# XiaoHan-Git/RO-MAP

Hardware: AMD Instinct MI355X
Metric: ray-samples/sec (train: hash-encode->MLP->composite fwd+bwd+optimizer) per object-NeRF (higher is better)
Workload: dtype fp16 params/activations, fp32 accumulate + fp32 master; 1 GPU; OfflineNeRF-style training, 1 synthetic 'room'-like object per GPU, base.json defaults (hash L=16 F=2 T=2^16, MLP 64x1), R=4096 rays x S=32 samples/step, 40 views 640x480 resident in HBM; objects=1, samples_per_ray=32, backend=1, parallelism=object-per-GPU (no training collective; RCCL gather-to-root of the final render), launcher=single process, ranks_in_collective=1, visible_devices=1

## Files before the change

include/mon_core_diag.h:

```cpp
#ifndef MON_CORE_DIAG_H
#define MON_CORE_DIAG_H
#include "mon_core.h"
#ifdef __cplusplus
extern "C" {
#endif

int mon_object_debug_read(mon_object* obj, int which, void* dst, size_t bytes);
int mon_dataset_debug_read(mon_dataset* ds, uint32_t frame, uint32_t* rgba, float* depth, float* pose16);
int mon_microbench(int device, int mode, int pattern, uint32_t n_entries, uint32_t n_ops, float* ms);
int mon_debug_fast_index(const mon_config* cfg, int level, uint32_t x, uint32_t y, uint32_t z, uint32_t* index, uint32_t* size);
int mon_debug_frag_layout(int encoded_width_padded, int n_neurons, int n_hidden_layers, int n_levels, int* source, int* slots, int* n_image, int* n_mlp);
int mon_debug_acc_layout(int encoded_width_padded, int n_neurons, int n_hidden_layers, int n_levels, int* param, int* n_cols);
int mon_selftest_mfma(int device, const uint16_t* A, const uint16_t* B, float* D);
int mon_debug_yaml_number(const char* text, const char* key, double* value);
int mon_debug_occupancy_state(mon_object* obj, uint32_t out[2]);
int mon_debug_occupancy_grid(mon_object* obj, uint32_t* raw, uint32_t* dilated, float* raw_threshold, uint32_t* n_parts);
int mon_debug_set_train_occupancy(mon_object* obj, const uint32_t* bits);

int mon_debug_render_jobs(mon_object* obj, int side, uint32_t* jobs);

int mon_debug_set_render_grid(mon_object* obj, int side, const uint32_t* bits);

int mon_debug_scene_samples(mon_object* const* objs, size_t n_objs, int side, mon_frame_bbox rect, const float* Twc16, size_t k, float* t, float* alpha,
                            float* rgb, uint32_t* count);
int mon_debug_scene_composite(int device, uint32_t n_rays, uint32_t n_lists, const float* t, const float* alpha, const float* rgb, const uint32_t* count,
                              const float* dn, float* out_rgb, float* out_depth, float* out_opacity, int32_t* out_instance);

int mon_debug_pose_samples(mon_object* obj, int side, const mon_frame_bbox* obs, size_t n_obs, const float* Tow16, const mon_pose_refine_params* p,
                           uint32_t iteration, float* x, float* raw, float* dldx);

int mon_debug_scene_pose_samples(mon_object* const* objs, size_t n_objs, int side, const mon_frame_bbox* obs, size_t n_obs, const float* Twc16,
                                 const mon_pose_refine_params* p, uint32_t iteration, const float* level_weights, size_t k, float* x_o, float* x_c, float* t,
                                 float* raw, float* dldx, uint32_t* count);
int mon_debug_scene_composite_grad(int device, uint32_t n_rays, uint32_t n_lists, const float* t, const float* alpha, const float* rgb, const uint32_t* count,
                                   const float* cstar, const float* mstar, const float* dstar, const float* dn, float w_rgb, float w_mask, float w_depth,
                                   float huber, float* out_l, float* out_W, float* out_D, float* out_dalpha, float* out_dc);
int mon_debug_checkpoint_timing(int enable, double* kernel_ms);

#ifdef __cplusplus
}
#endif
#endif
```

ro-map_amd/__init__.py:

```python
from .binding import (MonConfig, MonBBox, MonError, Dataset, ObjectNeRF, default_config, config_from_json, device_count, lib, lib_path,
                      exported_symbols, BUF, selftest_mfma, microbench, fast_index, OfflineManager, OnlineManager, png_read, png_write, marching_cubes,
                              generate_toc, frag_layout, acc_layout, device_mem_info, set_logical_devices, set_offline_schedule, set_option, get_option, diag_lib, diag_lib_path,
                              diag_symbols, yaml_number, MonRenderSkipStats, render_scene, scene_samples, scene_composite, PoseRefineParams, pose_refine_default,
                      PoseC2FParams, pose_c2f_default, pose_c2f_weights, scene_pose_loss, scene_refine_camera, scene_pose_samples,
                      scene_composite_grad, CheckpointInfo, checkpoint_info, checkpoint_timing, MON_LOAD_BOXES,
                      rccl_lib, rccl_lib_path, rccl_symbols, gather_plan, Gather)
```

ro-map_amd/binding.py:

```python
import ctypes as C
import os

import numpy as np

_HERE = os.path.dirname(os.path.abspath(__file__))


class MonError(RuntimeError):
    def __init__(self, code, msg):
        super().__init__("mon_core error %d: %s" % (code, msg)); self.code = code


class MonConfig(C.Structure):
    _fields_ = [("n_levels", C.c_int32), ("n_features", C.c_int32), ("log2_hashmap_size", C.c_int32), ("base_resolution", C.c_int32),
                ("per_level_scale", C.c_float), ("n_neurons", C.c_int32), ("n_hidden_layers", C.c_int32), ("rays_per_batch", C.c_int32),
                ("n_samples", C.c_int32), ("loss_scale", C.c_float), ("learning_rate", C.c_float), ("beta1", C.c_float), ("beta2", C.c_float),
                ("epsilon", C.c_float), ("l2_reg", C.c_float), ("ema_decay", C.c_float), ("decay_start", C.c_int32), ("decay_interval", C.c_int32),
                ("decay_base", C.c_float), ("param_seed", C.c_uint32), ("rng_flags", C.c_uint32), ("sample_seed", C.c_uint64),
                ("use_depth", C.c_int32), ("occupancy_skip", C.c_int32)]


class MonBBox(C.Structure):
    _fields_ = [("FrameId", C.c_uint32), ("x", C.c_uint32), ("y", C.c_uint32), ("h", C.c_uint32), ("w", C.c_uint32)]

# ... 19 lines not shown


class CheckpointInfo(C.Structure):
    _fields_ = [("version", C.c_uint32), ("cfg", MonConfig), ("class_id", C.c_int32), ("Tow", C.c_float * 16), ("aabb_min", C.c_float * 3),
                ("aabb_max", C.c_float * 3), ("n_params", C.c_uint32), ("n_mlp_params", C.c_uint32), ("n_grid_params", C.c_uint32),
                ("train_step", C.c_uint32), ("iter", C.c_uint32), ("n_boxes", C.c_uint32), ("backend", C.c_int32), ("has_occupancy", C.c_uint32),
                ("lazy_ema", C.c_uint32), ("file_bytes", C.c_uint64)]


MON_LOAD_BOXES = 1


def checkpoint_info(path, verify=True):
    i = CheckpointInfo(); _check(lib().mon_checkpoint_read_info(os.fsencode(path), int(bool(verify)), C.byref(i))); return i


def checkpoint_timing(enable=True):
    ms = C.c_double(0); _check(diag_lib().mon_debug_checkpoint_timing(int(bool(enable)), C.byref(ms))); return ms.value


class MonProfile(C.Structure):
    _fields_ = [("ms", C.c_double * 8), ("launches", C.c_uint64 * 8)]


K_BATCH, K_FWDBWD, K_OPTIM, K_RENDER = 0, 1, 2, 3

_SIGS = {
    "mon_last_error": (C.c_char_p, []),
    "mon_version": (C.c_int, []),
    "mon_device_count": (C.c_int, [C.POINTER(C.c_int)]),
    "mon_set_logical_devices": (C.c_int, [C.c_int]),
    "mon_offline_set_schedule": (C.c_int, [C.c_int, C.c_int]),
    "mon_set_option": (C.c_int, [C.c_char_p, C.c_long]),
    "mon_get_option": (C.c_int, [C.c_char_p, C.POINTER(C.c_long)]),
    "mon_config_default": (C.c_int, [C.POINTER(MonConfig)]),
    "mon_config_from_json": (C.c_int, [C.c_char_p, C.POINTER(MonConfig)]),
    "mon_dataset_create": (C.c_int, [C.c_int, C.c_int, C.c_int, C.c_float, C.c_float, C.c_float, C.c_float, C.c_uint32, C.c_int, C.POINTER(C.c_void_p)]),
    "mon_dataset_add_frame": (C.c_int, [C.c_void_p, C.c_uint32, C.c_void_p, C.c_int, C.c_int, C.c_void_p, C.c_void_p, C.c_void_p]),
    "mon_dataset_n_frames": (C.c_int, [C.c_void_p, C.POINTER(C.c_uint32)]),
    "mon_dataset_destroy": (C.c_int, [C.c_void_p]),
    "mon_object_create": (C.c_int, [C.c_void_p, C.POINTER(MonConfig), C.c_int, C.c_void_p, C.c_void_p, C.c_void_p, C.POINTER(C.c_void_p)]),
    "mon_object_add_boxes": (C.c_int, [C.c_void_p, C.c_void_p, C.c_size_t]),
    "mon_object_train": (C.c_int, [C.c_void_p, C.c_int, C.POINTER(C.c_float)]),
    "mon_object_render": (C.c_int, [C.c_void_p, MonBBox, C.c_void_p, C.c_int, C.c_void_p, C.c_void_p, C.c_void_p, C.c_int]),
    "mon_object_render_snapshot": (C.c_int, [C.c_void_p, MonBBox, C.c_void_p, C.c_int, C.c_void_p, C.c_void_p, C.c_void_p, C.POINTER(C.c_uint32)]),
    "mon_object_density_grid": (C.c_int, [C.c_void_p, C.c_int, C.c_int, C.c_int, C.c_void_p]),
    "mon_object_info_get": (C.c_int, [C.c_void_p, C.POINTER(MonInfo)]),
    "mon_object_get_params": (C.c_int, [C.c_void_p, C.c_int, C.c_void_p, C.c_size_t]),
    "mon_object_set_params": (C.c_int, [C.c_void_p, C.c_void_p, C.c_size_t]),
    "mon_object_train_stages": (C.c_int, [C.c_void_p, C.c_int]),
    "mon_object_set_backend": (C.c_int, [C.c_void_p, C.c_int]),
    "mon_object_set_debug_dump": (C.c_int, [C.c_void_p, C.c_int]),
    "mon_object_set_profiling": (C.c_int, [C.c_void_p, C.c_int]),
    "mon_object_get_profile": (C.c_int, [C.c_void_p, C.POINTER(MonProfile), C.c_int]),
    "mon_object_destroy": (C.c_int, [C.c_void_p]),
    "mon_offline_create": (C.c_int, [C.c_char_p, C.c_char_p, C.c_int, C.POINTER(C.c_void_p)]),
    "mon_offline_init": (C.c_int, [C.c_void_p]),
    "mon_offline_read_dataset": (C.c_int, [C.c_void_p]),
    "mon_offline_create_nerf": (C.c_int, [C.c_void_p, C.c_char_p]),
    "mon_offline_wait_threads_end": (C.c_int, [C.c_void_p]),
    "mon_offline_n_objects": (C.c_int, [C.c_void_p, C.POINTER(C.c_int)]),
    "mon_offline_object_loss": (C.c_int, [C.c_void_p, C.c_int, C.POINTER(C.c_float), C.POINTER(C.c_int)]),
    "mon_offline_render_test": (C.c_int, [C.c_void_p, C.c_int, C.c_char_p, C.c_int]),
    "mon_offline_save_mesh": (C.c_int, [C.c_void_p, C.c_int, C.c_char_p]),
    "mon_offline_destroy": (C.c_int, [C.c_void_p]),
    "mon_object_generate_mesh": (C.c_int, [C.c_void_p, C.c_int, C.c_float, C.POINTER(C.c_uint32), C.POINTER(C.c_uint32)]),
    "mon_object_mesh_counts": (C.c_int, [C.c_void_p, C.POINTER(C.c_uint32), C.POINTER(C.c_uint32), C.POINTER(C.c_uint32)]),
    "mon_object_get_mesh": (C.c_int, [C.c_void_p, C.c_void_p, C.c_void_p, C.c_void_p, C.c_void_p, C.c_int]),
    "mon_device_mem_info": (C.c_int, [C.c_int, C.c_void_p, C.c_void_p]),
    "mon_object_mesh_generation": (C.c_int, [C.c_void_p, C.c_void_p]),
    "mon_object_get_config": (C.c_int, [C.c_void_p, C.c_void_p]),
    "mon_object_copy_mesh": (C.c_int, [C.c_void_p, C.c_uint32, C.c_uint32, C.c_void_p, C.c_void_p, C.c_void_p, C.c_void_p, C.c_void_p, C.c_void_p, C.c_void_p,
            C.c_int]),
    "mon_object_get_mesh_raw": (C.c_int, [C.c_void_p, C.c_void_p, C.c_void_p]),
    "mon_object_save_mesh": (C.c_int, [C.c_void_p, C.c_char_p]),
    "mon_marching_cubes": (C.c_int, [C.c_int, C.c_void_p, C.c_int, C.c_int, C.c_int, C.c_float, C.c_void_p, C.c_void_p, C.c_void_p, C.c_void_p, C.c_void_p,
            C.c_uint32, C.c_uint32,
                                     C.POINTER(C.c_uint32), C.POINTER(C.c_uint32), C.POINTER(C.c_uint32)]),
    "mon_offline_get_intrinsics": (C.c_int, [C.c_void_p] + [C.POINTER(C.c_float)] * 4 + [C.POINTER(C.c_int)] * 2),
    "mon_offline_get_poses": (C.c_int, [C.c_void_p, C.c_void_p, C.c_size_t, C.POINTER(C.c_size_t)]),
    "mon_offline_object_meta": (C.c_int, [C.c_void_p, C.c_int, C.POINTER(C.c_int), C.c_void_p, C.c_void_p, C.c_void_p, C.c_void_p, C.c_size_t,
            C.POINTER(C.c_size_t)]),
    "mon_offline_set_output_dir": (C.c_int, [C.c_void_p, C.c_char_p]),
    "mon_offline_object": (C.c_int, [C.c_void_p, C.c_int, C.POINTER(C.c_void_p)]),
    "mon_online_object": (C.c_int, [C.c_void_p, C.c_size_t, C.POINTER(C.c_void_p)]),
    "mon_online_render_nerfs_test": (C.c_int, [C.c_void_p, C.c_char_p, C.c_size_t, C.POINTER(C.c_char_p), C.c_void_p, C.c_void_p, C.c_size_t, C.c_float]),
    "mon_generate_toc": (C.c_int, [C.c_float, C.c_float, C.c_float, C.c_void_p]),
    "mon_online_create": (C.c_int, [C.c_char_p, C.c_int, C.c_int, C.POINTER(C.c_void_p)]),
    "mon_online_init": (C.c_int, [C.c_void_p]),
    "mon_online_dataset_init": (C.c_int, [C.c_void_p, C.c_float, C.c_float, C.c_float, C.c_float, C.c_int, C.c_int, C.c_size_t]),
    "mon_online_new_frame": (C.c_int, [C.c_void_p, C.c_uint32, C.c_char_p, C.c_void_p, C.c_int, C.c_void_p, C.c_void_p, C.c_void_p]),
    "mon_online_create_nerf": (C.c_int, [C.c_void_p, C.c_int, C.c_void_p, C.c_void_p, C.c_void_p, C.POINTER(C.c_size_t)]),
    "mon_online_update_nerf_bbox": (C.c_int, [C.c_void_p, C.c_size_t, C.c_void_p, C.c_size_t, C.c_int]),
    "mon_online_get_frame_idx": (C.c_int, [C.c_void_p, C.c_char_p, C.POINTER(C.c_int)]),
    "mon_online_update_dataset": (C.c_int, [C.c_void_p, C.c_uint32, C.c_uint32, C.c_void_p]),
    "mon_online_get_pose": (C.c_int, [C.c_void_p, C.c_uint32, C.c_void_p]),
    "mon_online_wait_threads_end": (C.c_int, [C.c_void_p]),
    "mon_online_object_info": (C.c_int, [C.c_void_p, C.c_size_t, C.POINTER(C.c_float), C.POINTER(C.c_int), C.POINTER(C.c_int), C.POINTER(C.c_uint32)]),
    "mon_online_render": (C.c_int, [C.c_void_p, C.c_size_t, MonBBox, C.c_void_p, C.c_void_p, C.c_void_p, C.c_void_p]),
    "mon_online_destroy": (C.c_int, [C.c_void_p]),
    "mon_png_read": (C.c_int, [C.c_char_p, C.POINTER(C.c_int), C.POINTER(C.c_int), C.POINTER(C.c_int), C.POINTER(C.c_int), C.c_void_p, C.c_size_t]),
    "mon_png_write": (C.c_int, [C.c_char_p, C.c_int, C.c_int, C.c_int, C.c_int, C.c_void_p]),
    "mon_write_render_pngs": (C.c_int, [C.c_char_p, C.c_char_p, C.c_char_p, C.c_uint32, C.c_uint32, C.c_void_p, C.c_void_p, C.c_void_p]),
    "mon_physical_device": (C.c_int, [C.c_int, C.POINTER(C.c_int)]),
    "mon_offline_object_stamp": (C.c_int, [C.c_void_p, C.c_int, C.c_size_t, C.c_char_p, C.c_size_t]),
    "mon_device_synchronize": (C.c_int, [C.c_int]),
    "mon_object_set_render_skip": (C.c_int, [C.c_void_p, C.c_int, C.c_float]),
    "mon_object_render_skip_stats": (C.c_int, [C.c_void_p, C.c_int, C.POINTER(MonRenderSkipStats)]),
    "mon_object_render_occupancy": (C.c_int, [C.c_void_p, C.c_int, C.c_int, C.c_void_p]),
    "mon_scene_render": (C.c_int, [C.c_void_p, C.c_size_t, C.c_int, MonBBox, C.c_void_p, C.c_void_p, C.c_void_p, C.c_void_p, C.c_void_p]),
    "mon_online_render_scene": (C.c_int, [C.c_void_p, MonBBox, C.c_void_p, C.c_void_p, C.c_void_p, C.c_void_p, C.c_void_p]),
    "mon_pose_refine_default": (C.c_int, [C.POINTER(PoseRefineParams)]),
    "mon_object_pose_loss": (C.c_int, [C.c_void_p, C.c_int, C.c_void_p, C.c_size_t, C.c_void_p, C.POINTER(PoseRefineParams), C.c_uint32,
            C.POINTER(C.c_float), C.c_void_p]),
    "mon_object_refine_pose": (C.c_int, [C.c_void_p, C.c_int, C.c_void_p, C.c_size_t, C.POINTER(PoseRefineParams), C.c_void_p, C.c_void_p]),
    "mon_online_refine_pose": (C.c_int, [C.c_void_p, C.c_size_t, C.c_void_p, C.c_size_t, C.POINTER(PoseRefineParams), C.c_void_p, C.c_void_p]),
    "mon_pose_c2f_default": (C.c_int, [C.POINTER(PoseC2FParams)]),
    "mon_pose_c2f_weights": (C.c_int, [C.POINTER(PoseC2FParams), C.c_int, C.c_int, C.c_int, C.c_void_p]),
    "mon_object_pose_loss_levels": (C.c_int, [C.c_void_p, C.c_int, C.c_void_p, C.c_size_t, C.c_void_p, C.POINTER(PoseRefineParams), C.c_uint32,
            C.c_void_p, C.POINTER(C.c_float), C.c_void_p]),
    "mon_object_refine_pose_c2f": (C.c_int, [C.c_void_p, C.c_int, C.c_void_p, C.c_size_t, C.POINTER(PoseRefineParams), C.POINTER(PoseC2FParams),
            C.c_void_p, C.c_void_p]),
    "mon_online_refine_pose_c2f": (C.c_int, [C.c_void_p, C.c_size_t, C.c_void_p, C.c_size_t, C.POINTER(PoseRefineParams), C.POINTER(PoseC2FParams),
            C.c_void_p, C.c_void_p]),
    "mon_scene_pose_loss": (C.c_int, [C.c_void_p, C.c_size_t, C.c_int, C.c_void_p, C.c_size_t, C.c_void_p, C.POINTER(PoseRefineParams), C.c_uint32,
            C.c_void_p, C.POINTER(C.c_float), C.c_void_p]),
    "mon_scene_refine_camera": (C.c_int, [C.c_void_p, C.c_size_t, C.c_int, C.c_void_p, C.c_size_t, C.POINTER(PoseRefineParams), C.POINTER(PoseC2FParams),
            C.c_void_p, C.c_void_p]),
    "mon_online_refine_camera": (C.c_int, [C.c_void_p, C.c_void_p, C.c_size_t, C.POINTER(PoseRefineParams), C.POINTER(PoseC2FParams), C.c_void_p,
            C.c_void_p]),
    "mon_checkpoint_read_info": (C.c_int, [C.c_char_p, C.c_int, C.c_void_p]),
    "mon_object_save": (C.c_int, [C.c_void_p, C.c_char_p]),
    "mon_object_load": (C.c_int, [C.c_void_p, C.c_char_p, C.c_uint32, C.POINTER(C.c_void_p)]),
    "mon_online_save_map": (C.c_int, [C.c_void_p, C.c_char_p]),
    "mon_online_load_map": (C.c_int, [C.c_void_p, C.c_char_p, C.c_uint32, C.POINTER(C.c_size_t)]),
}


_DIAG_SIGS = {
    "mon_object_debug_read": (C.c_int, [C.c_void_p, C.c_int, C.c_void_p, C.c_size_t]),
    "mon_dataset_debug_read": (C.c_int, [C.c_void_p, C.c_uint32, C.c_void_p, C.c_void_p, C.c_void_p]),
    "mon_microbench": (C.c_int, [C.c_int, C.c_int, C.c_int, C.c_uint32, C.c_uint32, C.POINTER(C.c_float)]),
    "mon_debug_frag_layout": (C.c_int, [C.c_int, C.c_int, C.c_int, C.c_int, C.c_void_p, C.c_void_p, C.POINTER(C.c_int), C.POINTER(C.c_int)]),
    "mon_debug_acc_layout": (C.c_int, [C.c_int, C.c_int, C.c_int, C.c_int, C.c_void_p, C.POINTER(C.c_int)]),
    "mon_debug_fast_index": (C.c_int, [C.POINTER(MonConfig), C.c_int, C.c_uint32, C.c_uint32, C.c_uint32, C.POINTER(C.c_uint32), C.POINTER(C.c_uint32)]),
    "mon_selftest_mfma": (C.c_int, [C.c_int, C.c_void_p, C.c_void_p, C.c_void_p]),
    "mon_debug_yaml_number": (C.c_int, [C.c_char_p, C.c_char_p, C.POINTER(C.c_double)]),
    "mon_debug_render_jobs": (C.c_int, [C.c_void_p, C.c_int, C.POINTER(C.c_uint32)]),
    "mon_debug_occupancy_state": (C.c_int, [C.c_void_p, C.POINTER(C.c_uint32)]),
    "mon_debug_occupancy_grid": (C.c_int, [C.c_void_p, C.c_void_p, C.c_void_p, C.POINTER(C.c_float), C.POINTER(C.c_uint32)]),
    "mon_debug_set_train_occupancy": (C.c_int, [C.c_void_p, C.c_void_p]),
    "mon_debug_set_render_grid": (C.c_int, [C.c_void_p, C.c_int, C.c_void_p]),
    "mon_debug_checkpoint_timing": (C.c_int, [C.c_int, C.POINTER(C.c_double)]),
    "mon_debug_scene_samples": (C.c_int, [C.c_void_p, C.c_size_t, C.c_int, MonBBox, C.c_void_p, C.c_size_t, C.c_void_p, C.c_void_p, C.c_void_p, C.c_void_p]),
    "mon_debug_scene_composite": (C.c_int, [C.c_int, C.c_uint32, C.c_uint32, C.c_void_p, C.c_void_p, C.c_void_p, C.c_void_p, C.c_void_p, C.c_void_p,
            C.c_void_p, C.c_void_p, C.c_void_p]),
    "mon_debug_pose_samples": (C.c_int, [C.c_void_p, C.c_int, C.c_void_p, C.c_size_t, C.c_void_p, C.POINTER(PoseRefineParams), C.c_uint32, C.c_void_p,
            C.c_void_p, C.c_void_p]),
    "mon_debug_scene_pose_samples": (C.c_int, [C.c_void_p, C.c_size_t, C.c_int, C.c_void_p, C.c_size_t, C.c_void_p, C.POINTER(PoseRefineParams), C.c_uint32,
            C.c_void_p, C.c_size_t, C.c_void_p, C.c_void_p, C.c_void_p, C.c_void_p, C.c_void_p, C.c_void_p]),
    "mon_debug_scene_composite_grad": (C.c_int, [C.c_int, C.c_uint32, C.c_uint32, C.c_void_p, C.c_void_p, C.c_void_p, C.c_void_p, C.c_void_p, C.c_void_p,
            C.c_void_p, C.c_void_p, C.c_float, C.c_float, C.c_float, C.c_float, C.c_void_p, C.c_void_p, C.c_void_p, C.c_void_p, C.c_void_p]),
}


def exported_symbols():
    return sorted(_SIGS)


_RCCL_SIGS = {
    "mon_gather_create": (C.c_int, [C.c_int, C.POINTER(C.c_void_p)]),
    "mon_gather_destroy": (C.c_int, [C.c_void_p]),
    "mon_gather_plan": (C.c_int, [C.c_void_p, C.c_void_p, C.c_int, C.c_int, C.c_void_p, C.c_void_p]),
    "mon_gather_renders": (C.c_int, [C.c_void_p, C.c_void_p, C.c_void_p, C.c_void_p, C.c_int, C.c_int, C.c_void_p, C.c_void_p, C.c_void_p]),
    "mon_gather_stats": (C.c_int, [C.c_void_p, C.POINTER(C.c_uint64), C.POINTER(C.c_uint64), C.POINTER(C.c_int), C.POINTER(C.c_double)]),
    "mon_gather_transport_stats": (C.c_int, [C.c_void_p, C.POINTER(C.c_int), C.POINTER(C.c_uint64), C.POINTER(C.c_int), C.POINTER(C.c_uint64), C.POINTER(C.c_int)]),
    "mon_gather_set_transport": (C.c_int, [C.c_void_p, C.c_int]),
    "mon_gather_last_error": (C.c_char_p, []),
    "mon_offline_render_test_gathered": (C.c_int, [C.c_void_p, C.c_void_p, C.c_char_p, C.c_int]),
}
_rccl_lib = None


def rccl_symbols():
    return sorted(_RCCL_SIGS)


def rccl_lib_path():
    return os.path.join(os.path.dirname(os.path.abspath(__file__)), "libmon_core_rccl.so")


def rccl_lib():
    global _rccl_lib
    if _rccl_lib is None:
        lib()
        L = C.CDLL(rccl_lib_path(), mode=C.RTLD_GLOBAL)
        for name, (res, args) in _RCCL_SIGS.items():
            f = getattr(L, name); f.restype = res; f.argtypes = args
        _rccl_lib = L
    return _rccl_lib


def gather_plan(object_device, n_pix, n_devices):
    d = np.ascontiguousarray(object_device, np.int32); p = np.ascontiguousarray(n_pix, np.uint32)
    per = np.zeros(n_devices, np.uint64); off = np.zeros(len(d), np.uint64)
    rc = rccl_lib().mon_gather_plan(_p(d), _p(p), len(d), int(n_devices), _p(per), _p(off))
    if rc:
        raise MonError(rc, "mon_gather_plan failed")
    return per, off


def _gather_error():
    return (rccl_lib().mon_gather_last_error() or b"").decode("utf-8", "replace")


class Gather:

    def __init__(self, root_device=0):
        self.h = C.c_void_p()
        rc = rccl_lib().mon_gather_create(int(root_device), C.byref(self.h))
        if rc:
            raise MonError(rc, "mon_gather_create: " + _gather_error())

    AUTO, RCCL, PEER_COPY = 0, 1, 2

    def set_transport(self, transport):
        rc = rccl_lib().mon_gather_set_transport(self.h, int(transport))
        if rc:
            raise MonError(rc, "mon_gather_set_transport: " + _gather_error())

    def renders(self, objects, boxes, poses16, pose_is_Toc=False):
        n = len(objects); b = np.ascontiguousarray(boxes, np.uint32).reshape(n, 5); T = np.ascontiguousarray(poses16, np.float32).reshape(n, 16)
        oh = (C.c_void_p * n)(*[o.h for o in objects])
        rgb = [np.empty((int(q[3]), int(q[4]), 3), np.float32) for q in b]; dep = [np.empty((int(q[3]), int(q[4])), np.float32) for q in b]
        msk = [np.empty_like(d) for d in dep]
        pr = (C.c_void_p * n)(*[a.ctypes.data for a in rgb]); pd = (C.c_void_p * n)(*[a.ctypes.data for a in dep])
        pm = (C.c_void_p * n)(*[a.ctypes.data for a in msk])
        rc = rccl_lib().mon_gather_renders(self.h, oh, _p(b), _p(T), int(pose_is_Toc), n, pr, pd, pm)
        if rc:
            raise MonError(rc, "mon_gather_renders: " + _gather_error())
        return list(zip(rgb, dep, msk))

    def stats(self):
        a = C.c_uint64(0); b = C.c_uint64(0); s = C.c_int(0); ms = C.c_double(0)
        rccl_lib().mon_gather_stats(self.h, C.byref(a), C.byref(b), C.byref(s), C.byref(ms))
        nr = C.c_int(0); br = C.c_uint64(0); mr = C.c_int(0); bc = C.c_uint64(0); mc = C.c_int(0)
        rccl_lib().mon_gather_transport_stats(self.h, C.byref(nr), C.byref(br), C.byref(mr), C.byref(bc), C.byref(mc))
        return dict(bytes_over_links=a.value, bytes_on_root=b.value, sending_devices=s.value, transfer_ms=ms.value, n_ranks=nr.value, bytes_rccl=br.value,
                messages_rccl=mr.value, bytes_peer_copy=bc.value, messages_peer_copy=mc.value)

    def offline_render_test(self, manager, out_dir, max_views=0):
        rc = rccl_lib().mon_offline_render_test_gathered(self.h, manager.h, out_dir.encode(), int(max_views))
        if rc:
            raise MonError(rc, "mon_offline_render_test_gathered: " + _gather_error())

    def close(self):
        if self.h:
            rccl_lib().mon_gather_destroy(self.h); self.h = C.c_void_p()


def diag_symbols():
    return sorted(_DIAG_SIGS)


def lib_path():
    return os.environ.get("MON_CORE_LIB") or os.path.join(_HERE, "libmon_core.so")


_lib = None


def lib():
    global _lib
    if _lib is None:
        p = lib_path()
        if not os.path.exists(p):
            raise MonError(-1, "libmon_core.so not built (run python -c 'import __graft_entry__ as g; g.build()')")
        L = C.CDLL(p)
        for name, (res, args) in _SIGS.items():
            fn = getattr(L, name); fn.restype = res; fn.argtypes = args
        _lib = L
        for kv in filter(None, os.environ.get("MON_OPTIONS", "").split(",")):
            k, v = kv.split("=")
            if k.strip() == "offline_schedule":
                o, i = v.lower().split("x"); rc = L.mon_offline_set_schedule(int(o), int(i))
            else:
                rc = L.mon_set_option(k.strip().encode(), int(v))
            if rc != 0:
                raise MonError(rc, L.mon_last_error().decode("utf-8", "replace"))
    return _lib


_diag = None


def diag_lib_path():
    return os.path.join(os.path.dirname(lib_path()), "libmon_core_diag.so")


def diag_lib():
    global _diag
    if _diag is None:
        lib()
        p = diag_lib_path()
        if not os.path.exists(p):
            raise MonError(-1, "libmon_core_diag.so not built")
        L = C.CDLL(p)
        for name, (res, args) in _DIAG_SIGS.items():
            fn = getattr(L, name); fn.restype = res; fn.argtypes = args
        _diag = L
    return _diag


def set_option(name, value):
    _check(lib().mon_set_option(name.encode(), int(value)))


def get_option(name):
    v = C.c_long(0); _check(lib().mon_get_option(name.encode(), C.byref(v))); return v.value


def yaml_number(text, key):
    v = C.c_double(0); _check(diag_lib().mon_debug_yaml_number(text.encode(), key.encode(), C.byref(v))); return v.value


def _check(rc):
    if rc != 0:
        raise MonError(rc, lib().mon_last_error().decode("utf-8", "replace"))


def _p(a):
    return None if a is None else a.ctypes.data_as(C.c_void_p)


def device_count():
    n = C.c_int(0)
    rc = lib().mon_device_count(C.byref(n))
    return n.value if rc == 0 else 0


def set_offline_schedule(outer=10, inner=500):
    _check(lib().mon_offline_set_schedule(int(outer), int(inner)))


def set_logical_devices(n):
    _check(lib().mon_set_logical_devices(int(n)))


def device_mem_info(device=0):
    f = C.c_size_t(0); t = C.c_size_t(0); _check(lib().mon_device_mem_info(int(device), C.byref(f), C.byref(t))); return f.value, t.value


def default_config(**kw):
    c = MonConfig(); _check(lib().mon_config_default(C.byref(c)))
    kw = dict(kw)
    rng = int(kw.pop("xorwow", 0)) | (int(bool(kw.pop("tcnn_init_order", 0))) << 4) | ((int(kw.pop("xorwow_lanes", 0)) // 1024) << 16)
    for k, v in kw.items():
        setattr(c, k, v)
    c.rng_flags |= rng
    return c


def config_from_json(path):
    c = MonConfig(); _check(lib().mon_config_from_json(path.encode(), C.byref(c))); return c


def selftest_mfma(A_h, B_h, device=0):
    A = np.ascontiguousarray(A_h, np.uint16); B = np.ascontiguousarray(B_h, np.uint16); D = np.empty((32, 32), np.float32)
    _check(diag_lib().mon_selftest_mfma(device, _p(A), _p(B), _p(D))); return D


def fast_index(cfg, level, x, y, z):
    i = C.c_uint32(0); n = C.c_uint32(0); _check(diag_lib().mon_debug_fast_index(C.byref(cfg), level, x, y, z, C.byref(i), C.byref(n))); return i.value, n.value


def microbench(mode, pattern, n_entries, n_ops, device=0):
    ms = C.c_float(0); _check(diag_lib().mon_microbench(device, mode, pattern, n_entries, n_ops, C.byref(ms))); return ms.value


class Dataset:

    def __init__(self, device, H, W, fx, fy, cx, cy, max_frames, use_depth=False):
        self.h = C.c_void_p(); self.H, self.W = H, W
        _check(lib().mon_dataset_create(device, H, W, fx, fy, cx, cy, max_frames, int(use_depth), C.byref(self.h)))

    def add_frame(self, frame_id, rgb_u8, instance_u8, Twc16, depth=None, is_bgr=False):
        rgb = np.ascontiguousarray(rgb_u8, np.uint8); inst = np.ascontiguousarray(instance_u8, np.uint8)
        pose = np.ascontiguousarray(Twc16, np.float32); d = None if depth is None else np.ascontiguousarray(depth, np.float32)
        assert rgb.shape[:2] == (self.H, self.W) and inst.shape == (self.H, self.W) and pose.size == 16
        _check(lib().mon_dataset_add_frame(self.h, frame_id, _p(rgb), rgb.shape[2], int(is_bgr), _p(inst), _p(d), _p(pose)))

    @property
    def n_frames(self):
        n = C.c_uint32(0); _check(lib().mon_dataset_n_frames(self.h, C.byref(n))); return n.value

    def debug_read(self, frame_id, with_depth=False):
        rgba = np.empty((self.H, self.W), np.uint32); pose = np.empty(16, np.float32); dep = np.empty((self.H, self.W), np.float32) if with_depth else None
        _check(diag_lib().mon_dataset_debug_read(self.h, frame_id, _p(rgba), _p(dep), _p(pose)))
        return rgba, dep, pose

    def close(self):
        if self.h:
            lib().mon_dataset_destroy(self.h); self.h = None


BUF = dict(master=0, half=1, ema=2, m1=3, m2=4, steps=5, gmlp=6, ggrid_h=9, pts=10, tdist=11, E=12, Hid=13, O=14, dO=15, dHid=16, dE=17,
           rgb_ray=18, depth_ray=19, mask_ray=20, loss_ray=21, ray_o=22, ray_d=23, ray_t0=24, ray_t1=25, target=26, target_depth=27, bgcol=28,
           ray_flag=29, ray_dn=31, mask=32, state=33, frag_train=34, frag_ref=35, x_all=36, e_soa=37, half_tiles=38, ggrid_f32=39, live_cnt=40)


class ObjectNeRF:

    def __init__(self, dataset, cfg, class_id, Tow16, aabb_min, aabb_max):
        self.h = C.c_void_p(); self.cfg = cfg; self.ds = dataset
        a, b, c = (np.ascontiguousarray(v, np.float32) for v in (Tow16, aabb_min, aabb_max))
        _check(lib().mon_object_create(dataset.h, C.byref(cfg), int(class_id), _p(a), _p(b), _p(c), C.byref(self.h)))
        self.R, self.S = cfg.rays_per_batch, cfg.n_samples

    def close(self):
        if self.h:
            lib().mon_object_destroy(self.h); self.h = None

    def add_boxes(self, boxes):
        b = np.ascontiguousarray(boxes, np.uint32).reshape(-1, 5)
        _check(lib().mon_object_add_boxes(self.h, _p(b), b.shape[0]))

    def save(self, path):
        _check(lib().mon_object_save(self.h, os.fsencode(path)))

    @classmethod
    def load(cls, dataset, path, with_boxes=True):
        h = C.c_void_p()
        _check(lib().mon_object_load(dataset.h, os.fsencode(path), MON_LOAD_BOXES if with_boxes else 0, C.byref(h)))
        o = cls.__new__(cls); o.h = h; o.ds = dataset
        o.cfg = MonConfig(); _check(lib().mon_object_get_config(h, C.byref(o.cfg))); o.R, o.S = o.cfg.rays_per_batch, o.cfg.n_samples
        return o

    def train(self, iters):
        loss = C.c_float(0); _check(lib().mon_object_train(self.h, iters, C.byref(loss))); return loss.value

    def train_stages(self, bits):
        _check(lib().mon_object_train_stages(self.h, bits))

    def set_backend(self, backend):
        _check(lib().mon_object_set_backend(self.h, backend))

    def info(self):
        i = MonInfo(); _check(lib().mon_object_info_get(self.h, C.byref(i))); return i

    def render(self, box, pose16, pose_is_Toc=False):
        FrameId, x, y, h, w = (int(v) for v in box)
        rgb = np.empty((h, w, 3), np.float32); depth = np.empty((h, w), np.float32); mask = np.empty((h, w), np.float32)
        pose = np.ascontiguousarray(pose16, np.float32)
        _check(lib().mon_object_render(self.h, MonBBox(FrameId, x, y, h, w), _p(pose), int(pose_is_Toc), _p(rgb), _p(depth), _p(mask), 0))
        return rgb, depth, mask

    def render_snapshot(self, box, pose16, pose_is_Toc=False):
        FrameId, x, y, h, w = (int(v) for v in box)
        rgb = np.empty((h, w, 3), np.float32); depth = np.empty((h, w), np.float32); mask = np.empty((h, w), np.float32); st = C.c_uint32(0)
        pose = np.ascontiguousarray(pose16, np.float32)
        _check(lib().mon_object_render_snapshot(self.h, MonBBox(FrameId, x, y, h, w), _p(pose), int(pose_is_Toc), _p(rgb), _p(depth), _p(mask), C.byref(st)))
        return rgb, depth, mask, st.value

    def render_into(self, box, pose16, rgb_ptr, depth_ptr, mask_ptr, on_device, pose_is_Toc=False):
        FrameId, x, y, h, w = (int(v) for v in box)
        pose = np.ascontiguousarray(pose16, np.float32)
        _check(lib().mon_object_render(self.h, MonBBox(FrameId, x, y, h, w), _p(pose), int(pose_is_Toc), C.c_void_p(int(rgb_ptr)), C.c_void_p(int(depth_ptr)),
                C.c_void_p(int(mask_ptr)), int(bool(on_device))))

    def generate_mesh(self, res=64, thresh=2.0):
        nv = C.c_uint32(0); ni = C.c_uint32(0)
        _check(lib().mon_object_generate_mesh(self.h, int(res), float(thresh), C.byref(nv), C.byref(ni))); return nv.value, ni.value

    def get_mesh(self, try_lock=False, raw=False):
        nv = C.c_uint32(0); nr = C.c_uint32(0); ni = C.c_uint32(0)
        _check(lib().mon_object_mesh_counts(self.h, C.byref(nv), C.byref(nr), C.byref(ni)))
        for _ in range(8):
            cv, ci = nv.value, ni.value
            out = dict(verts=np.empty((cv, 3), np.float32), normals=np.empty((cv, 3), np.float32), colors=np.empty((cv, 3), np.uint8), indices=np.empty(ci,
                    np.uint32))
            rc = lib().mon_object_copy_mesh(self.h, cv, ci, _p(out["verts"]), _p(out["normals"]), _p(out["colors"]), _p(out["indices"]),
                                            C.byref(nv), C.byref(nr), C.byref(ni), int(try_lock))
            if rc == 1 and (nv.value > cv or ni.value > ci):
                continue
            _check(rc); break
        else:
            raise MonError(1, "get_mesh: mesh kept growing")
        out = {k: (v[:nv.value] if k != "indices" else v[:ni.value]) for k, v in out.items()}; out["n_verts_real"] = nr.value
        if raw:
            out["normals_raw"] = np.empty((nv.value, 3), np.float32); out["colors_f32"] = np.empty((nv.value, 3), np.float32)
            _check(lib().mon_object_get_mesh_raw(self.h, _p(out["normals_raw"]), _p(out["colors_f32"])))
        return out

    def mesh_generation(self):
        g = C.c_uint64(0); _check(lib().mon_object_mesh_generation(self.h, C.byref(g))); return g.value

    def save_mesh(self, path):
        _check(lib().mon_object_save_mesh(self.h, path.encode()))

    def set_render_skip(self, enable, min_alpha=1e-3):
        _check(lib().mon_object_set_render_skip(self.h, int(bool(enable)), float(min_alpha)))

    def render_skip_stats(self, side=0):
        st = MonRenderSkipStats(); _check(lib().mon_object_render_skip_stats(self.h, int(side), C.byref(st)))
        return {f: int(getattr(st, f)) for f, _ in MonRenderSkipStats._fields_}

    def render_occupancy(self, side=0, dilated=True):
        w = np.empty(8192, np.uint32); _check(lib().mon_object_render_occupancy(self.h, int(side), int(bool(dilated)), _p(w)))
        return np.unpackbits(w.view(np.uint8), bitorder="little").astype(bool).reshape(64, 64, 64)

    def debug_set_render_grid(self, side, grid):
        if grid is None:
            _check(diag_lib().mon_debug_set_render_grid(self.h, int(side), None)); return
        w = np.packbits(np.ascontiguousarray(grid, bool).reshape(-1), bitorder="little").view(np.uint32)
        _check(diag_lib().mon_debug_set_render_grid(self.h, int(side), _p(w)))

    def density_grid(self, rx, ry, rz):
        out = np.empty(rx * ry * rz, np.float32); _check(lib().mon_object_density_grid(self.h, rx, ry, rz, _p(out))); return out

    def get_params(self, which=0):
        n = self.info().n_params
        out = np.empty(n, np.float32 if which == 0 else np.uint16)
        _check(lib().mon_object_get_params(self.h, which, _p(out), out.nbytes)); return out

    def set_params(self, master):
        m = np.ascontiguousarray(master, np.float32); _check(lib().mon_object_set_params(self.h, _p(m), m.size))

    def buffer(self, name):
        i = self.info(); R, B, n = self.R, self.R * self.S, i.n_params
        W, NH, Ep = self.cfg.n_neurons, self.cfg.n_hidden_layers, i.encoded_width
        shapes = dict(master=(np.float32, n), half=(np.uint16, n), ema=(np.uint16, n), m1=(np.float32, n), m2=(np.float32, n), steps=(np.uint32, n),
                      gmlp=(np.float32, i.n_mlp_params), ggrid_h=(np.uint16, i.n_grid_params), ggrid_f32=(np.float32, i.n_grid_params), pts=(np.float32, B * 3), tdist=(np.float32, B),
                      E=(np.uint16, B * Ep), Hid=(np.uint16, B * W * NH), O=(np.uint16, B * 4), dO=(np.uint16, B * 4), dHid=(np.uint16, B * W * NH),
                      dE=(np.uint16, B * Ep), rgb_ray=(np.float32, R * 3), depth_ray=(np.float32, R), mask_ray=(np.float32, R), loss_ray=(np.float32, R),
                      ray_o=(np.float32, R * 3), ray_d=(np.float32, R * 3), ray_t0=(np.float32, R), ray_t1=(np.float32, R), target=(np.float32, R * 3),
                      target_depth=(np.float32, R), bgcol=(np.float32, R * 3), ray_flag=(np.uint8, R), ray_dn=(np.float32, R), mask=(np.uint64, R // 64),
                      state=(np.uint32, 28 + 2 * 128 * 16), frag_train=(np.uint16, 64 * 512), frag_ref=(np.uint16, 64 * 512),
                      live_cnt=(np.uint32, 2 * 64 * 16), x_all=(np.float32, B * 4), e_soa=(np.uint16, B * 2 * self.cfg.n_levels), half_tiles=(np.uint16, i.n_grid_params))
        dt, cnt = shapes[name]; out = np.empty(cnt, dt)
        _check(diag_lib().mon_object_debug_read(self.h, BUF[name], _p(out), out.nbytes)); return out

    def occupancy_state(self):
        out = (C.c_uint32 * 2)(); _check(diag_lib().mon_debug_occupancy_state(self.h, out)); return int(out[0]), int(out[1])

    def occupancy_grid(self):
        raw = np.empty(8192, np.uint32); dil = np.empty(8192, np.uint32); thr = C.c_float(0); n_parts = C.c_uint32(0)
        _check(diag_lib().mon_debug_occupancy_grid(self.h, _p(raw), _p(dil), C.byref(thr), C.byref(n_parts)))
        return raw, dil, float(thr.value), int(n_parts.value)

    def set_train_occupancy(self, bits):
        if bits is None:
            _check(diag_lib().mon_debug_set_train_occupancy(self.h, None)); return
        w = np.ascontiguousarray(bits, np.uint32); assert w.size == 8192
        _check(diag_lib().mon_debug_set_train_occupancy(self.h, _p(w)))

    def render_jobs(self, side=0):
        n = C.c_uint32(0); _check(diag_lib().mon_debug_render_jobs(self.h, int(side), C.byref(n))); return n.value

    def pose_loss(self, obs, Tow16, params=None, side=0, iteration=0):
        b, prm = _pose_boxes(obs), _pose_params(params); pose = np.ascontiguousarray(Tow16, np.float32).reshape(16)
        loss = C.c_float(0); g = np.empty(6, np.float32)
        _check(lib().mon_object_pose_loss(self.h, int(side), _p(b), b.shape[0], _p(pose), C.byref(prm), int(iteration), C.byref(loss), _p(g)))
        return loss.value, g

    def refine_pose(self, obs, Tow16, params=None, side=0):
        b, prm = _pose_boxes(obs), _pose_params(params); pose = np.array(Tow16, np.float32).reshape(16)
        trace = np.empty(prm.iters + 1, np.float32)
        _check(lib().mon_object_refine_pose(self.h, int(side), _p(b), b.shape[0], C.byref(prm), _p(pose), _p(trace)))
        return pose, trace

    def pose_loss_levels(self, obs, Tow16, level_weights, params=None, side=0, iteration=0):
        b, prm = _pose_boxes(obs), _pose_params(params); pose = np.ascontiguousarray(Tow16, np.float32).reshape(16)
        w = np.ascontiguousarray(level_weights, np.float32).reshape(-1)
        if w.size != self.cfg.n_levels:
            raise ValueError("level_weights: %d values for %d levels" % (w.size, self.cfg.n_levels))
        loss = C.c_float(0); g = np.empty(6, np.float32)
        _check(lib().mon_object_pose_loss_levels(self.h, int(side), _p(b), b.shape[0], _p(pose), C.byref(prm), int(iteration), _p(w), C.byref(loss), _p(g)))
        return loss.value, g

    def refine_pose_c2f(self, obs, Tow16, params=None, c2f=None, side=0):
        b, prm, c = _pose_boxes(obs), _pose_params(params), _c2f_params(c2f); pose = np.array(Tow16, np.float32).reshape(16)
        trace = np.empty(prm.iters + 1, np.float32)
        _check(lib().mon_object_refine_pose_c2f(self.h, int(side), _p(b), b.shape[0], C.byref(prm), C.byref(c), _p(pose), _p(trace)))
        return pose, trace

    def pose_samples(self, obs, Tow16, params=None, side=0, iteration=0):
        b, prm = _pose_boxes(obs), _pose_params(params); pose = np.ascontiguousarray(Tow16, np.float32).reshape(16)
        n = int(prm.rays_per_iter) or int(sum(int(v[3]) * int(v[4]) for v in b))
        x = np.empty((n, 64, 3), np.float32); raw = np.empty((n, 64, 4), np.float32); g = np.empty((n, 64, 3), np.float32)
        _check(diag_lib().mon_debug_pose_samples(self.h, int(side), _p(b), b.shape[0], _p(pose), C.byref(prm), int(iteration), _p(x), _p(raw), _p(g)))
        return x, raw, g

    def set_debug_dump(self, on):
        _check(lib().mon_object_set_debug_dump(self.h, int(on)))

    def set_profiling(self, on):
        _check(lib().mon_object_set_profiling(self.h, int(on)))

    def profile(self, reset=True):
        p = MonProfile(); _check(lib().mon_object_get_profile(self.h, C.byref(p), int(reset)))
        return {"ms": list(p.ms), "launches": list(p.launches)}


def png_read(path):
    w, h, c, d = C.c_int(0), C.c_int(0), C.c_int(0), C.c_int(0)
    _check(lib().mon_png_read(path.encode(), C.byref(w), C.byref(h), C.byref(c), C.byref(d), None, 0))
    buf = np.empty(w.value * h.value * c.value * d.value // 8, np.uint8)
    _check(lib().mon_png_read(path.encode(), C.byref(w), C.byref(h), C.byref(c), C.byref(d), _p(buf), buf.nbytes))
    if d.value == 16:
        return buf.view(">u2").astype(np.uint16).reshape(h.value, w.value, c.value)
    return buf.reshape(h.value, w.value, c.value)


def png_write(path, arr):
    a = np.asarray(arr)
    if a.ndim == 2:
        a = a[..., None]
    data = np.ascontiguousarray(a.astype(">u2") if a.dtype == np.uint16 else a.astype(np.uint8))
    _check(lib().mon_png_write(path.encode(), a.shape[1], a.shape[0], a.shape[2], 16 if arr.dtype == np.uint16 else 8, data.ctypes.data_as(C.c_void_p)))


class OfflineManager:

    def __init__(self, dataset_path, config_path, use_dense_depth=False):
        self.h = C.c_void_p()
        _check(lib().mon_offline_create(dataset_path.encode(), config_path.encode(), int(use_dense_depth), C.byref(self.h)))

    def init(self):
        _check(lib().mon_offline_init(self.h))

    def read_dataset(self):
        _check(lib().mon_offline_read_dataset(self.h))

    def create_nerf(self, object_file):
        _check(lib().mon_offline_create_nerf(self.h, object_file.encode()))

    def wait_threads_end(self):
        _check(lib().mon_offline_wait_threads_end(self.h))

    def n_objects(self):
        n = C.c_int(0); _check(lib().mon_offline_n_objects(self.h, C.byref(n))); return n.value

    def object_loss(self, idx):
        l = C.c_float(0); d = C.c_int(0); _check(lib().mon_offline_object_loss(self.h, idx, C.byref(l), C.byref(d))); return l.value, d.value

    def set_output_dir(self, path):
        _check(lib().mon_offline_set_output_dir(self.h, path.encode()))

    def intrinsics(self):
        f = [C.c_float(0) for _ in range(4)]; hw = [C.c_int(0), C.c_int(0)]
        _check(lib().mon_offline_get_intrinsics(self.h, *[C.byref(v) for v in f + hw])); return tuple(v.value for v in f + hw)

    def poses(self):
        n = C.c_size_t(0); _check(lib().mon_offline_get_poses(self.h, None, 0, C.byref(n)))
        T = np.empty((n.value, 16), np.float32); _check(lib().mon_offline_get_poses(self.h, _p(T), n.value, C.byref(n))); return T

    def object_meta(self, idx):
        n = C.c_size_t(0); cls = C.c_int(0); Tow = np.empty(16, np.float32); a0 = np.empty(3, np.float32); a1 = np.empty(3, np.float32)
        _check(lib().mon_offline_object_meta(self.h, idx, C.byref(cls), _p(Tow), _p(a0), _p(a1), None, 0, C.byref(n)))
        boxes = np.empty((n.value, 5), np.uint32)
        _check(lib().mon_offline_object_meta(self.h, idx, None, None, None, None, _p(boxes), n.value, C.byref(n)))
        return dict(cls=cls.value, Tow=Tow, aabb_min=a0, aabb_max=a1, boxes=boxes)

    def object(self, idx):
        h = C.c_void_p(); _check(lib().mon_offline_object(self.h, idx, C.byref(h))); return _borrowed_object(h)

    def render_test(self, idx, out_dir, max_views=0):
        _check(lib().mon_offline_render_test(self.h, idx, out_dir.encode(), max_views))

    def close(self):
        if self.h:
            lib().mon_offline_destroy(self.h); self.h = None


class OnlineManager:

    def __init__(self, config_path, use_sparse_depth=False, train_step_iterations=500):
        self.h = C.c_void_p()
        _check(lib().mon_online_create(config_path.encode(), int(use_sparse_depth), int(train_step_iterations), C.byref(self.h)))

    def init(self):
        _check(lib().mon_online_init(self.h))

    def dataset_init(self, fx, fy, cx, cy, H, W, imgs):
        _check(lib().mon_online_dataset_init(self.h, fx, fy, cx, cy, H, W, imgs))

    def new_frame(self, img_id, stamp, bgr_u8, instance_u8, Twc16, depth=None):
        bgr = np.ascontiguousarray(bgr_u8, np.uint8); inst = np.ascontiguousarray(instance_u8, np.uint8); pose = np.ascontiguousarray(Twc16, np.float32)
        d = None if depth is None else np.ascontiguousarray(depth, np.float32)
        _check(lib().mon_online_new_frame(self.h, img_id, stamp.encode(), _p(bgr), bgr.shape[2], _p(inst), _p(d), _p(pose)))

    def create_nerf(self, cls, Tow16, aabb_min, aabb_max):
        a, b, c = (np.ascontiguousarray(v, np.float32) for v in (Tow16, aabb_min, aabb_max)); idx = C.c_size_t(0)
        _check(lib().mon_online_create_nerf(self.h, int(cls), _p(a), _p(b), _p(c), C.byref(idx))); return idx.value

    def update_nerf_bbox(self, idx, boxes, train_step):
        b = np.ascontiguousarray(boxes, np.uint32).reshape(-1, 5)
        _check(lib().mon_online_update_nerf_bbox(self.h, idx, _p(b), b.shape[0], int(train_step)))

    def update_dataset(self, cur_id, Twc16s):
        T = np.ascontiguousarray(Twc16s, np.float32).reshape(-1, 16); _check(lib().mon_online_update_dataset(self.h, int(cur_id), T.shape[0], _p(T)))

    def get_pose(self, frame_id):
        T = np.empty(16, np.float32); _check(lib().mon_online_get_pose(self.h, int(frame_id), _p(T))); return T

    def get_frame_idx(self, stamp):
        i = C.c_int(0); _check(lib().mon_online_get_frame_idx(self.h, stamp.encode(), C.byref(i))); return i.value

# ... 220 lines not shown
```

ro-map_amd/csrc/diag.cpp:

```cpp
#include <algorithm>
#include <cstring>
#include <string>
#include <vector>
#include "model.h"
#include "frag_layout.h"
#include "../../include/mon_core_diag.h"

namespace mon {
void set_error(const char* fmt, ...);
int ensure_ema_current(Model& m);
int microbench(int device, int mode, int pattern, uint32_t n_entries, uint32_t n_ops, float* ms);
int selftest_mfma(int device, const uint16_t* A, const uint16_t* B, float* D);
bool read_yaml_number(const std::string& text, const char* key, double& v);

#define HIPCHECK(expr)                                                                                         \
    do { hipError_t _e = (expr); if (_e != hipSuccess) {                                                       \
        set_error("%s failed: %s (%s:%d)", #expr, hipGetErrorString(_e), __FILE__, __LINE__); return MON_ERR_HIP; } } while (0)

int model_debug_read(Model& m, int which, void* dst, size_t bytes) {
    model_leave_lane(m);
    if (which == MON_BUF_EMA) { int rc = ensure_ema_current(m); if (rc) return rc; }
    const size_t R = m.oc.R, B = R * m.oc.S, n = m.n_params; const void* src = nullptr; size_t sz = 0;
    if (m.P.rec && (which == MON_BUF_MASTER || which == MON_BUF_M1 || which == MON_BUF_M2 || which == MON_BUF_STEPS)) {
        if (!dst || bytes < n * 4) { set_error("debug_read: buffer too small"); return MON_ERR_ARG; }
        HIPCHECK(use_device(m.device)); void* tmp = nullptr; HIPCHECK(hipMalloc(&tmp, n * 4));
        launch_state_unpack(m.train_stream, m.P.rec, which == MON_BUF_MASTER ? 0 : which == MON_BUF_M1 ? 1 : which == MON_BUF_M2 ? 2 : 3, tmp, (uint32_t)n);
        hipError_t e = hipStreamSynchronize(m.train_stream); if (e == hipSuccess) e = hipMemcpy(dst, tmp, n * 4, hipMemcpyDeviceToHost);
        (void)hipFree(tmp); HIPCHECK(e); return MON_OK;
    }
    switch (which) {
        case MON_BUF_MASTER: src = m.P.master; sz = n * 4; break;       case MON_BUF_HALF: src = m.P.half; sz = n * 2; break;
        case MON_BUF_EMA: src = m.P.ema; sz = n * 2; break;             case MON_BUF_M1: src = m.P.m1; sz = n * 4; break;
        case MON_BUF_M2: src = m.P.m2; sz = n * 4; break;
        case MON_BUF_STEPS: src = m.P.steps ? (const void*)m.P.steps : (const void*)m.P.steps16; sz = n * 4; break;
        case MON_BUF_GMLP: src = m.P.gmlp; sz = (size_t)m.nd.n_mlp * 4; break;
        case MON_BUF_GGRID_H: src = m.P.ggrid; sz = (size_t)m.n_grid * 2; break;
        case MON_BUF_GGRID_F32: src = m.P.ggrid; sz = (size_t)m.n_grid * 4; break;
        case MON_BUF_PTS: src = m.B.pts; sz = B * 12; break;            case MON_BUF_TDIST: src = m.B.tdist; sz = B * 4; break;
        case MON_BUF_E: src = m.B.E; sz = B * m.nd.Epad * 2; break;     case MON_BUF_HID: src = m.B.Hid; sz = B * m.nd.W * m.nd.NH * 2; break;
        case MON_BUF_O: src = m.B.O; sz = B * 8; break;                 case MON_BUF_DO: src = m.B.dO; sz = B * 8; break;
        case MON_BUF_DHID: src = m.B.dHid; sz = B * m.nd.W * m.nd.NH * 2; break;
        case MON_BUF_DE: src = m.B.dE; sz = B * m.nd.Epad * 2; break;
        case MON_BUF_RGB_RAY: src = m.B.rgb_ray; sz = R * 12; break;    case MON_BUF_DEPTH_RAY: src = m.B.depth_ray; sz = R * 4; break;
        case MON_BUF_MASK_RAY: src = m.B.mask_ray; sz = R * 4; break;   case MON_BUF_LOSS_RAY: src = m.B.loss_ray; sz = R * 4; break;
        case MON_BUF_RAY_O: src = m.B.ray_o; sz = R * 12; break;        case MON_BUF_RAY_D: src = m.B.ray_d; sz = R * 12; break;
        case MON_BUF_RAY_T0: src = m.B.ray_t0; sz = R * 4; break;       case MON_BUF_RAY_T1: src = m.B.ray_t1; sz = R * 4; break;
        case MON_BUF_TARGET: src = m.B.target; sz = R * 12; break;      case MON_BUF_TARGET_DEPTH: src = m.B.target_depth; sz = R * 4; break;
        case MON_BUF_BGCOL: src = m.B.bgcol; sz = R * 12; break;        case MON_BUF_RAY_FLAG: src = m.B.ray_flag; sz = R; break;
        case MON_BUF_RAY_DN: src = m.B.ray_dn; sz = R * 4; break;       case MON_BUF_MASK: src = m.B.mask; sz = (R / 64) * 8; break;
        case MON_BUF_STATE: src = m.d_state; sz = sizeof(DevState); break;
        case MON_BUF_FRAG_TRAIN: src = m.d_frag_train; sz = 64 * 512 * 2; break;
        case MON_BUF_X_ALL: if (!m.d_x_all) { set_error("debug_read: level-tile encode not in use"); return MON_ERR_STATE; } src = m.d_x_all; sz = B * 16;
        break;
        case MON_BUF_E_SOA: if (!m.d_e_soa) { set_error("debug_read: level-tile encode not in use"); return MON_ERR_STATE; } src = m.d_e_soa;
        sz = B * (size_t)m.nd.L * 4; break;
        case MON_BUF_HALF_TILES: if (!m.d_half_tiles) { set_error("debug_read: level-tile encode not in use"); return MON_ERR_STATE; } src = m.d_half_tiles;
        sz = (size_t)m.n_grid * 2; break;
        case MON_BUF_LIVE_CNT: if (!m.d_live_cnt) { set_error("debug_read: no live-sample lists (occupancy_skip off, or not on the level tiles)"); return MON_ERR_STATE; }
            src = m.d_live_cnt; sz = 2u * kLiveMaxParts * kLiveCntStride * 4u; break;
        case MON_BUF_FRAG_REF:
            if (!m.d_frag_render) { set_error("debug_read: fused backend not available"); return MON_ERR_STATE; }
            HIPCHECK(use_device(m.device)); HIPCHECK(hipMemsetAsync(m.d_frag_render, 0, 64 * 512 * 2, m.train_stream));
            launch_build_frag_image(m.train_stream, m.P.half, m.nd, m.d_frag_render); src = m.d_frag_render; sz = 64 * 512 * 2; break;
        default: set_error("debug_read: unknown buffer id %d", which); return MON_ERR_ARG;
    }
    if (!dst || bytes < sz) { set_error("debug_read: buffer too small (%zu < %zu)", bytes, sz); return MON_ERR_ARG; }
    HIPCHECK(use_device(m.device)); HIPCHECK(hipStreamSynchronize(m.train_stream));
    if (which == MON_BUF_STEPS && !m.P.steps) {
        std::vector<uint16_t> h16(n); HIPCHECK(hipMemcpy(h16.data(), src, n * 2, hipMemcpyDeviceToHost));
        uint32_t* out = reinterpret_cast<uint32_t*>(dst); for (size_t i = 0; i < n; ++i) out[i] = h16[i];
        return MON_OK;
    }
    if (which == MON_BUF_GGRID_H || which == MON_BUF_GGRID_F32) {
        std::vector<uint16_t> tab(m.n_grid); HIPCHECK(hipMemcpy(tab.data(), m.P.ggrid, (size_t)m.n_grid * 2, hipMemcpyDeviceToHost));
        std::vector<float> acc(m.n_grid);
        for (uint32_t i = 0; i < m.n_grid; ++i) { _Float16 h; std::memcpy(&h, &tab[i], 2); acc[i] = (float)h; }
        const bool parts = (m.backend == 1 && m.lds_mask) || (m.backend == 0 && m.hybrid_scatter && which == MON_BUF_GGRID_F32);
        if (parts) {
            const uint32_t n_ent = m.part_halves / 2, n_half = n_ent / 2;
            std::vector<uint16_t> pa(m.part_halves), pb(m.part_halves);
            auto val = [&](const std::vector<uint16_t>& part, uint32_t e, uint32_t f) { _Float16 h;
                std::memcpy(&h, &part[((size_t)f * 2 + (e & 1u)) * n_half + (e >> 1)], 2); return (float)h; };
            for (uint32_t q = 0; q < m.scatter.max_P; q += 2) {
                HIPCHECK(hipMemcpy(pa.data(), m.d_gpart + (size_t)q * m.part_halves, (size_t)m.part_halves * 2, hipMemcpyDeviceToHost));
                if (q + 1 < m.scatter.max_P) HIPCHECK(hipMemcpy(pb.data(), m.d_gpart + (size_t)(q + 1) * m.part_halves, (size_t)m.part_halves * 2,
                        hipMemcpyDeviceToHost));
                for (int l = 0; l < m.nd.L; ++l) {
                    const bool lds_level = m.backend == 1 ? ((m.lds_mask >> l) & 1u) != 0u : true;
                    if (q >= m.scatter.P[l] || !lds_level) continue;
                    const bool two = q + 1 < m.scatter.P[l];
                    for (uint32_t e = m.lt.offset[l]; e < m.lt.offset[l + 1]; ++e) for (uint32_t f = 0; f < 2; ++f)
                        acc[2 * e + f] += two ? val(pa, e, f) + val(pb, e, f) : val(pa, e, f);
                }
            }
        }
        if (which == MON_BUF_GGRID_F32) {
            if (!dst || bytes < (size_t)m.n_grid * 4) { set_error("debug_read: buffer too small"); return MON_ERR_ARG; }
            std::memcpy(dst, acc.data(), (size_t)m.n_grid * 4); return MON_OK;
        }
        uint16_t* out = reinterpret_cast<uint16_t*>(dst);
        for (uint32_t i = 0; i < m.n_grid; ++i) { const _Float16 h = (_Float16)acc[i]; std::memcpy(&out[i], &h, 2); }
        return MON_OK;
    }
    HIPCHECK(hipMemcpy(dst, src, sz, hipMemcpyDeviceToHost));
    return MON_OK;
}


}

using namespace mon;
#define REQUIRE(p, what) do { if (!(p)) { set_error("%s: null %s", __func__, what); return MON_ERR_ARG; } } while (0)

extern "C" {
int mon_object_debug_read(mon_object* o, int which, void* dst, size_t bytes) { REQUIRE(o, "object"); return model_debug_read(*o->m, which, dst, bytes); }
int mon_dataset_debug_read(mon_dataset* ds, uint32_t frame, uint32_t* rgba, float* depth, float* pose16) {
    REQUIRE(ds, "dataset"); Dataset& d = *ds->d;
    if (frame >= d.max_frames) { set_error("dataset_debug_read: frame %u >= capacity %u", frame, d.max_frames); return MON_ERR_ARG; }
    const size_t px = (size_t)d.K.H * d.K.W;
    HIPCHECK(use_device(d.device)); HIPCHECK(hipDeviceSynchronize());
    if (rgba) HIPCHECK(hipMemcpy(rgba, d.d_rgba + px * frame, px * 4, hipMemcpyDeviceToHost));
    if (depth && d.d_depth) HIPCHECK(hipMemcpy(depth, d.d_depth + px * frame, px * 4, hipMemcpyDeviceToHost));
    if (pose16) HIPCHECK(hipMemcpy(pose16, d.d_poses + 16 * (size_t)frame, 64, hipMemcpyDeviceToHost));
    return MON_OK;
}
int mon_microbench(int device, int mode, int pattern, uint32_t n_entries, uint32_t n_ops, float* ms) { REQUIRE(ms, "ms");
    return microbench(device, mode, pattern, n_entries, n_ops, ms); }
int mon_debug_fast_index(const mon_config* cfg, int level, uint32_t x, uint32_t y, uint32_t z, uint32_t* index, uint32_t* size) {
    REQUIRE(cfg, "cfg"); REQUIRE(index, "index"); REQUIRE(size, "size");
    LevelTable lt{}; NetDims nd{}; uint32_t n_grid = 0; int rc = level_table_build(*cfg, lt, nd, n_grid); if (rc) return rc;
    if (level < 0 || level >= nd.L) { set_error("level out of range"); return MON_ERR_ARG; }
    LevelFast lf{}; level_fast_build(lt, nd, lf);
    *index = fast_grid_index(lf, level, x, y, z); *size = lf.size[level]; return MON_OK;
}
int mon_debug_frag_layout(int epad, int W, int NH, int L, int* source, int* slots, int* n_image, int* n_mlp) {
    if (!(epad == 16 || epad == 32) || !((((W == 32 || W == 64) && (NH == 1 || NH == 2)) || (W == 128 && NH == 1))) || L < 1 || 2 * L > epad) { set_error("frag_layout: unsupported shape");
        return MON_ERR_ARG; }
    const FragDims d{ epad, W, NH, L };
    if (n_image) *n_image = d.N_FRAGS() * 512;
    if (n_mlp) *n_mlp = d.N_MLP();
    if (source) for (int i = 0; i < d.N_FRAGS() * 512; ++i) source[i] = frag_source(d, i);
    if (slots) for (int p = 0; p < d.N_MLP(); ++p) { int o[2] = { -1, -1 }; const int n = frag_slots(d, p, o); slots[2 * p] = n > 0 ? o[0] : -1;
        slots[2 * p + 1] = n > 1 ? o[1] : -1; }
    return MON_OK;
}
int mon_debug_acc_layout(int epad, int W, int NH, int L, int* param, int* n_cols) {
    if (!(epad == 16 || epad == 32) || !((((W == 32 || W == 64) && (NH == 1 || NH == 2)) || (W == 128 && NH == 1))) || L < 1 || 2 * L > epad) { set_error("acc_layout: unsupported shape");
        return MON_ERR_ARG; }
    const FragDims d{ epad, W, NH, L };
    if (n_cols) *n_cols = acc_cols(d);
    if (param) for (int i = 0; i < acc_cols(d); ++i) param[i] = acc_param(d, i);
    return MON_OK;
}
int mon_selftest_mfma(int device, const uint16_t* A, const uint16_t* B, float* D) { REQUIRE(A, "A"); REQUIRE(B, "B"); REQUIRE(D, "D");
    return selftest_mfma(device, A, B, D); }
int mon_debug_checkpoint_timing(int enable, double* kernel_ms) { return mon::checkpoint_timing(enable, kernel_ms); }
int mon_debug_occupancy_state(mon_object* o, uint32_t out[2]) {
    if (!o || !o->m || !out) { mon::set_error("debug_occupancy_state: null argument"); return MON_ERR_ARG; }
    out[0] = o->m->occ_refreshed_iter; out[1] = o->m->occ_next_refresh; return MON_OK;
}
int mon_debug_occupancy_grid(mon_object* o, uint32_t* raw, uint32_t* dilated, float* raw_threshold, uint32_t* n_parts) {
    if (!o || !o->m) { mon::set_error("debug_occupancy_grid: null object"); return MON_ERR_ARG; }
    mon::Model& m = *o->m;
    if (!m.d_occ) { mon::set_error("debug_occupancy_grid: the object has no occupancy grid"); return MON_ERR_STATE; }
    mon::model_leave_lane(m);
    HIPCHECK(mon::use_device(m.device)); HIPCHECK(hipStreamSynchronize(m.train_stream));
    constexpr size_t bytes = (size_t)mon::kOccWords * 4;
    if (raw) HIPCHECK(hipMemcpy(raw, m.occ_refreshed_iter ? m.d_occ_tmp : m.d_occ, bytes, hipMemcpyDeviceToHost));
    if (dilated) HIPCHECK(hipMemcpy(dilated, m.d_occ, bytes, hipMemcpyDeviceToHost));
    if (raw_threshold) *raw_threshold = m.occ_raw_threshold;
    if (n_parts) { const uint32_t B = m.oc.R * m.oc.S, spw = mon::encode_tiles_spw(B); *n_parts = m.d_live_idx ? (B + spw - 1u) / spw : 0u; }
    return MON_OK;
}
int mon_debug_set_train_occupancy(mon_object* o, const uint32_t* bits) {
    if (!o || !o->m) { mon::set_error("debug_set_train_occupancy: null object"); return MON_ERR_ARG; }
    mon::Model& m = *o->m;
    if (!m.d_occ) { mon::set_error("debug_set_train_occupancy: the object has no occupancy grid"); return MON_ERR_STATE; }
    mon::model_leave_lane(m);
    HIPCHECK(mon::use_device(m.device)); HIPCHECK(hipStreamSynchronize(m.train_stream));
    constexpr size_t bytes = (size_t)mon::kOccWords * 4;
    if (bits) {
        HIPCHECK(hipMemcpy(m.d_occ, bits, bytes, hipMemcpyHostToDevice)); HIPCHECK(hipMemcpy(m.d_occ_tmp, bits, bytes, hipMemcpyHostToDevice));
        m.occ_pinned = true; if (!m.occ_refreshed_iter) m.occ_refreshed_iter = m.h_state.iter > 1u ? m.h_state.iter : 1u;
    } else if (m.occ_pinned) {
        m.occ_pinned = false;
        if (m.h_state.iter < (uint32_t)mon::kOccWarmup) { HIPCHECK(hipMemset(m.d_occ, 0xff, bytes)); m.occ_refreshed_iter = 0; }
        m.occ_next_refresh = 0;
    }
    m.points_ready = false;
    return MON_OK;
}
int mon_debug_render_jobs(mon_object* o, int side, uint32_t* jobs) {
    if (!o || !o->m || !jobs) { mon::set_error("debug_render_jobs: null argument"); return MON_ERR_ARG; }
    if (!o->m->tile_ok) { mon::set_error("debug_render_jobs: this object does not render on level tiles"); return MON_ERR_STATE; }
    mon::TileWs* ws = nullptr; const int rc = mon::tile_ws_get(*o->m, side, 0, &ws); if (rc) return rc;
    std::lock_guard<std::mutex> l(ws->mu);
    if (!ws->counters) { mon::set_error("debug_render_jobs: no tile workspace on the object's device"); return MON_ERR_STATE; }
    if (mon::use_device(o->m->device) != hipSuccess || hipDeviceSynchronize() != hipSuccess) { mon::set_error("debug_render_jobs: device error");
        return MON_ERR_HIP; }
    if (hipMemcpy(jobs, ws->counters + 16u * ((ws->flip + 1u) & 1u), 4, hipMemcpyDeviceToHost) != hipSuccess) {
        mon::set_error("debug_render_jobs: copy failed"); return MON_ERR_HIP; }
    return MON_OK;
}
int mon_debug_set_render_grid(mon_object* o, int side, const uint32_t* bits) { REQUIRE(o, "object");
    return mon::model_debug_set_render_grid(*o->m, side, bits); }
int mon_debug_scene_samples(mon_object* const* objs, size_t n_objs, int side, mon_frame_bbox rect, const float* Twc16, size_t k, float* t, float* alpha,
                            float* rgb, uint32_t* count) {
    REQUIRE(objs, "objs"); REQUIRE(Twc16, "Twc16");
    if (n_objs == 0 || k >= n_objs || rect.w == 0 || rect.h == 0) { set_error("debug_scene_samples: empty list or rect, or k out of range"); return MON_ERR_ARG; }
    std::vector<mon::Model*> ms(n_objs);
    for (size_t j = 0; j < n_objs; ++j) { REQUIRE(objs[j], "object"); ms[j] = objs[j]->m; }
    const size_t px = (size_t)rect.w * rect.h; std::vector<float> img(3 * px), dep(px);
    const mon::SceneDump dump{ (uint32_t)k, t, alpha, rgb, count };
    return mon::scene_render(ms.data(), n_objs, side, rect, Twc16, img.data(), dep.data(), nullptr, nullptr, nullptr, &dump);
}
int mon_debug_scene_composite(int device, uint32_t n_rays, uint32_t n_lists, const float* t, const float* alpha, const float* rgb, const uint32_t* count,
                              const float* dn, float* out_rgb, float* out_depth, float* out_opacity, int32_t* out_instance) {
    REQUIRE(t, "t"); REQUIRE(alpha, "alpha"); REQUIRE(rgb, "rgb"); REQUIRE(count, "count"); REQUIRE(dn, "dn"); REQUIRE(out_rgb, "out_rgb");
    REQUIRE(out_depth, "out_depth"); REQUIRE(out_opacity, "out_opacity"); REQUIRE(out_instance, "out_instance");
    if (n_rays == 0 || n_lists == 0 || n_lists > mon::kSceneMaxLists) { set_error("debug_scene_composite: %u rays, %u lists", n_rays, n_lists);
        return MON_ERR_ARG; }
    const size_t nl = (size_t)n_lists * n_rays, ns = nl * mon::kSceneListLen;
    for (size_t i = 0; i < nl; ++i) if (count[i] > mon::kSceneListLen) { set_error("debug_scene_composite: count %u > 64", count[i]); return MON_ERR_ARG; }
    std::vector<float> attr(4 * ns);
    for (size_t i = 0; i < ns; ++i) { attr[4 * i] = alpha[i]; attr[4 * i + 1] = rgb[3 * i]; attr[4 * i + 2] = rgb[3 * i + 1]; attr[4 * i + 3] = rgb[3 * i + 2]; }
    HIPCHECK(mon::use_device(device));
    char* d = nullptr; const size_t b_t = ns * 4, b_a = ns * 16, b_c = nl * 4, b_dn = (size_t)n_rays * 4, b_out = (size_t)n_rays * 24;
    HIPCHECK(hipMalloc((void**)&d, b_t + b_a + b_c + b_dn + b_out));
    float* d_t = (float*)d; float* d_a = (float*)(d + b_t); uint32_t* d_c = (uint32_t*)(d + b_t + b_a); float* d_dn = (float*)(d + b_t + b_a + b_c);
    float* d_out = (float*)(d + b_t + b_a + b_c + b_dn);
    hipError_t e = hipMemcpy(d_t, t, b_t, hipMemcpyHostToDevice);
    if (e == hipSuccess) e = hipMemcpy(d_a, attr.data(), b_a, hipMemcpyHostToDevice);
    if (e == hipSuccess) e = hipMemcpy(d_c, count, b_c, hipMemcpyHostToDevice);
    if (e == hipSuccess) e = hipMemcpy(d_dn, dn, b_dn, hipMemcpyHostToDevice);
    if (e == hipSuccess) {
        mon::launch_scene_composite(nullptr, n_rays, n_lists, n_rays, d_t, d_a, d_c, d_dn, d_out, d_out + 3 * (size_t)n_rays, d_out + 4 * (size_t)n_rays,
                reinterpret_cast<int32_t*>(d_out + 5 * (size_t)n_rays));
        e = hipGetLastError();
    }
    if (e == hipSuccess) e = hipDeviceSynchronize();
    std::vector<float> out(6 * (size_t)n_rays);
    if (e == hipSuccess) e = hipMemcpy(out.data(), d_out, b_out, hipMemcpyDeviceToHost);
    (void)hipFree(d);
    HIPCHECK(e);
    std::memcpy(out_rgb, out.data(), 12 * (size_t)n_rays); std::memcpy(out_depth, out.data() + 3 * (size_t)n_rays, 4 * (size_t)n_rays);
    std::memcpy(out_opacity, out.data() + 4 * (size_t)n_rays, 4 * (size_t)n_rays); std::memcpy(out_instance, out.data() + 5 * (size_t)n_rays, 4 * (size_t)n_rays);
    return MON_OK;
}
int mon_debug_pose_samples(mon_object* o, int side, const mon_frame_bbox* obs, size_t n_obs, const float* Tow16, const mon_pose_refine_params* p,
                           uint32_t iteration, float* x, float* raw, float* dldx) {
    REQUIRE(o, "object"); REQUIRE(obs, "obs"); REQUIRE(Tow16, "pose"); REQUIRE(p, "params");
    if (n_obs == 0) { set_error("debug_pose_samples: no boxes"); return MON_ERR_ARG; }
    const mon::PoseDump dump{ x, raw, dldx };
    return mon::pose_refine(*o->m, side, obs, n_obs, Tow16, *p, -1, iteration, nullptr, nullptr, nullptr, nullptr, &dump);
}
int mon_debug_scene_pose_samples(mon_object* const* objs, size_t n_objs, int side, const mon_frame_bbox* obs, size_t n_obs, const float* Twc16,
                                 const mon_pose_refine_params* p, uint32_t iteration, const float* level_weights, size_t k, float* x_o, float* x_c, float* t,
                                 float* raw, float* dldx, uint32_t* count) {
    REQUIRE(objs, "objs"); REQUIRE(obs, "obs"); REQUIRE(Twc16, "Twc16"); REQUIRE(p, "params");
    if (n_objs == 0 || n_objs > mon::kSceneMaxLists || k >= n_objs) { set_error("debug_scene_pose_samples: empty list or k out of range"); return MON_ERR_ARG; }
    std::vector<mon::Model*> ms(n_objs);
    for (size_t j = 0; j < n_objs; ++j) { REQUIRE(objs[j], "object"); ms[j] = objs[j]->m; }
    const mon::ScenePoseDump dump{ (uint32_t)k, x_o, x_c, t, raw, dldx, count };
    return mon::scene_pose(ms.data(), n_objs, side, obs, n_obs, Twc16, *p, -1, iteration, nullptr, nullptr, nullptr, nullptr, &dump, level_weights);
}
int mon_debug_scene_composite_grad(int device, uint32_t n_rays, uint32_t n_lists, const float* t, const float* alpha, const float* rgb, const uint32_t* count,
                                   const float* cstar, const float* mstar, const float* dstar, const float* dn, float w_rgb, float w_mask, float w_depth,
                                   float huber, float* out_l, float* out_W, float* out_D, float* out_dalpha, float* out_dc) {
    REQUIRE(t, "t"); REQUIRE(alpha, "alpha"); REQUIRE(rgb, "rgb"); REQUIRE(count, "count"); REQUIRE(cstar, "cstar"); REQUIRE(mstar, "mstar");
    REQUIRE(dstar, "dstar"); REQUIRE(dn, "dn"); REQUIRE(out_l, "out_l"); REQUIRE(out_W, "out_W"); REQUIRE(out_D, "out_D"); REQUIRE(out_dalpha, "out_dalpha");
    REQUIRE(out_dc, "out_dc");
    if (n_rays == 0 || n_lists == 0 || n_lists > mon::kSceneMaxLists) { set_error("debug_scene_composite_grad: %u rays, %u lists", n_rays, n_lists);
        return MON_ERR_ARG; }
    const size_t nl = (size_t)n_lists * n_rays, ns = nl * mon::kSceneListLen;
    for (size_t i = 0; i < nl; ++i) if (count[i] > mon::kSceneListLen) { set_error("debug_scene_composite_grad: count %u > 64", count[i]); return MON_ERR_ARG; }
    std::vector<float> attr(4 * ns), ray(12 * (size_t)n_rays, 0.f);
    for (size_t i = 0; i < ns; ++i) { attr[4 * i] = alpha[i]; attr[4 * i + 1] = rgb[3 * i]; attr[4 * i + 2] = rgb[3 * i + 1]; attr[4 * i + 3] = rgb[3 * i + 2]; }
    for (size_t r = 0; r < n_rays; ++r) {
        float M = 0.f; for (uint32_t k = 0; k < n_lists; ++k) M = std::max(M, mstar[(size_t)k * n_rays + r]);
        float* q = ray.data() + 12 * r; q[0] = cstar[3 * r]; q[1] = cstar[3 * r + 1]; q[2] = cstar[3 * r + 2]; q[3] = dstar[r]; q[4] = dn[r]; q[5] = M;
    }
    if (!mon::launch_scene_composite_grad || !mon::scene_comp_grad_grid) { set_error("debug_scene_composite_grad: built without kernels_scene_pose.hip");
        return MON_ERR_STATE; }
    HIPCHECK(mon::use_device(device));
    const uint32_t n_lp = mon::scene_comp_grad_grid(n_rays);
    const size_t b_t = ns * 4, b_a = ns * 16, b_c = nl * 4, b_m = nl * 4, b_ray = (size_t)n_rays * 48, b_gw = ns * 8, b_grow = (size_t)n_rays * 16,
                 b_lp = (size_t)n_lp * 4, b_W = nl * 4, b_D = (size_t)n_rays * 4;
    const size_t sizes[] = { b_a, b_ray, b_grow, b_gw, b_t, b_c, b_m, b_lp, b_W, b_D };
    size_t off[11] = { 0 }; for (int i = 0; i < 10; ++i) off[i + 1] = off[i] + ((sizes[i] + 15) & ~(size_t)15);
    char* d = nullptr; HIPCHECK(hipMalloc((void**)&d, off[10]));
    float* d_a = (float*)(d + off[0]); float* d_ray = (float*)(d + off[1]); float* d_grow = (float*)(d + off[2]); float* d_gw = (float*)(d + off[3]);
    float* d_t = (float*)(d + off[4]); uint32_t* d_c = (uint32_t*)(d + off[5]); float* d_m = (float*)(d + off[6]); float* d_lp = (float*)(d + off[7]);
    float* d_W = (float*)(d + off[8]); float* d_D = (float*)(d + off[9]);
    hipError_t e = hipMemcpy(d_t, t, b_t, hipMemcpyHostToDevice);
    if (e == hipSuccess) e = hipMemcpy(d_a, attr.data(), b_a, hipMemcpyHostToDevice);
    if (e == hipSuccess) e = hipMemcpy(d_c, count, b_c, hipMemcpyHostToDevice);
    if (e == hipSuccess) e = hipMemcpy(d_m, mstar, b_m, hipMemcpyHostToDevice);
    if (e == hipSuccess) e = hipMemcpy(d_ray, ray.data(), b_ray, hipMemcpyHostToDevice);
    if (e == hipSuccess) e = hipMemset(d_gw, 0, b_gw);
    if (e == hipSuccess) {
        mon::SceneCompGradArgs a{}; a.n_rays = n_rays; a.n_lists = n_lists; a.cap = n_rays; a.t = d_t; a.attr = reinterpret_cast<const float4*>(d_a); a.cnt = d_c;
        a.mstar = d_m; a.ray = reinterpret_cast<const float4*>(d_ray); a.w_rgb = w_rgb; a.w_mask = w_mask; a.w_depth = w_depth; a.huber = huber;
        a.gw = reinterpret_cast<float2*>(d_gw); a.grow = reinterpret_cast<float4*>(d_grow); a.loss_part = d_lp; a.out_W = d_W; a.out_D = d_D;
        mon::launch_scene_composite_grad(nullptr, a);
        e = hipGetLastError();
    }
    if (e == hipSuccess) e = hipDeviceSynchronize();
    std::vector<float> gw(2 * ns), grow(4 * (size_t)n_rays);
    if (e == hipSuccess) e = hipMemcpy(gw.data(), d_gw, b_gw, hipMemcpyDeviceToHost);
// ... 20 lines not shown
```

ro-map_amd/csrc/diag_kernels.hip:

```cpp
#include "device_common.h"
#include "model.h"

namespace mon {
void set_error(const char* fmt, ...);

__global__ void __launch_bounds__(64) k_selftest_mfma(const uint16_t* __restrict__ A, const uint16_t* __restrict__ B, float* __restrict__ D) {
    const int l = threadIdx.x, i = l & 31, hk = l >> 5;
    half8_t a, b;
#pragma unroll
    for (int j = 0; j < 8; ++j) {
        a[j] = reinterpret_cast<const half_t*>(A)[i * 16 + 8 * hk + j];
        b[j] = reinterpret_cast<const half_t*>(B)[(8 * hk + j) * 32 + i];
    }
    float16_t c = { 0 };
    c = __builtin_amdgcn_mfma_f32_32x32x16_f16(a, b, c, 0, 0, 0);
#pragma unroll
    for (int r = 0; r < 16; ++r) D[((r & 3) + 8 * (r >> 2) + 4 * hk) * 32 + i] = c[r];
}

int selftest_mfma(int device, const uint16_t* A, const uint16_t* B, float* D) {
    int ndev = 0;
    if (hipGetDeviceCount(&ndev) != hipSuccess || ndev < 1 || use_device(device) != hipSuccess) { set_error("selftest: no HIP device");
        return MON_ERR_NO_DEVICE; }
    uint16_t *dA = nullptr, *dB = nullptr; float* dD = nullptr;
    if (hipMalloc((void**)&dA, 32 * 16 * 2) != hipSuccess || hipMalloc((void**)&dB, 16 * 32 * 2) != hipSuccess
            || hipMalloc((void**)&dD, 32 * 32 * 4) != hipSuccess) { set_error("selftest: hipMalloc failed"); return MON_ERR_HIP; }
    hipMemcpy(dA, A, 32 * 16 * 2, hipMemcpyHostToDevice); hipMemcpy(dB, B, 16 * 32 * 2, hipMemcpyHostToDevice);
    hipLaunchKernelGGL(k_selftest_mfma, dim3(1), dim3(64), 0, 0, dA, dB, dD);
    const hipError_t e = hipMemcpy(D, dD, 32 * 32 * 4, hipMemcpyDeviceToHost);
    hipFree(dA); hipFree(dB); hipFree(dD);
    if (e != hipSuccess) { set_error("selftest: %s", hipGetErrorString(e)); return MON_ERR_HIP; }
    return MON_OK;
}


}
```

ro-map_amd/csrc/kernels_optim.hip:

```cpp
#include <cstdlib>
#include "device_common.h"
#include "model.h"
#include "frag_layout.h"
#include "batch_device.h"
#include "encode_device.h"
#include "store_policy.h"

namespace mon {

template <bool STREAM, class T> __device__ __forceinline__ void state_store(T v, T* p) { policy_store<STREAM ? MON_SP_STATE : MON_SP_PLAIN>(v, p); }

__device__ __forceinline__ float adam_update(float g, float w, float& m1, float& m2, uint32_t& steps, float lr0, const OptimConst& oc, uint32_t step_cap) {
    const float gsq = g * g;
    m1 = oc.beta1 * m1 + (1.f - oc.beta1) * g;
    m2 = oc.beta2 * m2 + (1.f - oc.beta2) * gsq;
    const uint32_t cs = min(steps + 1u, step_cap); steps = cs;
    const float lr = lr0 * sqrtf(1.f - exp2f((float)cs * oc.log2_beta2)) / (1.f - exp2f((float)cs * oc.log2_beta1));
    const float eff = lr / (sqrtf(m2) + oc.epsilon);
    return w - eff * m1;
}

__device__ __forceinline__ void ema_catch_up(half8_t& e, const half8_t& w, uint32_t t, uint32_t k, float log2_d) {
    const float dk = exp2f((float)k * log2_d), a = dk * (1.f - exp2f((float)t * log2_d)), b = 1.f - dk, inv = 1.f / (1.f - exp2f((float)(t + k) * log2_d));
#pragma unroll
    for (int j = 0; j < 8; ++j) e[j] = (half_t)(((float)e[j] * a + (float)w[j] * b) * inv);
}

template <bool DENSE, bool LAZY, bool ONE = false ,
          bool LIVE = false>
__global__ void __launch_bounds__(256) k_optimizer(ParamPtrs p, OptimConst oc, const DevState* __restrict__ st, DevState* __restrict__ st_next, OptimNext nx,
        uint32_t lazy_below) {
    const uint32_t n_extra = nx.cand_blocks + nx.pos_blocks, n_opt = gridDim.x - n_extra, vblock = blockIdx.x < n_opt ? blockIdx.x + n_extra
            : blockIdx.x - n_opt;
    typedef uint32_t u32x4 __attribute__((ext_vector_type(4)));
    constexpr int kSpHalf = DENSE ? MON_SP_HALF : MON_SP_PLAIN, kSpTiles = DENSE ? MON_SP_TILES : MON_SP_PLAIN, kSpEma = DENSE ? MON_SP_EMA : MON_SP_PLAIN;
    constexpr int kSpFrag = DENSE ? MON_SP_FRAG : MON_SP_PLAIN;
    float* const prec = LAZY ? p.rec : nullptr;
    const uint32_t step_cap = (p.steps16 || prec) ? 65535u : 0xffffffffu;
    auto st_master = [&](uint32_t c) -> float* { return prec ? prec + 32u * (size_t)c : p.master + 8u * (size_t)c; };
    auto st_m1 = [&](uint32_t c) -> float* { return prec ? prec + 32u * (size_t)c + 8u : p.m1 + 8u * (size_t)c; };
    auto st_m2 = [&](uint32_t c) -> float* { return prec ? prec + 32u * (size_t)c + 16u : p.m2 + 8u * (size_t)c; };
    auto st_steps16 = [&](uint32_t c) -> uint16_t* { return prec ? reinterpret_cast<uint16_t*>(prec + 32u * (size_t)c + 24u) : p.steps16 + 8u * (size_t)c; };
    auto ema_step_of = [&](uint32_t c) -> uint32_t* { return prec ? reinterpret_cast<uint32_t*>(prec + 32u * (size_t)c + 28u) : p.ema_step + c; };
    auto load_steps = [&](uint32_t i0, u32x4& s0, u32x4& s1) __attribute__((always_inline)) {
        if (p.steps16 || prec) { const u32x4 v = *reinterpret_cast<const u32x4*>(st_steps16(i0 >> 3));
            s0 = u32x4{ v[0] & 0xffffu, v[0] >> 16, v[1] & 0xffffu, v[1] >> 16 }; s1 = u32x4{ v[2] & 0xffffu, v[2] >> 16, v[3] & 0xffffu, v[3] >> 16 }; }
        else { s0 = *reinterpret_cast<const u32x4*>(p.steps + i0); s1 = *reinterpret_cast<const u32x4*>(p.steps + i0 + 4); }
    };
    struct Pre { float4_t w0, w1, a0, a1, b0, b1; u32x4 s0, s1; half8_t e; float4_t gm0, gm1; };
    auto issue = [&](uint32_t c, Pre& L) __attribute__((always_inline)) {
        const uint32_t i0 = c << 3;
        L.w0 = *reinterpret_cast<const float4_t*>(st_master(c)); L.w1 = *reinterpret_cast<const float4_t*>(st_master(c) + 4);
        L.a0 = *reinterpret_cast<const float4_t*>(st_m1(c)); L.a1 = *reinterpret_cast<const float4_t*>(st_m1(c) + 4);
        L.b0 = *reinterpret_cast<const float4_t*>(st_m2(c)); L.b1 = *reinterpret_cast<const float4_t*>(st_m2(c) + 4);
        load_steps(i0, L.s0, L.s1);
        L.e = *reinterpret_cast<const half8_t*>(p.ema + i0);
        if (i0 < oc.n_mlp) { L.gm0 = *reinterpret_cast<const float4_t*>(p.gmlp + i0); L.gm1 = *reinterpret_cast<const float4_t*>(p.gmlp + i0 + 4); }
    };
    Pre early; bool early_issued = false;
    if constexpr (ONE) {
        const uint32_t extra0 = nx.cand_blocks + nx.pos_blocks;
        if (vblock >= extra0) { const uint32_t ce = (vblock - extra0) * blockDim.x + threadIdx.x; if (ce < (oc.n_params >> 3)) { issue(ce, early);
                early_issued = true; } }
    }
    const uint32_t n_valid = st->n_valid, step = st->step;
    const bool eager = DENSE && (ONE || !(lazy_below != 0u && st->n_scatter_now <= lazy_below));
    const uint32_t extra = nx.cand_blocks + nx.pos_blocks;
    const bool cand_block = vblock < extra;
    if (vblock < nx.cand_blocks) gen_candidate(nx.b, nx.ds, nx.oc, st->n_boxes, st->iter + 1u, vblock * blockDim.x + threadIdx.x);
    else if (cand_block) {
        __shared__ PointsLds plds;
        const uint32_t nwords = nx.oc.R >> 6, nv = points_prefix(plds, nx.b.mask, nwords);
        if (vblock == 0 && threadIdx.x == 0) st_next->n_valid_pre = nv;
#if defined(MON_OPT_ABLATE) && (MON_OPT_ABLATE & 4)
        if (false)
#else
        if (nv != 0u)
#endif
            for (uint32_t s = vblock * blockDim.x + threadIdx.x; s < nx.oc.R * 32u; s += nx.pos_blocks * blockDim.x) {
                if constexpr (LIVE) points_sample<true>(plds, nx.b, nx.oc, st->iter + 1u, nv, nwords, s, reinterpret_cast<float4_t*>(nx.x_all), nx.live);
                else points_sample<false>(plds, nx.b, nx.oc, st->iter + 1u, nv, nwords, s, reinterpret_cast<float4_t*>(nx.x_all));
            }
    }
    const uint32_t bid = vblock - extra, nblk = gridDim.x - extra;
    const float lr0 = st->lr;
    const uint32_t cur = step + 1u;
    const float d = oc.ema_decay;
    const float deb_old = st->ema_deb_old, deb_new = st->ema_deb_new;
    if (vblock == 0 && threadIdx.x == 0) {
        DevState& nxs = *st_next;
        nxs.iter = st->iter + 1u; nxs.n_valid = n_valid; nxs.loss_sum = st->loss_sum;
        { const uint32_t tot = st->n_scatter_now; nxs.n_scatter_last = tot; nxs.n_scatter_total = st->n_scatter_total + tot; }
        uint32_t nstep = step;
        if (n_valid != 0u) {
            nstep = cur; nxs.skipped = st->skipped;
            nxs.lr = ((int)cur >= oc.decay_start && oc.decay_interval > 0 && ((int)cur - oc.decay_start) % oc.decay_interval == 0) ? lr0 * oc.decay_base : lr0;
        } else { nxs.skipped = st->skipped + 1u; nxs.lr = lr0; }
        nxs.step = nstep;
        nxs.ema_deb_old = 1.f - (float)pow((double)d, (double)nstep); nxs.ema_deb_new = 1.f / (1.f - (float)pow((double)d, (double)(nstep + 1u)));
    }
    const bool pow2_scale = (__float_as_uint(oc.loss_scale) & 0x007fffffu) == 0u && oc.loss_scale > 0.f;
    const float inv_scale = 1.0f / oc.loss_scale;
    auto unscale = [&](float g) { return pow2_scale ? g * inv_scale : g / oc.loss_scale; };
    if (n_valid != 0u && !cand_block) {
        const uint32_t n_chunks = oc.n_params >> 3, c_stride = nblk * blockDim.x, c_first = bid * blockDim.x + threadIdx.x;
        half8_t nx_g, nx_w, nx_e;
        auto prefetch = [&](uint32_t cn) {
            if (!DENSE && cn < n_chunks && (cn << 3) >= oc.n_mlp) {
                const uint32_t in0 = cn << 3;
                nx_g = *reinterpret_cast<const half8_t*>(p.ggrid + (in0 - oc.n_mlp));
                if (!LAZY) { nx_w = *reinterpret_cast<const half8_t*>(p.half + in0); nx_e = *reinterpret_cast<const half8_t*>(p.ema + in0); }
            }
        };
        auto update_chunk = [&](uint32_t c, bool pre, const half8_t& cur_g, const half8_t& cur_w, const half8_t& cur_e,
                const Pre* L = nullptr) __attribute__((always_inline)) {
            const uint32_t i0 = c << 3;
            const bool is_matrix = i0 < oc.n_mlp;
            float g[8]; bool any = false;
            uint32_t lvl_off = 0u, lvl_end = p.sl.entry_offset[1];
            float4_t w0, w1, a0, a1, b0, b1; uint4 s0, s1;
            if (L) { w0 = L->w0; w1 = L->w1; a0 = L->a0; a1 = L->a1; b0 = L->b0; b1 = L->b1; s0 = uint4{ L->s0[0], L->s0[1], L->s0[2], L->s0[3] };
                s1 = uint4{ L->s1[0], L->s1[1], L->s1[2], L->s1[3] }; }
            else if (eager) {
                w0 = *reinterpret_cast<const float4_t*>(st_master(c)); w1 = *reinterpret_cast<const float4_t*>(st_master(c) + 4);
                a0 = *reinterpret_cast<const float4_t*>(st_m1(c)); a1 = *reinterpret_cast<const float4_t*>(st_m1(c) + 4);
                b0 = *reinterpret_cast<const float4_t*>(st_m2(c)); b1 = *reinterpret_cast<const float4_t*>(st_m2(c) + 4);
                { u32x4 t0, t1; load_steps(i0, t0, t1); s0 = uint4{ t0[0], t0[1], t0[2], t0[3] }; s1 = uint4{ t1[0], t1[1], t1[2], t1[3] }; }
            }
            const bool lazy_chunk = LAZY && !is_matrix;
            half8_t ema_in;
            if (L) ema_in = L->e;
            else if (!lazy_chunk) ema_in = pre ? cur_e : *reinterpret_cast<const half8_t*>(p.ema + i0);
            if (is_matrix) {
#pragma unroll
                for (int j = 0; j < 8; ++j) {
                    const uint32_t i = i0 + j;
                    const float gs = L ? (j < 4 ? L->gm0[j & 3] : L->gm1[j & 3]) : p.gmlp[i]; p.gmlp[i] = 0.f;
                    g[j] = unscale(gs);
                }
                any = true;
            } else {
#pragma unroll
                for (int j = 0; j < 8; ++j) g[j] = 0.f;
                if (!DENSE) {
                    half8_t* gp = reinterpret_cast<half8_t*>(p.ggrid + (i0 - oc.n_mlp));
                    const half8_t gh = pre ? cur_g : *reinterpret_cast<const half8_t*>(p.ggrid + (i0 - oc.n_mlp));
                    bool anyg = false;
#pragma unroll
                    for (int j = 0; j < 8; ++j) { g[j] = (float)gh[j]; anyg |= (float)gh[j] != 0.f; }
                    if (anyg) { half8_t z;
#pragma unroll
                        for (int j = 0; j < 8; ++j) z[j] = (half_t)0.f;
                        *gp = z; }
                }
                uint32_t n_part = 0;
                if (p.gpart) {
                    const uint32_t e0 = (i0 - oc.n_mlp) >> 1; int lvl = 0;
#pragma unroll
                    for (int l = 1; l < kMaxLevels; ++l) { const bool in = e0 >= p.sl.entry_offset[l]; lvl += in ? 1 : 0;
                        lvl_off = in ? p.sl.entry_offset[l] : lvl_off; lvl_end = in ? p.sl.entry_offset[l + 1] : lvl_end; }
                    n_part = p.sl.P[lvl];
                }
                const uint16_t* pp = p.gpart + ((i0 - oc.n_mlp) >> 2);
                const size_t plane = p.part_stride >> 2;
                auto quad = [&](uint32_t q, float (&v)[8]) {
#pragma unroll
                    for (int f = 0; f < 2; ++f)
#pragma unroll
                        for (int b = 0; b < 2; ++b) {
                            const half2_t h = *reinterpret_cast<const half2_t*>(pp + ((size_t)(q * 2u + (uint32_t)f) * 2u + (uint32_t)b) * plane);
                            v[2 * b + f] = (float)h.x; v[2 * (2 + b) + f] = (float)h.y;
                        }
                };
                uint32_t q = 0;
#if defined(MON_OPT_ABLATE) && (MON_OPT_ABLATE & 2)
                for (int j = 0; j < 8; ++j) g[j] = 1e-3f;
                n_part = 0;
#endif
                for (; q + 2 <= n_part; q += 2) {
                    float va[8], vb[8]; quad(q, va); quad(q + 1u, vb);
#pragma unroll
                    for (int j = 0; j < 8; ++j) g[j] += va[j] + vb[j];
                }
                for (; q < n_part; ++q) {
                    float va[8]; quad(q, va);
#pragma unroll
                    for (int j = 0; j < 8; ++j) g[j] += va[j];
                }
#pragma unroll
                for (int j = 0; j < 8; ++j) { any |= g[j] != 0.f; g[j] = unscale(g[j]); }
            }
            if (lazy_chunk && !any) return;
            half8_t wh;
            if (eager) {
                const float wm[8] = { w0[0], w0[1], w0[2], w0[3], w1[0], w1[1], w1[2], w1[3] };
#pragma unroll
                for (int j = 0; j < 8; ++j) wh[j] = (half_t)wm[j];
            } else wh = (pre && !LAZY) ? cur_w : *reinterpret_cast<const half8_t*>(p.half + i0);
            if (lazy_chunk) {
                ema_in = *reinterpret_cast<const half8_t*>(p.ema + i0);
                const uint32_t last = *ema_step_of(c), k = (cur - 1u) - last;
                if (k) ema_catch_up(ema_in, wh, last, k, oc.log2_decay);
                *ema_step_of(c) = cur;
            }
            if (any) {
                if (!eager) {
                    w0 = *reinterpret_cast<const float4_t*>(st_master(c)); w1 = *reinterpret_cast<const float4_t*>(st_master(c) + 4);
                    a0 = *reinterpret_cast<const float4_t*>(st_m1(c)); a1 = *reinterpret_cast<const float4_t*>(st_m1(c) + 4);
                    b0 = *reinterpret_cast<const float4_t*>(st_m2(c)); b1 = *reinterpret_cast<const float4_t*>(st_m2(c) + 4);
                    { u32x4 t0, t1; load_steps(i0, t0, t1); s0 = uint4{ t0[0], t0[1], t0[2], t0[3] }; s1 = uint4{ t1[0], t1[1], t1[2], t1[3] }; }
                }
                float w[8] = { w0[0], w0[1], w0[2], w0[3], w1[0], w1[1], w1[2], w1[3] };
                float m1[8] = { a0[0], a0[1], a0[2], a0[3], a1[0], a1[1], a1[2], a1[3] };
                float m2[8] = { b0[0], b0[1], b0[2], b0[3], b1[0], b1[1], b1[2], b1[3] };
                uint32_t sc[8] = { s0.x, s0.y, s0.z, s0.w, s1.x, s1.y, s1.z, s1.w };
#pragma unroll
                for (int j = 0; j < 8; ++j) {
                    float gj = g[j];
                    if (is_matrix) gj += oc.l2_reg * w[j];
                    else if (gj == 0.f) continue;
#if defined(MON_OPT_ABLATE) && (MON_OPT_ABLATE & 1)
                    m1[j] += gj; m2[j] += gj; sc[j] += 1u; w[j] -= 1e-6f * gj;
#else
                    w[j] = adam_update(gj, w[j], m1[j], m2[j], sc[j], lr0, oc, step_cap);
#endif
                    wh[j] = (half_t)w[j];
                }
                state_store<!LAZY>(float4_t{ w[0], w[1], w[2], w[3] }, reinterpret_cast<float4_t*>(st_master(c)));
                state_store<!LAZY>(float4_t{ w[4], w[5], w[6], w[7] }, reinterpret_cast<float4_t*>(st_master(c) + 4));
                state_store<!LAZY>(float4_t{ m1[0], m1[1], m1[2], m1[3] }, reinterpret_cast<float4_t*>(st_m1(c)));
                state_store<!LAZY>(float4_t{ m1[4], m1[5], m1[6], m1[7] }, reinterpret_cast<float4_t*>(st_m1(c) + 4));
                state_store<!LAZY>(float4_t{ m2[0], m2[1], m2[2], m2[3] }, reinterpret_cast<float4_t*>(st_m2(c)));
                state_store<!LAZY>(float4_t{ m2[4], m2[5], m2[6], m2[7] }, reinterpret_cast<float4_t*>(st_m2(c) + 4));
                typedef uint32_t u4v __attribute__((ext_vector_type(4)));
                if (p.steps16 || prec) state_store<!LAZY>(u4v{ sc[0] | (sc[1] << 16), sc[2] | (sc[3] << 16), sc[4] | (sc[5] << 16), sc[6] | (sc[7] << 16) },
                        reinterpret_cast<u4v*>(st_steps16(c)));
                else { state_store<!LAZY>(u4v{ sc[0], sc[1], sc[2], sc[3] }, reinterpret_cast<u4v*>(p.steps + i0));
                    state_store<!LAZY>(u4v{ sc[4], sc[5], sc[6], sc[7] }, reinterpret_cast<u4v*>(p.steps + i0 + 4)); }
                policy_store<kSpHalf>(wh, reinterpret_cast<half8_t*>(p.half + i0));
#if defined(MON_OPT_ABLATE) && (MON_OPT_ABLATE & 8)
                if (false) {
#else
                if (p.half_tiles && !is_matrix) {
#endif
                    const uint32_t e0 = (i0 - oc.n_mlp) >> 1, size = lvl_end - lvl_off, e_rel = e0 - lvl_off;
                    if (size <= kEncWholeMax) policy_store<kSpTiles>(wh, reinterpret_cast<half8_t*>(p.half_tiles + 2u * (size_t)e0));
                    else {
                        const size_t s0 = lvl_off + (e_rel >> 1);
                        policy_store<kSpTiles>(half4_t{ wh[0], wh[1], wh[4], wh[5] }, reinterpret_cast<half4_t*>(p.half_tiles + 2u * s0));
                        policy_store<kSpTiles>(half4_t{ wh[2], wh[3], wh[6], wh[7] }, reinterpret_cast<half4_t*>(p.half_tiles + 2u * (s0 + (size >> 1))));
                    }
                }
                if (is_matrix && nx.frag_image) {
#pragma unroll
                    for (int j = 0; j < 8; ++j) { int sl[2]; const int ns = frag_slots(nx.fd, (int)(i0 + j), sl);
                        for (int q = 0; q < ns; ++q) policy_store<kSpFrag>((half_t)wh[j], reinterpret_cast<half_t*>(nx.frag_image) + sl[q]); }
                }
            }
            half8_t* ep = reinterpret_cast<half8_t*>(p.ema + i0);
            half8_t e = ema_in;
#pragma unroll
            for (int j = 0; j < 8; ++j) e[j] = (half_t)((((float)e[j] * d) * deb_old + (float)wh[j] * (1.f - d)) * deb_new);
            policy_store<kSpEma>(e, ep);
        };
        if constexpr (LAZY) {
            constexpr uint32_t kQueueCap = 2048;
            __shared__ uint32_t queue[4][kQueueCap];
            const uint32_t wave = threadIdx.x >> 6, lane = threadIdx.x & 63u; uint32_t qn = 0;
            const half8_t none{};
            if (p.touched) {
                const uint32_t w_end = (n_chunks + 3u) >> 2; uint32_t* flags = reinterpret_cast<uint32_t*>(p.touched);
                constexpr uint32_t kFlagPre = 8;
                const uint32_t wf0 = (p.first_flag_chunk >> 2) + c_first - lane; uint32_t fpre[kFlagPre];
#pragma unroll
                for (uint32_t k = 0; k < kFlagPre; ++k) { const uint32_t w = wf0 + k * c_stride + lane; fpre[k] = (w < w_end) ? flags[w] : 0u; }
                for (uint32_t c = c_first; c < p.first_flag_chunk; c += c_stride) update_chunk(c, false, none, none, none);
                uint32_t trip = 0;
                for (uint32_t w0 = wf0; w0 < w_end; w0 += c_stride, ++trip) {
                    const uint32_t w = w0 + lane; uint32_t f = 0u;
                    if (trip < kFlagPre) {
#pragma unroll
                        for (uint32_t k = 0; k < kFlagPre; ++k) f = (trip == k) ? fpre[k] : f;
                    } else if (w < w_end) f = flags[w];
                    if (f) flags[w] = 0u;
                    uint32_t before = 0u, total = 0u;
#pragma unroll
                    for (uint32_t j = 0; j < 4u; ++j) {
                        const unsigned long long tm = __ballot(((f >> (8u * j)) & 0xffu) != 0u);
                        before += (uint32_t)__popcll(tm & ((1ull << lane) - 1ull)); total += (uint32_t)__popcll(tm);
                    }
                    if (total == 0u) continue;
                    uint32_t pos = qn + before; qn += total;
#pragma unroll
                    for (uint32_t j = 0; j < 4u; ++j) {
                        if (((f >> (8u * j)) & 0xffu) == 0u) continue;
                        const uint32_t c = 4u * w + j;
                        if (pos < kQueueCap) queue[wave][pos] = c; else update_chunk(c, false, none, none, none);
                        ++pos;
                    }
                }
            } else {
            prefetch(c_first);
            for (uint32_t c0 = c_first - lane; c0 < n_chunks; c0 += c_stride) {
                const uint32_t c = c0 + lane; const bool valid = c < n_chunks;
                const half8_t cur_g = nx_g; prefetch(c + c_stride);
                bool direct = false, touched = false;
                if (valid) {
                    const uint32_t i0 = c << 3;
                    if (i0 < oc.n_mlp) direct = true;
                    else {
                        const uint32_t e0 = (i0 - oc.n_mlp) >> 1; int lvl = 0;
#pragma unroll
                        for (int l = 1; l < kMaxLevels; ++l) lvl += (e0 >= p.sl.entry_offset[l]) ? 1 : 0;
                        if (p.gpart && p.sl.P[lvl]) direct = true;
                        else { const uint4 gb = __builtin_bit_cast(uint4, cur_g); touched = ((gb.x | gb.y | gb.z | gb.w) & 0x7fff7fffu) != 0u; }
                    }
                }
                const unsigned long long tm = __ballot(touched);
                const uint32_t pos = qn + (uint32_t)__popcll(tm & ((1ull << lane) - 1ull));
                if (touched) { if (pos < kQueueCap) queue[wave][pos] = c; else direct = true; }
                qn += (uint32_t)__popcll(tm);
                if (direct) update_chunk(c, false, none, none, none);
            }
            }
            if (qn > kQueueCap) qn = kQueueCap;
            const auto update_queued = [&](uint32_t c) __attribute__((always_inline)) {
                const uint32_t i0 = c << 3;
                half8_t* gp = reinterpret_cast<half8_t*>(p.ggrid + (i0 - oc.n_mlp));
                const half8_t gh = *gp; half8_t e = *reinterpret_cast<const half8_t*>(p.ema + i0);
                const uint32_t last = *ema_step_of(c);
                const float4_t w0 = *reinterpret_cast<const float4_t*>(st_master(c)), w1 = *reinterpret_cast<const float4_t*>(st_master(c) + 4);
                const float4_t a0 = *reinterpret_cast<const float4_t*>(st_m1(c)), a1 = *reinterpret_cast<const float4_t*>(st_m1(c) + 4);
                const float4_t b0 = *reinterpret_cast<const float4_t*>(st_m2(c)), b1 = *reinterpret_cast<const float4_t*>(st_m2(c) + 4);
                u32x4 t0, t1; load_steps(i0, t0, t1);
                float g[8]; bool any = false;
#pragma unroll
                for (int j = 0; j < 8; ++j) { g[j] = (float)gh[j]; any |= g[j] != 0.f; }
                if (!any) return;
                { half8_t z;
#pragma unroll
                  for (int j = 0; j < 8; ++j) z[j] = (half_t)0.f;
                  *gp = z; }
#pragma unroll
                for (int j = 0; j < 8; ++j) g[j] = unscale(g[j]);
                float w[8] = { w0[0], w0[1], w0[2], w0[3], w1[0], w1[1], w1[2], w1[3] };
                half8_t wh;
#pragma unroll
                for (int j = 0; j < 8; ++j) wh[j] = (half_t)w[j];
                const uint32_t k = (cur - 1u) - last;
                if (k) ema_catch_up(e, wh, last, k, oc.log2_decay);
                *ema_step_of(c) = cur;
                float m1[8] = { a0[0], a0[1], a0[2], a0[3], a1[0], a1[1], a1[2], a1[3] };
                float m2[8] = { b0[0], b0[1], b0[2], b0[3], b1[0], b1[1], b1[2], b1[3] };
                uint32_t sc[8] = { t0[0], t0[1], t0[2], t0[3], t1[0], t1[1], t1[2], t1[3] };
#pragma unroll
                for (int j = 0; j < 8; ++j) {
                    if (g[j] == 0.f) continue;
                    w[j] = adam_update(g[j], w[j], m1[j], m2[j], sc[j], lr0, oc, step_cap);
                    wh[j] = (half_t)w[j];
                }
                state_store<false>(float4_t{ w[0], w[1], w[2], w[3] }, reinterpret_cast<float4_t*>(st_master(c)));
                state_store<false>(float4_t{ w[4], w[5], w[6], w[7] }, reinterpret_cast<float4_t*>(st_master(c) + 4));
                state_store<false>(float4_t{ m1[0], m1[1], m1[2], m1[3] }, reinterpret_cast<float4_t*>(st_m1(c)));
                state_store<false>(float4_t{ m1[4], m1[5], m1[6], m1[7] }, reinterpret_cast<float4_t*>(st_m1(c) + 4));
                state_store<false>(float4_t{ m2[0], m2[1], m2[2], m2[3] }, reinterpret_cast<float4_t*>(st_m2(c)));
                state_store<false>(float4_t{ m2[4], m2[5], m2[6], m2[7] }, reinterpret_cast<float4_t*>(st_m2(c) + 4));
                typedef uint32_t u4v __attribute__((ext_vector_type(4)));
                if (p.steps16 || prec) state_store<false>(u4v{ sc[0] | (sc[1] << 16), sc[2] | (sc[3] << 16), sc[4] | (sc[5] << 16), sc[6] | (sc[7] << 16) },
                        reinterpret_cast<u4v*>(st_steps16(c)));
                else { state_store<false>(u4v{ sc[0], sc[1], sc[2], sc[3] }, reinterpret_cast<u4v*>(p.steps + i0));
                    state_store<false>(u4v{ sc[4], sc[5], sc[6], sc[7] }, reinterpret_cast<u4v*>(p.steps + i0 + 4)); }
                *reinterpret_cast<half8_t*>(p.half + i0) = wh;
#pragma unroll
                for (int j = 0; j < 8; ++j) e[j] = (half_t)((((float)e[j] * d) * deb_old + (float)wh[j] * (1.f - d)) * deb_new);
                *reinterpret_cast<half8_t*>(p.ema + i0) = e;
            };
            for (uint32_t q0 = 0; q0 < qn; q0 += 64u) if (q0 + lane < qn) update_queued(queue[wave][q0 + lane]);
        } else if (eager) {
            const half8_t none{};
            const uint32_t c0 = c_first, c1 = c_first + c_stride;
            if constexpr (ONE) {
                if (c0 < n_chunks) { if (!early_issued) issue(c0, early); update_chunk(c0, false, none, none, none, &early); }
            } else if (c0 < n_chunks) {
                Pre A, B2; const bool two = c1 < n_chunks;
                issue(c0, A); if (two) issue(c1, B2);
                update_chunk(c0, false, none, none, none, &A);
                if (two) update_chunk(c1, false, none, none, none, &B2);
                for (uint32_t c = c1 + c_stride; c < n_chunks; c += c_stride) update_chunk(c, false, none, none, none);
            }
        } else {
            prefetch(c_first);
            for (uint32_t c = c_first; c < n_chunks; c += c_stride) {
                const bool pre = !DENSE && (c << 3) >= oc.n_mlp;
                const half8_t cur_g = nx_g, cur_w = nx_w, cur_e = nx_e;
                prefetch(c + c_stride);
                update_chunk(c, pre, cur_g, cur_w, cur_e);
            }
        }
    }
}

__global__ void __launch_bounds__(256) k_reduce_partials(const float* __restrict__ partials, uint32_t n_partials, uint32_t stride, uint32_t n_cols, FragDims fd,
                                                         float* __restrict__ gmlp, DevState* __restrict__ st) {
    if (st->n_valid == 0u) return;
    __shared__ float4_t red[256];
    const uint32_t c4 = threadIdx.x & 3u, sub = threadIdx.x >> 2;
    const uint32_t p0 = blockIdx.x * 16u + c4 * 4u;
    float4_t acc = { 0.f, 0.f, 0.f, 0.f };
    if (p0 < n_cols + 4u) {
        for (uint32_t k = sub; k < n_partials; k += 64u) acc += *reinterpret_cast<const float4_t*>(partials + (size_t)k * stride + p0);
    }
    red[threadIdx.x] = acc;
    __syncthreads();
    for (int off = 128; off >= 4; off >>= 1) { if ((int)threadIdx.x < off) red[threadIdx.x] += red[threadIdx.x + off]; __syncthreads(); }
    if (threadIdx.x < 4u) {
        const float4_t v = red[threadIdx.x];
#pragma unroll
        for (int j = 0; j < 4; ++j) { const uint32_t pi = p0 + j; if (pi < n_cols) { const int prm = acc_param(fd, (int)pi); if (prm >= 0) gmlp[prm] = v[j];
                } else if (pi == n_cols) st->loss_sum = v[j]; }
    }
}

void launch_reduce_partials(hipStream_t s, const float* partials, uint32_t n_partials, const NetDims& nd, float* gmlp, DevState* st) {
    const uint32_t n_cols = fused_partial_cols(nd);
    hipLaunchKernelGGL(k_reduce_partials, dim3((n_cols + 1 + 15) / 16), dim3(256), 0, s, partials, n_partials, n_cols + 64u, n_cols, FragDims{ nd.Epad, nd.W,
            nd.NH, nd.L }, gmlp, st);
}

__global__ void __launch_bounds__(256) k_ema_finalize(ParamPtrs p, OptimConst oc, const DevState* __restrict__ st) {
    const uint32_t done = st->step, n_chunks = oc.n_params >> 3;
    for (uint32_t c = (oc.n_mlp >> 3) + blockIdx.x * blockDim.x + threadIdx.x; c < n_chunks; c += gridDim.x * blockDim.x) {
        uint32_t* lp = p.rec ? reinterpret_cast<uint32_t*>(p.rec + 32u * (size_t)c + 28u) : p.ema_step + c;
        const uint32_t last = *lp;
        if (last >= done) continue;
        half8_t e = *reinterpret_cast<const half8_t*>(p.ema + (c << 3)); const half8_t w = *reinterpret_cast<const half8_t*>(p.half + (c << 3));
        ema_catch_up(e, w, last, done - last, oc.log2_decay);
        *reinterpret_cast<half8_t*>(p.ema + (c << 3)) = e; *lp = done;
    }
}
void launch_ema_finalize(hipStream_t s, const ParamPtrs& p, const OptimConst& oc, const DevState* st) {
    hipLaunchKernelGGL(k_ema_finalize, dim3(2048), dim3(256), 0, s, p, oc, st);
}

__global__ void __launch_bounds__(256) k_master_to_half(const float* __restrict__ master, uint16_t* __restrict__ half, uint32_t n) {
    for (uint32_t i = blockIdx.x * blockDim.x + threadIdx.x; i < n; i += gridDim.x * blockDim.x) { const half_t h = (half_t)master[i];
        half[i] = __builtin_bit_cast(uint16_t, h); }
}
__global__ void __launch_bounds__(256) k_copy_params(const uint4* __restrict__ src, uint4* __restrict__ dst, uint32_t n16,
        const uint16_t* __restrict__ src_tail, uint16_t* __restrict__ dst_tail, uint32_t n_tail) {
    for (uint32_t i = blockIdx.x * blockDim.x + threadIdx.x; i < n16; i += gridDim.x * blockDim.x) dst[i] = src[i];
    if (blockIdx.x == 0 && threadIdx.x < n_tail) dst_tail[threadIdx.x] = src_tail[threadIdx.x];
}
void launch_copy_params(hipStream_t s, const uint16_t* src, uint16_t* dst, uint32_t n) {
    const uint32_t n16 = n / 8u, tail = n - n16 * 8u;
    const uint32_t blocks = n16 >= 512u * 256u ? 512u : (n16 + 255u) / 256u + (n16 == 0u ? 1u : 0u);
    hipLaunchKernelGGL(k_copy_params, dim3(blocks), dim3(256), 0, s, reinterpret_cast<const uint4*>(src), reinterpret_cast<uint4*>(dst), n16,
            src + (size_t)n16 * 8u, dst + (size_t)n16 * 8u, tail);
}
__global__ void __launch_bounds__(256) k_state_unpack(const float* __restrict__ rec, int which, uint32_t* __restrict__ dst, uint32_t n) {
    for (uint32_t i = blockIdx.x * blockDim.x + threadIdx.x; i < n; i += gridDim.x * blockDim.x) {
        const float* r = rec + 32u * (size_t)(i >> 3);
        dst[i] = which < 3 ? __builtin_bit_cast(uint32_t, r[8 * which + (i & 7u)]) : (uint32_t)reinterpret_cast<const uint16_t*>(r + 24)[i & 7u];
    }
}
__global__ void __launch_bounds__(256) k_state_pack_master(const float* __restrict__ master, float* __restrict__ rec, uint32_t n) {
    for (uint32_t i = blockIdx.x * blockDim.x + threadIdx.x; i < n; i += gridDim.x * blockDim.x) rec[32u * (size_t)(i >> 3) + (i & 7u)] = master[i];
}
void launch_state_unpack(hipStream_t s, const float* rec, int which, void* dst, uint32_t n) {
    hipLaunchKernelGGL(k_state_unpack, dim3(2048), dim3(256), 0, s, rec, which, static_cast<uint32_t*>(dst), n);
}
void launch_state_pack_master(hipStream_t s, const float* master, float* rec, uint32_t n) {
    hipLaunchKernelGGL(k_state_pack_master, dim3(2048), dim3(256), 0, s, master, rec, n);
}
typedef uint32_t ck_u32x4 __attribute__((ext_vector_type(4)));
__global__ void __launch_bounds__(256) k_state_unpack_range(const float* __restrict__ rec, int which, ck_u32x4* __restrict__ dst, uint32_t first_chunk,
        uint32_t n_chunks) {
    const uint32_t n_pieces = 2u * n_chunks;
    for (uint32_t i = blockIdx.x * blockDim.x + threadIdx.x; i < n_pieces; i += gridDim.x * blockDim.x) {
        const float* r = rec + 32u * (size_t)(first_chunk + (i >> 1)) + 8u * (uint32_t)which + 4u * (i & 1u);
        dst[i] = *reinterpret_cast<const ck_u32x4*>(r);
    }
}
__global__ void __launch_bounds__(256) k_state_pack_range(float* __restrict__ rec, int which, const ck_u32x4* __restrict__ src, uint32_t first_chunk,
        uint32_t n_chunks) {
    const uint32_t n_pieces = 2u * n_chunks;
    for (uint32_t i = blockIdx.x * blockDim.x + threadIdx.x; i < n_pieces; i += gridDim.x * blockDim.x) {
        float* r = rec + 32u * (size_t)(first_chunk + (i >> 1)) + 8u * (uint32_t)which + 4u * (i & 1u);
        *reinterpret_cast<ck_u32x4*>(r) = src[i];
    }
}
__global__ void __launch_bounds__(256) k_steps_unpack_range(const ck_u32x4* __restrict__ base16, uint32_t stride16, ck_u32x4* __restrict__ dst,
        uint32_t first_chunk, uint32_t n_chunks) {
    for (uint32_t c = blockIdx.x * blockDim.x + threadIdx.x; c < n_chunks; c += gridDim.x * blockDim.x) {
        const ck_u32x4 v = base16[(size_t)(first_chunk + c) * stride16];
        dst[2u * c] = ck_u32x4{ v[0] & 0xffffu, v[0] >> 16, v[1] & 0xffffu, v[1] >> 16 };
        dst[2u * c + 1u] = ck_u32x4{ v[2] & 0xffffu, v[2] >> 16, v[3] & 0xffffu, v[3] >> 16 };
    }
}
__global__ void __launch_bounds__(256) k_steps_pack_range(ck_u32x4* __restrict__ base16, uint32_t stride16, const ck_u32x4* __restrict__ src,
        uint32_t first_chunk, uint32_t n_chunks) {
    for (uint32_t c = blockIdx.x * blockDim.x + threadIdx.x; c < n_chunks; c += gridDim.x * blockDim.x) {
        const ck_u32x4 a = src[2u * c], b = src[2u * c + 1u];
        const auto pk = [](uint32_t lo, uint32_t hi) -> uint32_t { return (lo < 65535u ? lo : 65535u) | ((hi < 65535u ? hi : 65535u) << 16); };
        base16[(size_t)(first_chunk + c) * stride16] = ck_u32x4{ pk(a[0], a[1]), pk(a[2], a[3]), pk(b[0], b[1]), pk(b[2], b[3]) };
    }
}
__global__ void __launch_bounds__(256) k_ema_step_unpack_range(const float* __restrict__ rec, uint32_t* __restrict__ dst, uint32_t first_chunk,
        uint32_t n_chunks) {
    const uint32_t n_quads = (n_chunks + 3u) >> 2;
    for (uint32_t q = blockIdx.x * blockDim.x + threadIdx.x; q < n_quads; q += gridDim.x * blockDim.x) {
        const uint32_t c = 4u * q; const uint32_t* w = reinterpret_cast<const uint32_t*>(rec) + 32u * (size_t)(first_chunk + c) + 28u;
        if (c + 4u <= n_chunks) reinterpret_cast<ck_u32x4*>(dst)[q] = ck_u32x4{ w[0], w[32], w[64], w[96] };
        else for (uint32_t j = 0; c + j < n_chunks; ++j) dst[c + j] = w[32u * j];
    }
}
__global__ void __launch_bounds__(256) k_ema_step_pack_range(float* __restrict__ rec, const uint32_t* __restrict__ src, uint32_t first_chunk,
        uint32_t n_chunks) {
    const uint32_t n_quads = (n_chunks + 3u) >> 2;
    for (uint32_t q = blockIdx.x * blockDim.x + threadIdx.x; q < n_quads; q += gridDim.x * blockDim.x) {
        const uint32_t c = 4u * q; uint32_t* w = reinterpret_cast<uint32_t*>(rec) + 32u * (size_t)(first_chunk + c) + 28u;
        if (c + 4u <= n_chunks) { const ck_u32x4 v = reinterpret_cast<const ck_u32x4*>(src)[q]; w[0] = v[0]; w[32] = v[1]; w[64] = v[2]; w[96] = v[3]; }
        else for (uint32_t j = 0; c + j < n_chunks; ++j) w[32u * j] = src[c + j];
    }
}
static uint32_t range_blocks(uint32_t lanes) { const uint32_t b = (lanes + 255u) / 256u; return b < 1u ? 1u : (b > 2048u ? 2048u : b); }
void launch_state_unpack_range(hipStream_t s, const float* rec, int which, void* dst, uint32_t first_chunk, uint32_t n_chunks) {
    if (n_chunks == 0u) return;
    if (which < 3) hipLaunchKernelGGL(k_state_unpack_range, dim3(range_blocks(2u * n_chunks)), dim3(256), 0, s, rec, which, static_cast<ck_u32x4*>(dst),
            first_chunk, n_chunks);
    else if (which == 3) hipLaunchKernelGGL(k_steps_unpack_range, dim3(range_blocks(n_chunks)), dim3(256), 0, s,
            reinterpret_cast<const ck_u32x4*>(rec + 24), 8u, static_cast<ck_u32x4*>(dst), first_chunk, n_chunks);
    else hipLaunchKernelGGL(k_ema_step_unpack_range, dim3(range_blocks((n_chunks + 3u) >> 2)), dim3(256), 0, s, rec, static_cast<uint32_t*>(dst), first_chunk,
            n_chunks);
}
void launch_state_pack_range(hipStream_t s, float* rec, int which, const void* src, uint32_t first_chunk, uint32_t n_chunks) {
    if (n_chunks == 0u) return;
    if (which < 3) hipLaunchKernelGGL(k_state_pack_range, dim3(range_blocks(2u * n_chunks)), dim3(256), 0, s, rec, which, static_cast<const ck_u32x4*>(src),
            first_chunk, n_chunks);
    else if (which == 3) hipLaunchKernelGGL(k_steps_pack_range, dim3(range_blocks(n_chunks)), dim3(256), 0, s, reinterpret_cast<ck_u32x4*>(rec + 24), 8u,
            static_cast<const ck_u32x4*>(src), first_chunk, n_chunks);
    else hipLaunchKernelGGL(k_ema_step_pack_range, dim3(range_blocks((n_chunks + 3u) >> 2)), dim3(256), 0, s, rec, static_cast<const uint32_t*>(src), first_chunk,
            n_chunks);
}
void launch_steps16_unpack_range(hipStream_t s, const uint16_t* steps16, void* dst, uint32_t first_chunk, uint32_t n_chunks) {
    if (n_chunks) hipLaunchKernelGGL(k_steps_unpack_range, dim3(range_blocks(n_chunks)), dim3(256), 0, s, reinterpret_cast<const ck_u32x4*>(steps16), 1u,
            static_cast<ck_u32x4*>(dst), first_chunk, n_chunks);
}
void launch_steps16_pack_range(hipStream_t s, uint16_t* steps16, const void* src, uint32_t first_chunk, uint32_t n_chunks) {
    if (n_chunks) hipLaunchKernelGGL(k_steps_pack_range, dim3(range_blocks(n_chunks)), dim3(256), 0, s, reinterpret_cast<ck_u32x4*>(steps16), 1u,
            static_cast<const ck_u32x4*>(src), first_chunk, n_chunks);
}
void launch_master_to_half(hipStream_t s, const float* master, uint16_t* half, uint32_t n) {
    hipLaunchKernelGGL(k_master_to_half, dim3(1024), dim3(256), 0, s, master, half, n);
}

void launch_optimizer(hipStream_t s, const ParamPtrs& p, const OptimConst& oc, const DevState* st, DevState* st_next, const OptimNext& nx,
        uint32_t lazy_below) {
    const uint32_t chunks = oc.n_params >> 3;
    uint32_t cap = chunks / (256u * 8u); if (cap < 1024u) cap = 1024u; if (cap > 2048u) cap = 2048u;
    uint32_t blocks = (chunks + 255) / 256; if (blocks > cap) blocks = cap; if (blocks < 1u) blocks = 1u;
    const dim3 grid(blocks + nx.cand_blocks + nx.pos_blocks); const bool live = nx.pos_blocks && nx.live.occ_bits;
#define MON_OPT_LAUNCH(D, L, O) do { if (live) hipLaunchKernelGGL((k_optimizer<D, L, O, true>), grid, dim3(256), 0, s, p, oc, st, st_next, nx, lazy_below); \
        else hipLaunchKernelGGL((k_optimizer<D, L, O, false>), grid, dim3(256), 0, s, p, oc, st, st_next, nx, lazy_below); } while (0)
    if (p.gpart && p.all_levels_dense) {
        if ((size_t)blocks * 256u >= chunks) MON_OPT_LAUNCH(true, false, true);
        else MON_OPT_LAUNCH(true, false, false);
    }
    else if (p.lazy) MON_OPT_LAUNCH(false, true, false);
    else MON_OPT_LAUNCH(false, false, false);
#undef MON_OPT_LAUNCH
}

}
```

ro-map_amd/csrc/model.cpp:

```cpp
#include <cmath>
#include <cstdarg>
#include <cstdio>
#include <cstdlib>
#include <algorithm>
#include <atomic>
#include <chrono>
#include <cstring>
#include <map>
#include <mutex>
#include <string>
#include <vector>
#include <dlfcn.h>
#include <unistd.h>
#include <zlib.h>
#include "model.h"
#include "xorwow.h"

namespace mon {

static thread_local std::string g_err;
void set_error(const char* fmt, ...) {
    char buf[1024]; va_list ap; va_start(ap, fmt); vsnprintf(buf, sizeof(buf), fmt, ap); va_end(ap); g_err = buf;
}
const char* last_error() { return g_err.c_str(); }
// ... 290 lines not shown
    InferShared* sh = static_cast<InferShared*>(d->upload); std::lock_guard<std::mutex> one(sh->mu);
    uint8_t* st_rgb = d->h_stage, *st_inst = st_rgb + px * 4; float* st_depth = reinterpret_cast<float*>(st_inst + ((px + 15) & ~(size_t)15));
    float* st_pose = st_depth + (d->use_depth ? px : 0);
    std::memcpy(st_rgb, rgb, px * (size_t)ch); std::memcpy(st_inst, inst, px); std::memcpy(st_pose, Twc, 64);
    launch_pack_frame(sh->stream, st_rgb, ch, ri, bi, st_inst, d->d_rgba + px * id, (uint32_t)px);
    if (d->use_depth) { std::memcpy(st_depth, depth, px * 4); launch_copy_from_host(sh->stream, st_depth, d->d_depth + px * id, (uint32_t)px); }
    launch_copy_from_host(sh->stream, st_pose, d->d_poses + 16 * (size_t)id, 16u);
    HIPCHECK(hipStreamSynchronize(sh->stream)); HIPCHECK(hipGetLastError());
    if (id + 1 > d->n_frames) d->n_frames = id + 1;
    d->present[id] = 1;
    return MON_OK;
}
int dataset_update_poses(Dataset* d, uint32_t first, uint32_t n, const float* Twc16s) {
    if (!d || !Twc16s || first + n > d->max_frames) {
        set_error("update_poses: frames %u..%u outside the dataset (%u frames)", first, first + n, d ? d->max_frames : 0u); return MON_ERR_ARG; }
    HIPCHECK(use_device(d->device));
    HIPCHECK(hipMemcpy(d->d_poses + 16 * (size_t)first, Twc16s, 64 * (size_t)n, hipMemcpyHostToDevice));
    return MON_OK;
}
int dataset_destroy(Dataset* d) {
    if (!d) return MON_OK;
    use_device(d->device);
    if (d->d_rgba) hipFree(d->d_rgba);
    if (d->d_depth) hipFree(d->d_depth);
    if (d->d_poses) hipFree(d->d_poses);
    if (d->h_stage) hipHostFree(d->h_stage);
    delete d; return MON_OK;
}

static std::mutex g_stream_mu; static std::map<int, std::vector<hipStream_t>> g_stream_pool;
static int stream_acquire(int device, hipStream_t* out) {
    { std::lock_guard<std::mutex> l(g_stream_mu); auto& v = g_stream_pool[device]; if (!v.empty()) { *out = v.back(); v.pop_back(); return MON_OK; } }
    HIPCHECK(hipStreamCreateWithFlags(out, hipStreamNonBlocking));
    return MON_OK;
}
static void stream_release(int device, hipStream_t s) { std::lock_guard<std::mutex> l(g_stream_mu); g_stream_pool[device].push_back(s); }
int stream_pool_reserve(int device, int n) {
    HIPCHECK(use_device(device));
    std::vector<hipStream_t> fresh;
    { std::lock_guard<std::mutex> l(g_stream_mu); n -= (int)g_stream_pool[device].size(); }
    int rc = MON_OK;
    for (int i = 0; i < n; ++i) {
        hipStream_t s; const hipError_t e = hipStreamCreateWithFlags(&s, hipStreamNonBlocking);
        if (e != hipSuccess) { set_error("hipStreamCreateWithFlags failed: %s", hipGetErrorString(e)); rc = MON_ERR_HIP; break; }
        fresh.push_back(s);
    }
    std::lock_guard<std::mutex> l(g_stream_mu); for (hipStream_t s : fresh) g_stream_pool[device].push_back(s);
    return rc;
}

struct InferState {
    InferShared* shared = nullptr;
    uint16_t* snap[2] = { nullptr, nullptr }; hipEvent_t ready[2] = { nullptr, nullptr }; uint32_t step_of[2] = { 0, 0 }; bool written[2] = { false, false };
    int latest = -1, readers[2] = { 0, 0 }; std::mutex mu;
    uint64_t epoch_of[2] = { 0, 0 };
    std::atomic<bool> wanted{ false }; std::chrono::steady_clock::time_point last_pub{};
    BatchPtrs rb{}; float *out_all = nullptr, *out_rgb = nullptr, *out_depth = nullptr, *out_mask = nullptr; size_t out_cap = 0; uint16_t* frag = nullptr;
    std::vector<void*> grown;
    RenderSkipSide rskip;
};

template <class T> static int dev_alloc(Model& m, T*& p, size_t n, bool zero = true) {
    void* q = nullptr; const size_t bytes = (n ? n : 1) * sizeof(T);
    HIPCHECK(hipMalloc(&q, bytes));
    if (zero) HIPCHECK(hipMemset(q, 0, bytes));
    m.allocs.push_back(q); p = (T*)q; return MON_OK;
}

static constexpr uint32_t kRenderChunkRays = 16384;

static int rskip_alloc(Model& m, RenderSkipSide& k) {
    if (k.d_grid) return MON_OK;
    int rc;
    if ((rc = dev_alloc(m, k.d_grid, kOccWords)) || (rc = dev_alloc(m, k.d_raw, kOccWords)) || (rc = dev_alloc(m, k.d_stats, 4))) return rc;
    HIPCHECK(hipHostMalloc((void**)&k.h_stats, 16, hipHostMallocDefault)); std::memset(k.h_stats, 0, 16);
    return MON_OK;
}
static const uint32_t* rskip_grid(Model& m, RenderSkipSide& k, hipStream_t s, float alpha, const uint16_t* prm, uint64_t epoch, uint16_t* frag) {
    if (!k.d_grid) return nullptr;
    if (!k.pinned && (!k.built || k.epoch != epoch || k.alpha != alpha)) {
        if (alpha <= 0.f) {
            (void)hipMemsetAsync(k.d_raw, 0xff, kOccWords * 4, s); (void)hipMemsetAsync(k.d_grid, 0xff, kOccWords * 4, s);
        } else {
            double diag2 = 0.0; for (int a = 0; a < 3; ++a) diag2 += (double)(m.oc.aabb.mx[a] - m.oc.aabb.mn[a]) * (m.oc.aabb.mx[a] - m.oc.aabb.mn[a]);
            const double dt = std::max(std::sqrt(diag2) / (2.0 * m.oc.S), 1e-9);
            launch_occupancy_update(s, m.lf, m.nd, prm, m.oc, frag, (float)std::log(-std::log1p(-(double)alpha) / dt), k.d_raw, k.d_grid);
        }
        k.built = true; k.epoch = epoch; k.alpha = alpha; ++k.builds;
    }
    return k.d_grid;
}
static RenderSkipArgs rskip_begin(Model& m, RenderSkipSide& k, hipStream_t s, bool on, float alpha, const uint16_t* prm, uint64_t epoch, uint16_t* frag) {
    k.active = false;
    if (!on || !k.d_grid) return RenderSkipArgs{};
    rskip_grid(m, k, s, alpha, prm, epoch, frag);
    (void)hipMemsetAsync(k.d_stats, 0, 16, s);
    k.active = true;
    RenderSkipArgs a; a.bits = k.d_grid; a.stats = k.d_stats; return a;
}
static void rskip_read(hipStream_t s, RenderSkipSide& k) { if (k.active) launch_copy_params(s, reinterpret_cast<const uint16_t*>(k.d_stats),
        reinterpret_cast<uint16_t*>(k.h_stats), 4u); }
static void rskip_end(RenderSkipSide& k) { if (k.active) { k.samples_live = k.h_stats[0]; k.samples_in_box = k.h_stats[1]; } }

static int upload_master(Model& m, const float* master) {
    const size_t n = m.n_params;
    if (!m.P.rec) {
        HIPCHECK(hipMemcpy(m.P.master, master, n * 4, hipMemcpyHostToDevice));
        launch_master_to_half(m.train_stream, m.P.master, m.P.half, (uint32_t)n);
        return MON_OK;
    }
    float* tmp = nullptr; HIPCHECK(hipMalloc((void**)&tmp, n * 4));
    hipError_t e = hipMemcpy(tmp, master, n * 4, hipMemcpyHostToDevice);
    if (e == hipSuccess) { launch_state_pack_master(m.train_stream, tmp, m.P.rec, (uint32_t)n);
        launch_master_to_half(m.train_stream, tmp, m.P.half, (uint32_t)n); e = hipStreamSynchronize(m.train_stream); }
    (void)hipFree(tmp); HIPCHECK(e); return MON_OK;
}
MeshState* mesh_state_create(int device);
static bool steps16_exact(const mon_config& cfg) {
    const double kSteps16Bound = std::ldexp(1.0, -29);
    return kSteps16 && std::pow((double)cfg.beta1, 65535.0) < kSteps16Bound && std::pow((double)cfg.beta2, 65535.0) < kSteps16Bound;
}
static int model_init(Model& m, Dataset* ds, const mon_config& cfg, int class_id, const float* Tow, const float* amin, const float* amax,
        bool init_params = true) {
    m.ds = ds; m.cfg = cfg; m.device = ds->device;
    int rc = level_table_build(cfg, m.lt, m.nd, m.n_grid);
    if (rc) return rc;
    m.n_params = m.nd.n_mlp + m.n_grid;
    level_fast_build(m.lt, m.nd, m.lf);
    {
        int shift = 0; while (shift < 23 && 128.0f * (float)(1u << shift) < cfg.loss_scale) ++shift;
        m.lf.fix_scale = 16777216.0f / (float)(1u << shift); m.lf.fix_clamp = 100.0f * (float)(1u << shift);
    }
    HIPCHECK(use_device(m.device));
    std::memcpy(m.oc.Tow.m, Tow, 64);
    for (int a = 0; a < 3; ++a) { m.oc.aabb.mn[a] = amin[a]; m.oc.aabb.mx[a] = amax[a]; }
    m.oc.instance_id = (uint32_t)(uint8_t)class_id;
    m.oc.R = (uint32_t)cfg.rays_per_batch; m.oc.S = (uint32_t)cfg.n_samples; m.oc.use_depth = cfg.use_depth && ds->use_depth;
    m.oc.sample_seed = cfg.sample_seed; m.oc.loss_scale = cfg.loss_scale;
    m.n_bins = kDefaultScatterBins;
    m.opt = OptimConst{ cfg.beta1, cfg.beta2, cfg.epsilon, cfg.l2_reg, cfg.ema_decay, cfg.loss_scale, cfg.decay_base, std::log2(cfg.beta1),
            std::log2(cfg.beta2), std::log2(cfg.ema_decay), cfg.decay_start, cfg.decay_interval, m.nd.n_mlp, m.n_params };
    { const int rcs = stream_acquire(m.device, &m.own_stream); if (rcs) return rcs; }
    m.train_stream = m.own_stream; m.lanes = lanes_get(m.device); m.lanes->objects.fetch_add(1);
    const size_t n = m.n_params;
    const bool steps16 = steps16_exact(cfg);
    m.lazy_ema = m.n_grid > (8u << 20);
    const bool records = m.lazy_ema && steps16 && kStateRecords && (n & 7u) == 0u;
    if (records) { if ((rc = dev_alloc(m, m.P.rec, 4 * n))) return rc; }
    else if ((rc = dev_alloc(m, m.P.master, n, false)) || (rc = dev_alloc(m, m.P.m1, n)) || (rc = dev_alloc(m, m.P.m2, n)) ||
             (rc = steps16 ? dev_alloc(m, m.P.steps16, n + 8) : dev_alloc(m, m.P.steps, n))) return rc;
    if ((rc = dev_alloc(m, m.P.half, n, false)) || (rc = dev_alloc(m, m.P.ema, n)) || (rc = records ? MON_OK : dev_alloc(m, m.d_ema_step, n / 8 + 1)) ||
        
        (rc = dev_alloc(m, m.P.gmlp, m.nd.n_mlp)) || (rc = dev_alloc(m, m.P.ggrid, m.n_grid))) return rc;
    if (init_params) {
        std::vector<float> master; init_params_host(cfg, m.nd, m.n_params, master);
        const int urc = upload_master(m, master.data()); if (urc) return urc;
    }
    const uint32_t R = m.oc.R, S = m.oc.S;
    m.ws_rays = R > kRenderChunkRays ? R : kRenderChunkRays;
    const bool fused_inference = fused_supported(m.nd, S, R) && options().backend != 0;
    const uint32_t Btrain = R * S, Brender = fused_inference ? Btrain : kRenderChunkRays * 2 * S;
    m.ws_samples = Btrain > Brender ? Btrain : Brender;
    BatchPtrs& B = m.B;
    if ((rc = dev_alloc(m, B.cand_o, 3 * (size_t)R)) || (rc = dev_alloc(m, B.cand_d, 3 * (size_t)R)) || (rc = dev_alloc(m, B.cand_dn, R)) ||
        (rc = dev_alloc(m, B.cand_t0, R)) || (rc = dev_alloc(m, B.cand_t1, R)) || (rc = dev_alloc(m, B.cand_depth, R)) ||
        (rc = dev_alloc(m, B.cand_rgba, R)) || (rc = dev_alloc(m, B.mask, (R + 63) / 64 + 64)) ||
        (rc = dev_alloc(m, B.ray_o, 3 * (size_t)m.ws_rays)) || (rc = dev_alloc(m, B.ray_d, 3 * (size_t)m.ws_rays))
                || (rc = dev_alloc(m, B.ray_dn, m.ws_rays)) ||
        (rc = dev_alloc(m, B.ray_t0, m.ws_rays)) || (rc = dev_alloc(m, B.ray_t1, m.ws_rays)) || (rc = dev_alloc(m, B.target, 3 * (size_t)R)) ||
        (rc = dev_alloc(m, B.target_depth, R)) || (rc = dev_alloc(m, B.bgcol, 3 * (size_t)R)) || (rc = dev_alloc(m, B.ray_flag, m.ws_rays)) ||
        (rc = dev_alloc(m, B.pts, 3 * (size_t)m.ws_samples)) || (rc = dev_alloc(m, B.tdist, m.ws_samples)) ||
        (rc = dev_alloc(m, B.E, (size_t)m.ws_samples * m.nd.Epad)) || (rc = dev_alloc(m, B.O, (size_t)m.ws_samples * kOut)) ||
        (rc = dev_alloc(m, B.Hid, (size_t)Btrain * m.nd.W * m.nd.NH)) || (rc = dev_alloc(m, B.dO, (size_t)Btrain * kOut)) ||
        (rc = dev_alloc(m, B.dHid, (size_t)Btrain * m.nd.W * m.nd.NH)) || (rc = dev_alloc(m, B.dE, (size_t)Btrain * m.nd.Epad)) ||
        (rc = dev_alloc(m, B.rgb_ray, 3 * (size_t)R)) || (rc = dev_alloc(m, B.depth_ray, R)) || (rc = dev_alloc(m, B.mask_ray, R))
                || (rc = dev_alloc(m, B.loss_ray, R)) ||
        (rc = dev_alloc(m, m.d_state, 2)) || (rc = dev_alloc(m, m.d_dw_partials, (size_t)(fused_partial_cols(m.nd) + 64) * kMaxFusedGrid)) ||
        (rc = dev_alloc(m, m.d_out_all, 5 * (size_t)kRenderChunkRays))) return rc;
    m.out_cap = kRenderChunkRays;
    if (rng_stream_mode(cfg.rng_flags)) {
        m.xw_lanes = rng_xorwow_lanes(cfg.rng_flags); m.xw_flavour = rng_stream_mode(cfg.rng_flags) == 2 ? kXorwowRocrand : kXorwowCurand;
        std::vector<XorwowState> st; xorwow_lane_states(0ull , m.xw_flavour, m.xw_lanes, st);
        XorwowState *d_a = nullptr, *d_b = nullptr, *d_c = nullptr;
        if ((rc = dev_alloc(m, d_a, m.xw_lanes, false)) || (rc = dev_alloc(m, d_b, m.xw_lanes, false)) || (rc = dev_alloc(m, d_c, m.xw_lanes, false)) ||
            (rc = dev_alloc(m, m.d_xw, 2 * (size_t)(5 + S) * R))) return rc;
        HIPCHECK(hipMemcpy(d_a, st.data(), sizeof(XorwowState) * m.xw_lanes, hipMemcpyHostToDevice));
        HIPCHECK(hipMemcpy(d_c, st.data(), sizeof(XorwowState) * m.xw_lanes, hipMemcpyHostToDevice));
        m.d_xw_states = d_a; m.d_xw_render_states = d_b; m.d_xw_render_init = d_c;
        m.oc.xw[0] = m.d_xw; m.oc.xw[1] = m.d_xw + (size_t)(5 + S) * R;
    }
    if (fused_supported(m.nd, S, m.oc.R)) {
        if ((rc = dev_alloc(m, m.d_frag_train, 64 * 512)) || (rc = dev_alloc(m, m.d_frag_render, 64 * 512))) return rc;
        m.lds_mask = scatter_plan(m.lt, m.nd, m.scatter);
        {
            int last = -1; for (int l = 0; l < m.nd.L; ++l) if ((m.lds_mask >> l) & 1u) last = l;
            m.part_halves = last < 0 ? 0u : ((2u * m.lt.offset[last + 1] + 15u) & ~15u);
        }
        if (m.lds_mask && ((rc = dev_alloc(m, m.d_de_soa, (size_t)m.nd.L * Btrain * 2)) || (rc = dev_alloc(m, m.d_x_soa, 4 * (size_t)Btrain)) ||
                           (rc = dev_alloc(m, m.d_gpart, (size_t)m.scatter.max_P * m.part_halves)))) return rc;
        const size_t big_bytes = m.lds_mask ? big_scatter_workspace_bytes(m.lt, m.nd, m.lds_mask, Btrain) : 0;
        const uint32_t big_switch = (uint32_t)options().big_switch;
        if (big_bytes && big_switch) { if ((rc = dev_alloc(m, m.d_big_ws, big_bytes))) return rc; m.big_switch = big_switch; }
        const bool tiles_pay = options().lds_encode >= 2 || Btrain >= 98304u;
        if (options().lds_encode && tiles_pay && m.lds_mask == ((1u << m.nd.L) - 1u) && encode_tiles_supported(m.lt, m.nd)) {
            if ((rc = dev_alloc(m, B.ray_rec, 12 * (size_t)R))) return rc;
            m.B_alt = B;
            if ((rc = dev_alloc(m, m.B_alt.cand_o, 3 * (size_t)R)) || (rc = dev_alloc(m, m.B_alt.cand_d, 3 * (size_t)R))
                    || (rc = dev_alloc(m, m.B_alt.cand_dn, R)) ||
                (rc = dev_alloc(m, m.B_alt.cand_t0, R)) || (rc = dev_alloc(m, m.B_alt.cand_t1, R)) || (rc = dev_alloc(m, m.B_alt.cand_depth, R)) ||
                (rc = dev_alloc(m, m.B_alt.cand_rgba, R)) || (rc = dev_alloc(m, m.B_alt.mask, (R + 63) / 64 + 64))) return rc;
            if ((rc = dev_alloc(m, m.d_x_all, 4 * (size_t)Btrain)) || (rc = dev_alloc(m, m.d_e_soa, (size_t)m.nd.L * Btrain * 2))
                    || (rc = dev_alloc(m, m.d_half_tiles, (size_t)m.n_grid + 64))) return rc;
            encode_tiles_setup_device();
        }
        const bool flags_on = kTouchedFlags;
        if (flags_on && m.lazy_ema && m.lds_mask && m.lds_mask != ((m.nd.L >= 32) ? 0xffffffffu : ((1u << m.nd.L) - 1u))
                && (rc = dev_alloc(m, m.d_touched, (m.n_params >> 3) + 16))) return rc;
    }
    if (!fused_supported(m.nd, S, m.oc.R) && (Btrain & 31u) == 0u) {
        if ((rc = dev_alloc(m, m.d_layers_T, layers_workspace_halves(m.nd, Btrain)))) return rc;
    }
    if (fused_supported(m.nd, S, m.oc.R)) { }
    else if (S == 32u && !m.lazy_ema) {
        ScatterLevels plan{}; const uint32_t mask = scatter_plan(m.lt, m.nd, plan);
        if (mask == ((1u << m.nd.L) - 1u) && (R % kDefaultScatterBins) == 0u) {
            m.scatter = plan; m.part_halves = (2u * m.lt.offset[m.nd.L] + 15u) & ~15u;
            if ((rc = dev_alloc(m, m.d_de_soa, (size_t)m.nd.L * Btrain * 2)) || (rc = dev_alloc(m, m.d_x_soa, 4 * (size_t)Btrain)) ||
                (rc = dev_alloc(m, m.d_gpart, (size_t)m.scatter.max_P * m.part_halves))) return rc;
            m.hybrid_scatter = true;
            const bool tiles_pay_b0 = options().lds_encode >= 2 || Btrain >= 98304u;
            if (m.d_layers_T && options().lds_encode && tiles_pay_b0 && encode_tiles_supported(m.lt, m.nd)) {
                if ((rc = dev_alloc(m, m.d_x_all, 4 * (size_t)Btrain)) || (rc = dev_alloc(m, m.d_e_soa, (size_t)m.nd.L * Btrain * 2))
                        || (rc = dev_alloc(m, m.d_half_tiles, (size_t)m.n_grid + 64))) return rc;
                encode_tiles_setup_device();
            }
        }
    }
    if (cfg.occupancy_skip && fused_supported(m.nd, S, m.oc.R)) {
        constexpr size_t words = (size_t)kOccRes * kOccRes * kOccRes / 32;
        if ((rc = dev_alloc(m, m.d_occ, words, false)) || (rc = dev_alloc(m, m.d_occ_tmp, words, false))
                || (rc = dev_alloc(m, m.d_frag_occ, 64 * 512))) return rc;
        HIPCHECK(hipMemset(m.d_occ, 0xff, words * 4));
        float diag2 = 0.f; for (int a = 0; a < 3; ++a) diag2 += (amax[a] - amin[a]) * (amax[a] - amin[a]);
        const float dt = std::sqrt(diag2) / (float)S;
        m.occ_raw_threshold = std::log(1e-3f / std::max(dt, 1e-6f));
        const uint32_t spw_l = encode_tiles_spw(Btrain), parts_l = (Btrain + spw_l - 1u) / spw_l, blocks_l = (Btrain + 255u) / 256u;
        if (m.d_e_soa && Btrain % 256u == 0u && parts_l <= kLiveMaxParts && ((blocks_l + parts_l - 1u) / parts_l) * 256u <= spw_l) {
            if ((rc = dev_alloc(m, m.d_live_idx, Btrain)) || (rc = dev_alloc(m, m.d_live_cnt, 2u * kLiveMaxParts * kLiveCntStride))) return rc;
        }
    }
    m.boxes_cap = 1024;
    if ((rc = dev_alloc(m, m.d_boxes, m.boxes_cap))) return rc;
    B.boxes = m.d_boxes; m.B_alt.boxes = m.d_boxes;
    m.h_state = DevState{}; m.h_state.lr = cfg.learning_rate;
    m.h_state.ema_deb_old = 0.0f; m.h_state.ema_deb_new = 1.0f / (1.0f - (float)std::pow((double)cfg.ema_decay, 1.0));
    m.d_state_next = m.d_state + 1;
    HIPCHECK(hipMemcpy(m.d_state, &m.h_state, sizeof(DevState), hipMemcpyHostToDevice));
    HIPCHECK(hipMemcpy(m.d_state_next, &m.h_state, sizeof(DevState), hipMemcpyHostToDevice));
    HIPCHECK(hipHostMalloc((void**)&m.h_state_pinned, sizeof(DevState), hipHostMallocDefault));
    m.backend = fused_supported(m.nd, S, m.oc.R) ? 1 : 0;
    if (options().backend >= 0) m.backend = options().backend ? (fused_supported(m.nd, S, m.oc.R) ? 1 : 0) : 0;
    m.mesh = mesh_state_create(m.device);
    m.tile_ok = fused_supported(m.nd, S, m.oc.R) && !m.lazy_ema && tile_render_supported(m.lt, m.nd);
    m.weights_epoch = next_weights_epoch();
    if (m.tile_ok) { tile_ws_object_born(m.device); m.tile_counted = true; }
    if (m.backend == 1 && !m.lazy_ema && !m.d_xw) {
        InferState* is = new InferState(); m.infer = is;
        if ((rc = infer_shared_get(m.device, (size_t)ds->K.W * (size_t)ds->K.H, &is->shared))) return rc;
        for (int k = 0; k < 2; ++k) { if ((rc = dev_alloc(m, is->snap[k], n, false))) return rc;
            HIPCHECK(hipEventCreateWithFlags(&is->ready[k], hipEventDisableTiming)); }
        is->rb = m.B;
        if ((rc = dev_alloc(m, is->rb.ray_o, 3 * (size_t)kRenderChunkRays)) || (rc = dev_alloc(m, is->rb.ray_d, 3 * (size_t)kRenderChunkRays))
                || (rc = dev_alloc(m, is->rb.ray_dn, kRenderChunkRays)) ||
            (rc = dev_alloc(m, is->rb.ray_t0, kRenderChunkRays)) || (rc = dev_alloc(m, is->rb.ray_t1, kRenderChunkRays))
                    || (rc = dev_alloc(m, is->rb.ray_flag, kRenderChunkRays)) ||
            (rc = dev_alloc(m, is->out_all, 5 * (size_t)kRenderChunkRays)) || (rc = dev_alloc(m, is->frag, 64 * 512))) return rc;
        is->out_cap = kRenderChunkRays;
    }
    HIPCHECK(hipStreamSynchronize(nullptr)); HIPCHECK(hipStreamSynchronize(m.train_stream));
    return MON_OK;
}

static int publish_snapshot(Model& m, bool force = true) {
    InferState* is = m.infer; if (!is) return MON_OK;
    const auto now = std::chrono::steady_clock::now();
    if (!force && is->latest >= 0 && !is->wanted.load() && now - is->last_pub < std::chrono::milliseconds(10)) return MON_OK;
    int w;
    {   std::lock_guard<std::mutex> l(is->mu); w = is->latest == 0 ? 1 : 0;
        if (is->readers[w] > 0) return MON_OK;
        is->written[w] = false; }
    const uint16_t* src = (m.h_state.step > 0) ? m.P.ema : m.P.half;
    launch_copy_params(m.train_stream, src, is->snap[w], m.n_params);
    HIPCHECK(hipEventRecord(is->ready[w], m.train_stream));
    { std::lock_guard<std::mutex> l(is->mu); is->step_of[w] = m.h_state.step; is->epoch_of[w] = next_weights_epoch(); is->written[w] = true; is->latest = w; }
    is->wanted.store(false); is->last_pub = now;
    return MON_OK;
}

int model_destroy(Model* mp);
static int config_check(const mon_config& cfg) {
    if (cfg.rays_per_batch < 64 || (cfg.rays_per_batch % 64) != 0 || cfg.n_samples < 1 || cfg.n_samples > 64) {
        set_error("rays_per_batch must be a multiple of 64, n_samples 1..64"); return MON_ERR_ARG; }
    if ((cfg.rng_flags & 3u) == 3u || (cfg.rng_flags & ~0xffff0013u) != 0u || (cfg.rng_flags >> 16) > 1024u) {
        set_error("rng_flags: bits 0-1 = 0 (counter RNG) | 1 (XORWOW, cuRAND flavour) | 2 (XORWOW, rocRAND flavour), bit 4 = tcnn init order, "
                  "bits 16-31 = XORWOW lanes / 1024 (at most 1024)");
        return MON_ERR_ARG;
// ... 1400 lines not shown
```

ro-map_amd/csrc/model.h:

```cpp
#pragma once
#include <hip/hip_runtime.h>
#include <stdint.h>
#include <atomic>
#include <mutex>
#include <string>
#include <vector>
#include "../../include/mon_core.h"
#include "device_common.h"
#include "frag_layout.h"

namespace mon {

struct DevState {
    uint32_t step;
    uint32_t iter;
    uint32_t n_valid;
    uint32_t n_boxes;
    float lr;
    float loss_sum;
    uint32_t n_valid_pre;
    uint32_t skipped;
    uint32_t n_scatter_now;
    float ema_deb_even_old, ema_deb_even_new;
    uint32_t reserved_bins[13];
    uint32_t n_scatter_last;
    uint32_t n_scatter_total;
    float ema_deb_old, ema_deb_new;
    uint32_t n_scatter[2 * kMaxScatterBins * kScatterCounterStride];
};

struct DatasetPtrs {
    const uint32_t* rgba;
    const float* depth;
    const float* poses;
    Intrinsics K;
};

struct ObjectConst {
    Mat4 Tow; Aabb aabb;
    uint32_t instance_id; uint32_t R; uint32_t S; int use_depth;
    uint64_t sample_seed;
    float loss_scale;
    const float* xw[2]; const float* xw_render;
};
__device__ __forceinline__ float batch_rand(const ObjectConst& oc, uint32_t stream, uint32_t step, uint32_t idx) {
    if (oc.xw[0]) return oc.xw[step & 1u][(stream == kStreamXY ? 0u : stream == kStreamColor ? 2u * oc.R : 5u * oc.R) + idx];
    return rand01(oc.sample_seed, stream, step, idx);
}
__device__ __forceinline__ float render_rand(const ObjectConst& oc, uint32_t idx) {
    return oc.xw_render ? oc.xw_render[idx] : rand01(oc.sample_seed, kStreamRender, 0u, idx); }

struct BatchPtrs {
    const mon_frame_bbox* boxes;
    float *cand_o, *cand_d, *cand_dn, *cand_t0, *cand_t1, *cand_depth; uint32_t* cand_rgba; unsigned long long* mask;
    float *ray_o, *ray_d, *ray_dn, *ray_t0, *ray_t1, *target, *target_depth, *bgcol; uint8_t* ray_flag;
    float *pts, *tdist;
    uint16_t *E, *Hid, *O, *dO, *dHid, *dE;
    float *rgb_ray, *depth_ray, *mask_ray, *loss_ray;
    float* ray_rec;
};

struct ScatterLevels { uint32_t entry_offset[kMaxLevels + 1]; uint8_t P[kMaxLevels]; uint8_t level[kMaxLevels]; uint32_t n_levels; uint32_t max_P; };

struct ParamPtrs {
    float* master; uint16_t* half; uint16_t* ema; float* m1; float* m2; uint32_t* steps;
    uint16_t* steps16;
    float* rec;
    float* gmlp;
    uint16_t* ggrid;
    const uint16_t* gpart; uint32_t part_stride;
    ScatterLevels sl;
    uint32_t* ema_step; int lazy;
    uint8_t* touched; uint32_t first_flag_chunk;
    int all_levels_dense;
    uint16_t* half_tiles;
};

constexpr uint32_t kEncWholeMax = 163840u / 4u;
__host__ __device__ inline uint32_t tile_slot(uint32_t off, uint32_t size, uint32_t e_rel) {
    return size <= kEncWholeMax ? off + e_rel : off + (e_rel & 1u) * (size >> 1) + (e_rel >> 1); }

struct OptimConst {
    float beta1, beta2, epsilon, l2_reg, ema_decay, loss_scale, decay_base, log2_beta1, log2_beta2, log2_decay;
    int decay_start, decay_interval;
    uint32_t n_mlp, n_params;
};

constexpr uint32_t kLiveMaxParts = 64, kLiveCntStride = 16;
struct LiveArgs { const uint32_t* occ_bits; uint32_t* idx; uint32_t* cnt; uint32_t spw, n_parts; };

struct OptimNext { uint32_t cand_blocks; uint16_t* frag_image; FragDims fd; BatchPtrs b; DatasetPtrs ds; ObjectConst oc;
                   uint32_t pos_blocks; float* x_all; LiveArgs live; };

enum {
    MON_BUF_MASTER = 0, MON_BUF_HALF = 1, MON_BUF_EMA = 2, MON_BUF_M1 = 3, MON_BUF_M2 = 4, MON_BUF_STEPS = 5,
    MON_BUF_GMLP = 6, MON_BUF_GGRID_H = 9, MON_BUF_PTS = 10, MON_BUF_TDIST = 11, MON_BUF_E = 12, MON_BUF_HID = 13,
    MON_BUF_O = 14, MON_BUF_DO = 15, MON_BUF_DHID = 16, MON_BUF_DE = 17, MON_BUF_RGB_RAY = 18, MON_BUF_DEPTH_RAY = 19,
    MON_BUF_MASK_RAY = 20, MON_BUF_LOSS_RAY = 21, MON_BUF_RAY_O = 22, MON_BUF_RAY_D = 23, MON_BUF_RAY_T0 = 24,
    MON_BUF_RAY_T1 = 25, MON_BUF_TARGET = 26, MON_BUF_TARGET_DEPTH = 27, MON_BUF_BGCOL = 28, MON_BUF_RAY_FLAG = 29,
    MON_BUF_RAY_DN = 31, MON_BUF_MASK = 32, MON_BUF_STATE = 33,
    MON_BUF_FRAG_TRAIN = 34,
    MON_BUF_FRAG_REF = 35,
    MON_BUF_X_ALL = 36,
    MON_BUF_E_SOA = 37,
    MON_BUF_HALF_TILES = 38,
    MON_BUF_LIVE_CNT = 40,
    MON_BUF_GGRID_F32 = 39
};

struct Options {
    std::atomic<long> backend{ -1 }, use_graph{ 0 }, big_switch{ 16384 }, lds_encode{ 1 }, train_lanes{ 2 }, roctx{ 0 }, step_variant{ 0 },
         keep_zero_samples{ 0 },
         tile_render{ 1 };
    std::atomic<long> offline_outer{ 10 }, offline_inner{ 500 };
#ifdef MON_OVERLAP_PROBE
    std::atomic<long> overlap{ 0 }, enc_lds_kb{ 0 };
#endif
};
#ifdef MON_VARIANT_STEPS32
constexpr bool kSteps16 = false;
#else
constexpr bool kSteps16 = true;
#endif
#ifdef MON_VARIANT_ARRAYS
constexpr bool kStateRecords = false;
#else
constexpr bool kStateRecords = true;
#endif
#ifdef MON_VARIANT_NO_FLAGS
constexpr bool kTouchedFlags = false;
#else
constexpr bool kTouchedFlags = true;
#endif
constexpr int kLaneChunk = 16;
constexpr long kOnlineSliceMin = 2;
Options& options();
int option_set(const char* name, long value);
int option_get(const char* name, long* value);

hipError_t use_device(int logical_device);
int set_logical_devices(int n);

void launch_gen_candidates(hipStream_t s, const BatchPtrs& b, const DatasetPtrs& ds, const ObjectConst& oc, const DevState* st);
void launch_build_rays(hipStream_t s, const BatchPtrs& b, const ObjectConst& oc, DevState* st);
void launch_gen_samples(hipStream_t s, const BatchPtrs& b, const ObjectConst& oc, const DevState* st, uint32_t S, uint32_t n_samples, uint32_t stream_id,
        uint32_t idx_base, int render, float* x4_or_null = nullptr);
void launch_render_rays(hipStream_t s, const BatchPtrs& b, const Intrinsics& K, const ObjectConst& oc, mon_frame_bbox box, const Mat4& pose, int pose_is_Toc,
        uint32_t pix0, uint32_t n);
void launch_grid_points(hipStream_t s, float* pts, int rx, int ry, int rz, uint32_t p0, uint32_t n);

void launch_encode(hipStream_t s, const LevelTable& lt, const NetDims& nd, const uint16_t* params, const float* pts, uint16_t* E, uint32_t n,
        const DevState* st_or_null);
void launch_mlp_forward(hipStream_t s, const NetDims& nd, const uint16_t* params, const uint16_t* E, uint16_t* Hid_or_null, uint16_t* O, uint32_t n,
        const DevState* st_or_null);
void launch_mlp_backward(hipStream_t s, const NetDims& nd, const uint16_t* params, const uint16_t* Hid, const uint16_t* dO, uint16_t* dHid, uint16_t* dE,
        uint32_t n, const DevState* st);
void launch_weight_grads(hipStream_t s, const NetDims& nd, const uint16_t* E, const uint16_t* Hid, const uint16_t* dHid, const uint16_t* dO, float* gmlp,
        uint32_t n, const DevState* st);
void launch_grid_backward(hipStream_t s, const LevelTable& lt, const NetDims& nd, const float* pts, const uint16_t* dE, uint16_t* ggrid, uint32_t n,
        const DevState* st);

size_t layers_workspace_halves(const NetDims& nd, uint32_t n);
bool launch_mlp_forward_layers(hipStream_t s, const NetDims& nd, const uint16_t* params, const uint16_t* E, uint16_t* Hid, uint16_t* O, uint32_t n,
        const DevState* st_or_null, uint16_t* ws_T_or_null,
        const uint16_t* e_soa_or_null = nullptr, uint16_t* E_out = nullptr,
        bool keep_rowmajor = true);
bool launch_mlp_backward_layers(hipStream_t s, const NetDims& nd, const uint16_t* params, const uint16_t* Hid, const uint16_t* dO, uint16_t* dHid, uint16_t* dE,
        uint32_t n, const DevState* st, uint16_t* ws_T,
        bool keep_rowmajor = true ,
        const struct BinsOut* bins = nullptr);
struct BinsOut { uint16_t* de_soa; float* x_soa; const float* pts; uint32_t n_bins; float clampv; DevState* st; };
void launch_weight_grads_layers(hipStream_t s, const NetDims& nd, float* gmlp, uint32_t n, const DevState* st, uint16_t* ws_T);
struct Model;
void mlp_forward_inference(Model& m, hipStream_t s, const uint16_t* params, const uint16_t* E, uint16_t* O, uint32_t n);

void launch_composite_grad(hipStream_t s, const BatchPtrs& b, const ObjectConst& oc, DevState* st);
void launch_loss_sum(hipStream_t s, const float* loss_ray, uint32_t R, DevState* st);
void launch_composite_render(hipStream_t s, const BatchPtrs& b, uint32_t S, uint32_t n_rays, float* rgb, float* depth, float* mask);
void launch_extract_density(hipStream_t s, const uint16_t* O, float* out, uint32_t n);
void launch_master_to_half(hipStream_t s, const float* master, uint16_t* half, uint32_t n);
void launch_state_unpack(hipStream_t s, const float* rec, int which, void* dst, uint32_t n);
void launch_state_pack_master(hipStream_t s, const float* master, float* rec, uint32_t n);
void launch_state_unpack_range(hipStream_t s, const float* rec, int which, void* dst, uint32_t first_chunk, uint32_t n_chunks);
void launch_state_pack_range(hipStream_t s, float* rec, int which, const void* src, uint32_t first_chunk, uint32_t n_chunks);
void launch_steps16_unpack_range(hipStream_t s, const uint16_t* steps16, void* dst, uint32_t first_chunk, uint32_t n_chunks);
void launch_steps16_pack_range(hipStream_t s, uint16_t* steps16, const void* src, uint32_t first_chunk, uint32_t n_chunks);
void launch_copy_params(hipStream_t s, const uint16_t* src, uint16_t* dst, uint32_t n);
void model_leave_lane(struct Model& m);
void launch_pack_frame(hipStream_t s, const uint8_t* rgb, int ch, int ri, int bi, const uint8_t* inst, uint32_t* dst, uint32_t px);
void launch_copy_from_host(hipStream_t s, const void* src, void* dst, uint32_t n_words);

void launch_step_compaction(hipStream_t s, const BatchPtrs& b, const ObjectConst& oc, DevState* st, uint32_t* steps, float* pts_compacted);

void launch_optimizer(hipStream_t s, const ParamPtrs& p, const OptimConst& oc, const DevState* st, DevState* st_next, const OptimNext& nx, uint32_t lazy_below);
void launch_ema_finalize(hipStream_t s, const ParamPtrs& p, const OptimConst& oc, const DevState* st);
void launch_reduce_partials(hipStream_t s, const float* partials, uint32_t n_partials, const NetDims& nd, float* gmlp, DevState* st);
uint32_t fused_partial_cols(const NetDims& nd);

constexpr uint32_t kMaxFusedGrid = 512;
bool fused_supported(const NetDims& nd, uint32_t S, uint32_t R);
uint32_t fused_train_grid(const NetDims& nd, uint32_t R);
void launch_fused_train(hipStream_t s, const LevelFast& lt, const NetDims& nd, const ParamPtrs& p, const BatchPtrs& b, const ObjectConst& oc, DevState* st,
        float* dw_partials, int debug_dump,
                        uint16_t* de_soa, float* x_soa, uint32_t lds_level_mask, uint16_t* frag_image, uint32_t big_switch, uint8_t* touched,
                                const uint32_t* occ_bits, uint32_t n_bins, const uint16_t* e_soa_or_null);
bool encode_tiles_supported(const LevelTable& lt, const NetDims& nd);
void encode_tiles_setup_device();
void launch_sample_points(hipStream_t s, const BatchPtrs& b, const ObjectConst& oc, DevState* st, float* x_all, const LiveArgs& live = LiveArgs{});
void launch_encode_tiles(hipStream_t s, const LevelFast& lf, const NetDims& nd, const uint16_t* half_tiles, const float* x_all, uint16_t* e_soa, uint32_t B,
        const DevState* st,
                         const BatchPtrs* b_next_or_null, const DatasetPtrs& ds, const ObjectConst& oc, uint32_t lds_bytes = 0, const LiveArgs& live = LiveArgs{});
uint32_t encode_tiles_spw(uint32_t B);
void launch_xorwow_fill(hipStream_t s, void* lane_states, uint32_t lanes, int flavour, uint32_t start_lane, float* out0, uint32_t n0, float* out1, uint32_t n1,
        float* out2, uint32_t n2);
void launch_build_tiles_image(hipStream_t s, const LevelFast& lf, const NetDims& nd, const uint16_t* params, uint16_t* half_tiles);
void launch_occupancy_update(hipStream_t s, const LevelFast& lt, const NetDims& nd, const uint16_t* params, const ObjectConst& oc, uint16_t* frag_image,
        float raw_threshold, uint32_t* tmp, uint32_t* bits);
uint32_t scatter_plan(const LevelTable& lt, const NetDims& nd, ScatterLevels& sl);
uint32_t scatter_level_mask(const LevelTable& lt, const NetDims& nd);
bool grid_scatter_sums_partials(const LevelTable& lt, const NetDims& nd);
void launch_grid_scatter(hipStream_t s, const LevelTable& lt, const LevelFast& lf, const NetDims& nd, const uint16_t* de_soa, const float* x_soa, uint32_t B,
        uint32_t n_bins, uint16_t* gpart, uint32_t part_stride_entries, DevState* st,
                         const float* partials_or_null, uint32_t n_partials, float* gmlp, DevState* st_next);
void launch_rows_to_bins(hipStream_t s, const LevelFast& lf, const NetDims& nd, const uint16_t* dE, const float* pts, uint32_t R, uint32_t S, uint32_t n_bins,
        uint16_t* de_soa, float* x_soa, DevState* st);
size_t big_scatter_workspace_bytes(const LevelTable& lt, const NetDims& nd, uint32_t lds_mask, uint32_t B);
void launch_big_scatter(hipStream_t s, const LevelTable& lt, const LevelFast& lf, const NetDims& nd, uint32_t lds_mask, const uint16_t* de_soa,
        const float* x_soa, uint32_t B,
                        uint32_t n_bins, const DevState* st, uint32_t big_switch, void* workspace, uint16_t* ggrid, uint8_t* touched_grid);
struct RenderSkipArgs {
    const uint32_t* bits = nullptr;
    uint32_t* stats = nullptr;
    uint32_t* job_bits = nullptr; uint32_t* idx = nullptr; uint32_t* cnt = nullptr; uint32_t spw = 0;
};
constexpr uint32_t kRenderListStride = 16;
void launch_fused_render(hipStream_t s, const LevelFast& lt, const NetDims& nd, const uint16_t* params, const BatchPtrs& b, const ObjectConst& oc,
        uint32_t n_rays, uint32_t idx_base, float* rgb, float* depth, float* mask, uint16_t* frag_image, int build_image,
        const RenderSkipArgs& skip = RenderSkipArgs{});
void launch_build_frag_image(hipStream_t s, const uint16_t* params, const NetDims& nd, uint16_t* image);
constexpr uint32_t kSceneListLen = 64, kSceneMaxLists = 256;
constexpr uint32_t scene_composite_lds(uint32_t n_lists) { return n_lists * (2u * kSceneListLen + 20u); }
void launch_fused_render_emit(hipStream_t s, const LevelFast& lt, const NetDims& nd, const uint16_t* params, const BatchPtrs& b, const ObjectConst& oc,
        uint32_t n_rays, uint32_t idx_base, float* t, float* attr, uint32_t* cnt, uint16_t* frag_image, int build_image, const uint32_t* skip_bits);
void launch_scene_composite(hipStream_t s, uint32_t n_rays, uint32_t n_lists, uint32_t cap, const float* t, const float* attr, const uint32_t* cnt,
        const float* dn, float* rgb, float* depth, float* opacity, int32_t* instance);
constexpr uint32_t kStreamPose = 4, kStreamPoseXY = 5;
constexpr uint32_t kPoseMaxGrid = 1024, kPoseMaxRays = 1u << 22;
struct PoseRayArgs {
    const mon_frame_bbox* boxes; const uint32_t* prefix;
    uint32_t n_obs, n_rays, total, drawn, iteration; uint64_t seed;
    DatasetPtrs ds; Aabb aabb; uint32_t instance_id; const float* pose; float4* rec;
};
struct PoseGradArgs {
    const float4* rec; uint32_t n_rays;
    uint64_t seed; uint32_t stream, step;
    float w_rgb, w_mask, w_depth, huber, inv_n;
    float* partials;
    float *dbg_x, *dbg_raw, *dbg_g;
};
struct PoseGradArgsLW : PoseGradArgs { const float* level_w; };
__attribute__((weak)) uint32_t pose_grad_grid(uint32_t n_rays);
__attribute__((weak)) void launch_pose_rays(hipStream_t s, const PoseRayArgs& a);
__attribute__((weak)) void launch_pose_grad(hipStream_t s, const LevelFast& lt, const NetDims& nd, const ObjectConst& oc, const uint16_t* params, uint16_t* frag_image,
        int build_image, const PoseGradArgs& p, const float* level_w);
__attribute__((weak)) void launch_pose_update(hipStream_t s, const float* partials, uint32_t n_parts, float inv_n, float* out, float* trace, uint32_t it, int step, float lr_t,
        float lr_r, float* pose, float* moments);
constexpr uint32_t kSceneLossParts = 4096;
constexpr uint32_t scene_composite_grad_lds(uint32_t n_lists) { return n_lists * (2u * kSceneListLen + 28u); }
struct SceneObjConst { float Tow[16]; Aabb aabb; uint32_t instance_id; uint32_t pad; };
struct ScenePoseRayArgs {
    const mon_frame_bbox* boxes; const uint32_t* prefix;
    uint32_t n_obs, n_rays, ray0, total, drawn, iteration; uint64_t seed;
    DatasetPtrs ds; const SceneObjConst* objs; uint32_t n_objs, cap; const float* pose;
    float4* rec; float* mstar; float4* ray;
};
struct ScenePoseObjArgs {
    const float4* rec; uint32_t n_rays, ray0;
    uint64_t seed; uint32_t stream, step;
    float* t; float4* attr; uint32_t* cnt;
    const float2* gw; const float4* grow; const float4* ray;
    float inv_n; float* partials;
    float* dbg;
    const float* level_w;
};
struct SceneCompGradArgs {
    uint32_t n_rays, n_lists, cap;
    const float* t; const float4* attr; const uint32_t* cnt;
    const float* mstar; const float4* ray;
    float w_rgb, w_mask, w_depth, huber;
    float2* gw; float4* grow; float* loss_part;
    float* out_W; float* out_D;
};
struct ScenePoseUpdateArgs {
    const float* partials; uint32_t n_objs, n_rows, row_stride;
    const float* loss_part; uint32_t n_loss_parts;
    const SceneObjConst* objs; float inv_n; float* out; uint32_t it; int step; float lr_t, lr_r; float* pose; float* moments;
};
__attribute__((weak)) void launch_scene_pose_rays(hipStream_t s, const ScenePoseRayArgs& a);
__attribute__((weak)) void launch_scene_pose_obj(hipStream_t s, const LevelFast& lt, const NetDims& nd, const ObjectConst& oc, const uint16_t* params, uint16_t* frag_image,
        int build_image, int backward, uint32_t grid, const ScenePoseObjArgs& p);
__attribute__((weak)) uint32_t scene_comp_grad_grid(uint32_t n_rays);
__attribute__((weak)) void launch_scene_composite_grad(hipStream_t s, const SceneCompGradArgs& a);
__attribute__((weak)) void launch_scene_pose_update(hipStream_t s, const ScenePoseUpdateArgs& a);
constexpr uint32_t kTileChunkJobs = 32768;
bool tile_render_supported(const LevelTable& lt, const NetDims& nd);
void launch_build_feat_image(hipStream_t s, const LevelFast& lf, const NetDims& nd, const uint16_t* params, uint16_t* image, uint32_t* zero_counter);
void launch_forward_frag_image(hipStream_t s, const NetDims& nd, const uint16_t* params, uint16_t* image);
void launch_render_rays_jobs(hipStream_t s, const Intrinsics& K, const ObjectConst& oc, mon_frame_bbox box, const Mat4& pose, int pose_is_Toc, uint32_t n_pix,
                             float* rec, uint32_t* count, uint32_t* next_count, float* rgb, float* depth, float* mask);
void launch_render_points(hipStream_t s, const ObjectConst& oc, const float* rec, const uint32_t* count, uint32_t job_base, uint32_t jobs_cap, float* x,
        const RenderSkipArgs& skip = RenderSkipArgs{});
uint32_t render_list_parts();
uint32_t render_list_spw(uint32_t cap);
void launch_grid_points4(hipStream_t s, float* x, int rx, int ry, int rz, uint32_t p0, uint32_t n);
void launch_mesh_warp4(hipStream_t s, const float* verts, float* x, uint32_t v0, uint32_t n, const Aabb& box);
void launch_encode_feat(hipStream_t s, const LevelFast& lf, const NetDims& nd, const uint16_t* image, const float* x, uint16_t* e, uint32_t cap,
                        uint32_t n_host, const uint32_t* count, uint32_t job_base, uint32_t jobs_cap, uint32_t spj,
                        const RenderSkipArgs& skip = RenderSkipArgs{});
void launch_tile_render(hipStream_t s, const NetDims& nd, const ObjectConst& oc, const uint16_t* frag_image, const float* rec, const uint32_t* count,
                        uint32_t job_base, uint32_t jobs_cap, const float* x, const uint16_t* e, uint32_t cap, uint32_t n_pix, float* rgb, float* depth,
                                float* mask, const RenderSkipArgs& skip = RenderSkipArgs{});
void launch_tile_points_mlp(hipStream_t s, const NetDims& nd, const uint16_t* frag_image, const uint16_t* e, uint32_t cap, uint32_t n_points, uint16_t* O);
void launch_candidates_and_frags(hipStream_t s, const BatchPtrs& b, const DatasetPtrs& ds, const ObjectConst& oc, const DevState* st, const uint16_t* params,
        const NetDims& nd, uint16_t* frag_image);
int selftest_mfma(int device, const uint16_t* A, const uint16_t* B, float* D);

struct Dataset {
    int device = 0; Intrinsics K{}; uint32_t max_frames = 0, n_frames = 0; bool use_depth = false;
    uint32_t* d_rgba = nullptr; float* d_depth = nullptr; float* d_poses = nullptr;
    std::vector<uint8_t> present;
    uint8_t* h_stage = nullptr; size_t stage_bytes = 0; void* upload = nullptr;
    DatasetPtrs ptrs() const { return DatasetPtrs{ d_rgba, d_depth, d_poses, K }; }
};

struct MeshState;
struct InferState;

struct RenderSkipSide {
    uint32_t* d_grid = nullptr; uint32_t* d_raw = nullptr;
    uint32_t* d_stats = nullptr; uint32_t* h_stats = nullptr;
    bool built = false, pinned = false;
    uint64_t epoch = 0; float alpha = 0.f;
    uint64_t builds = 0; bool active = false; uint64_t samples_in_box = 0, samples_live = 0;
};

struct Model {
    MeshState* mesh = nullptr;
    InferState* infer = nullptr;
// ... 98 lines not shown
```

Measured before the change: 2.138 billion ray-samples/s.

## Precompute Adam bias-correction table and speed up optimizer gradient partial reduction

Adds a device table of Adam bias-correction factors indexed by step count, so the optimizer does a lookup instead of two exp2f and a sqrt per parameter. The partial-gradient reduction now loads raw fp16 pairs and accumulates them with v_fma_mix instructions instead of converting each half to float first. The hash-level lookup is made wave-uniform with readfirstlane and a ballot fallback, and the optimizer kernel gets launch_bounds occupancy 4. The costs are an extra gather from the table, mixed-precision adds of two halves before the fp32 accumulate, and possible register spills from the occupancy hint.

```diff
diff --git a/include/mon_core_diag.h b/include/mon_core_diag.h
--- a/include/mon_core_diag.h
+++ b/include/mon_core_diag.h
@@ -36,6 +36,8 @@
                                    const float* cstar, const float* mstar, const float* dstar, const float* dn, float w_rgb, float w_mask, float w_depth,
                                    float huber, float* out_l, float* out_W, float* out_D, float* out_dalpha, float* out_dc);
 int mon_debug_checkpoint_timing(int enable, double* kernel_ms);
+int mon_debug_adam_lr(int device, float beta1, float beta2, float lr0, const uint32_t* cs, size_t n, float* lr_table, float* lr_direct, uint32_t* table_len);
+int mon_debug_adam_bias_table(mon_object* obj, int switch_off, uint32_t* table_len);
 
 #ifdef __cplusplus
 }
diff --git a/ro-map_amd/__init__.py b/ro-map_amd/__init__.py
--- a/ro-map_amd/__init__.py
+++ b/ro-map_amd/__init__.py
@@ -4,4 +4,4 @@
                               diag_symbols, yaml_number, MonRenderSkipStats, render_scene, scene_samples, scene_composite, PoseRefineParams, pose_refine_default,
                       PoseC2FParams, pose_c2f_default, pose_c2f_weights, scene_pose_loss, scene_refine_camera, scene_pose_samples,
                       scene_composite_grad, CheckpointInfo, checkpoint_info, checkpoint_timing, MON_LOAD_BOXES,
-                      rccl_lib, rccl_lib_path, rccl_symbols, gather_plan, Gather)
+                      rccl_lib, rccl_lib_path, rccl_symbols, gather_plan, Gather, adam_lr)
diff --git a/ro-map_amd/binding.py b/ro-map_amd/binding.py
--- a/ro-map_amd/binding.py
+++ b/ro-map_amd/binding.py
@@ -195,6 +195,8 @@
     "mon_debug_set_train_occupancy": (C.c_int, [C.c_void_p, C.c_void_p]),
     "mon_debug_set_render_grid": (C.c_int, [C.c_void_p, C.c_int, C.c_void_p]),
     "mon_debug_checkpoint_timing": (C.c_int, [C.c_int, C.POINTER(C.c_double)]),
+    "mon_debug_adam_lr": (C.c_int, [C.c_int, C.c_float, C.c_float, C.c_float, C.c_void_p, C.c_size_t, C.c_void_p, C.c_void_p, C.POINTER(C.c_uint32)]),
+    "mon_debug_adam_bias_table": (C.c_int, [C.c_void_p, C.c_int, C.POINTER(C.c_uint32)]),
     "mon_debug_scene_samples": (C.c_int, [C.c_void_p, C.c_size_t, C.c_int, MonBBox, C.c_void_p, C.c_size_t, C.c_void_p, C.c_void_p, C.c_void_p, C.c_void_p]),
     "mon_debug_scene_composite": (C.c_int, [C.c_int, C.c_uint32, C.c_uint32, C.c_void_p, C.c_void_p, C.c_void_p, C.c_void_p, C.c_void_p, C.c_void_p,
             C.c_void_p, C.c_void_p, C.c_void_p]),
@@ -417,6 +419,11 @@
     i = C.c_uint32(0); n = C.c_uint32(0); _check(diag_lib().mon_debug_fast_index(C.byref(cfg), level, x, y, z, C.byref(i), C.byref(n))); return i.value, n.value
 
 
+def adam_lr(beta1, beta2, lr0, cs, device=0):
+    c = np.ascontiguousarray(cs, np.uint32).ravel(); a = np.empty(c.size, np.float32); b = np.empty(c.size, np.float32); n = C.c_uint32(0)
+    _check(diag_lib().mon_debug_adam_lr(device, float(beta1), float(beta2), float(lr0), _p(c), c.size, _p(a), _p(b), C.byref(n))); return a, b, n.value
+
+
 def microbench(mode, pattern, n_entries, n_ops, device=0):
     ms = C.c_float(0); _check(diag_lib().mon_microbench(device, mode, pattern, n_entries, n_ops, C.byref(ms))); return ms.value
 
@@ -597,6 +604,9 @@
         w = np.ascontiguousarray(bits, np.uint32); assert w.size == 8192
         _check(diag_lib().mon_debug_set_train_occupancy(self.h, _p(w)))
 
+    def adam_bias_table(self, switch_off=False):
+        n = C.c_uint32(0); _check(diag_lib().mon_debug_adam_bias_table(self.h, int(bool(switch_off)), C.byref(n))); return n.value
+
     def render_jobs(self, side=0):
         n = C.c_uint32(0); _check(diag_lib().mon_debug_render_jobs(self.h, int(side), C.byref(n))); return n.value
 
diff --git a/ro-map_amd/csrc/adam_bias.h b/ro-map_amd/csrc/adam_bias.h
--- /dev/null
+++ b/ro-map_amd/csrc/adam_bias.h
@@ -0,0 +1,24 @@
+#pragma once
+#include <cstdint>
+#include <hip/hip_runtime.h>
+
+namespace mon {
+
+typedef float adam_f2 __attribute__((ext_vector_type(2)));
+constexpr uint32_t kAdamBiasCap = 2048, kAdamBiasMargin = 16;
+
+inline uint32_t adam_bias_table_len(float log2_beta1, float log2_beta2) {
+    for (uint32_t cs = 1; cs + kAdamBiasMargin <= kAdamBiasCap; ++cs)
+        if ((float)cs * log2_beta1 <= -26.f && (float)cs * log2_beta2 <= -26.f) return cs + kAdamBiasMargin;
+    return 0u;
+}
+
+__device__ __forceinline__ adam_f2 adam_bias_direct(uint32_t cs, float log2_beta1, float log2_beta2) {
+    return adam_f2{ sqrtf(1.f - exp2f((float)cs * log2_beta2)), 1.f - exp2f((float)cs * log2_beta1) };
+}
+__device__ __forceinline__ adam_f2 adam_bias_lookup(const float* __restrict__ table, uint32_t last, uint32_t cs) {
+    return reinterpret_cast<const adam_f2*>(table)[cs < last ? cs : last];
+}
+__device__ __forceinline__ float adam_bias_lr(float lr0, adam_f2 sd) { return lr0 * sd.x / sd.y; }
+
+}
diff --git a/ro-map_amd/csrc/diag.cpp b/ro-map_amd/csrc/diag.cpp
--- a/ro-map_amd/csrc/diag.cpp
+++ b/ro-map_amd/csrc/diag.cpp
@@ -11,6 +11,7 @@
 int ensure_ema_current(Model& m);
 int microbench(int device, int mode, int pattern, uint32_t n_entries, uint32_t n_ops, float* ms);
 int selftest_mfma(int device, const uint16_t* A, const uint16_t* B, float* D);
+int adam_lr_probe(int device, float beta1, float beta2, float lr0, const uint32_t* cs, size_t n, float* lr_ship, float* lr_direct, uint32_t* table_len);
 bool read_yaml_number(const std::string& text, const char* key, double& v);
 
 #define HIPCHECK(expr)                                                                                         \
@@ -155,6 +156,16 @@
 int mon_selftest_mfma(int device, const uint16_t* A, const uint16_t* B, float* D) { REQUIRE(A, "A"); REQUIRE(B, "B"); REQUIRE(D, "D");
     return selftest_mfma(device, A, B, D); }
 int mon_debug_checkpoint_timing(int enable, double* kernel_ms) { return mon::checkpoint_timing(enable, kernel_ms); }
+int mon_debug_adam_lr(int device, float beta1, float beta2, float lr0, const uint32_t* cs, size_t n, float* lr_table, float* lr_direct, uint32_t* table_len) {
+    if (n) { REQUIRE(cs, "cs"); REQUIRE(lr_table, "lr_table"); REQUIRE(lr_direct, "lr_direct"); }
+    return adam_lr_probe(device, beta1, beta2, lr0, cs, n, lr_table, lr_direct, table_len);
+}
+int mon_debug_adam_bias_table(mon_object* o, int switch_off, uint32_t* table_len) {
+    REQUIRE(o, "object"); mon::Model& m = *o->m;
+    if (switch_off) { m.P.bias = nullptr; m.P.bias_last = 0u; }
+    if (table_len) *table_len = m.P.bias ? m.P.bias_last + 1u : 0u;
+    return MON_OK;
+}
 int mon_debug_occupancy_state(mon_object* o, uint32_t out[2]) {
     if (!o || !o->m || !out) { mon::set_error("debug_occupancy_state: null argument"); return MON_ERR_ARG; }
     out[0] = o->m->occ_refreshed_iter; out[1] = o->m->occ_next_refresh; return MON_OK;
diff --git a/ro-map_amd/csrc/diag_kernels.hip b/ro-map_amd/csrc/diag_kernels.hip
--- a/ro-map_amd/csrc/diag_kernels.hip
+++ b/ro-map_amd/csrc/diag_kernels.hip
@@ -1,3 +1,4 @@
+#include <cmath>
 #include "device_common.h"
 #include "model.h"
 
@@ -33,5 +34,39 @@
     return MON_OK;
 }
 
+__global__ void __launch_bounds__(256) k_adam_lr_probe(const float* __restrict__ table, uint32_t last, const uint32_t* __restrict__ cs, uint32_t n, float lr0,
+        float log2_beta1, float log2_beta2, float* __restrict__ lr_ship, float* __restrict__ lr_direct) {
+    const uint32_t i = blockIdx.x * blockDim.x + threadIdx.x;
+    if (i >= n) return;
+    const adam_f2 direct = adam_bias_direct(cs[i], log2_beta1, log2_beta2);
+    lr_ship[i] = adam_bias_lr(lr0, table ? adam_bias_lookup(table, last, cs[i]) : direct);
+    lr_direct[i] = adam_bias_lr(lr0, direct);
+}
+
+int adam_lr_probe(int device, float beta1, float beta2, float lr0, const uint32_t* cs, size_t n, float* lr_ship, float* lr_direct, uint32_t* table_len) {
+    int ndev = 0;
+    if (hipGetDeviceCount(&ndev) != hipSuccess || ndev < 1 || use_device(device) != hipSuccess) { set_error("adam_lr_probe: no HIP device");
+        return MON_ERR_NO_DEVICE; }
+    const float l1 = std::log2(beta1), l2 = std::log2(beta2);
+    const uint32_t len = adam_bias_table_len(l1, l2);
+    if (table_len) *table_len = len;
+    if (n == 0) return MON_OK;
+    char* d = nullptr; const size_t b_tab = (size_t)2 * kAdamBiasCap * 4, b_n = n * 4;
+    if (hipMalloc((void**)&d, b_tab + 3 * b_n) != hipSuccess) { set_error("adam_lr_probe: hipMalloc failed"); return MON_ERR_HIP; }
+    float* d_tab = reinterpret_cast<float*>(d); uint32_t* d_cs = reinterpret_cast<uint32_t*>(d + b_tab); float* d_ship = reinterpret_cast<float*>(d + b_tab + b_n);
+    float* d_dir = reinterpret_cast<float*>(d + b_tab + 2 * b_n);
+    hipError_t e = hipMemcpy(d_cs, cs, b_n, hipMemcpyHostToDevice);
+    if (e == hipSuccess) {
+        launch_adam_bias_table(nullptr, d_tab, len, l1, l2);
+        hipLaunchKernelGGL(k_adam_lr_probe, dim3((uint32_t)((n + 255) / 256)), dim3(256), 0, nullptr, len ? d_tab : nullptr, len ? len - 1u : 0u, d_cs, (uint32_t)n,
+                lr0, l1, l2, d_ship, d_dir);
+        e = hipGetLastError();
+    }
+    if (e == hipSuccess) e = hipMemcpy(lr_ship, d_ship, b_n, hipMemcpyDeviceToHost);
+    if (e == hipSuccess) e = hipMemcpy(lr_direct, d_dir, b_n, hipMemcpyDeviceToHost);
+    (void)hipFree(d);
+    if (e != hipSuccess) { set_error("adam_lr_probe: %s", hipGetErrorString(e)); return MON_ERR_HIP; }
+    return MON_OK;
+}
 
 }
diff --git a/ro-map_amd/csrc/kernels_optim.hip b/ro-map_amd/csrc/kernels_optim.hip
--- a/ro-map_amd/csrc/kernels_optim.hip
+++ b/ro-map_amd/csrc/kernels_optim.hip
@@ -10,15 +10,28 @@
 
 template <bool STREAM, class T> __device__ __forceinline__ void state_store(T v, T* p) { policy_store<STREAM ? MON_SP_STATE : MON_SP_PLAIN>(v, p); }
 
-__device__ __forceinline__ float adam_update(float g, float w, float& m1, float& m2, uint32_t& steps, float lr0, const OptimConst& oc, uint32_t step_cap) {
+__device__ __forceinline__ float adam_update(float g, float w, float& m1, float& m2, uint32_t& steps, float lr0, const OptimConst& oc, uint32_t step_cap,
+        bool table, float lr_table) {
     const float gsq = g * g;
     m1 = oc.beta1 * m1 + (1.f - oc.beta1) * g;
     m2 = oc.beta2 * m2 + (1.f - oc.beta2) * gsq;
     const uint32_t cs = min(steps + 1u, step_cap); steps = cs;
-    const float lr = lr0 * sqrtf(1.f - exp2f((float)cs * oc.log2_beta2)) / (1.f - exp2f((float)cs * oc.log2_beta1));
+    const float lr = table ? lr_table : adam_bias_lr(lr0, adam_bias_direct(cs, oc.log2_beta1, oc.log2_beta2));
     const float eff = lr / (sqrtf(m2) + oc.epsilon);
     return w - eff * m1;
 }
+template <bool HI> __device__ __forceinline__ float add_f16_f16(uint32_t a, uint32_t b) {
+    float r;
+    if (HI) asm("v_fma_mix_f32 %0, %1, %3, %2 op_sel:[1,0,1] op_sel_hi:[1,0,1]" : "=v"(r) : "v"(a), "v"(b), "s"(1.0f));
+    else asm("v_fma_mix_f32 %0, %1, %3, %2 op_sel:[0,0,0] op_sel_hi:[1,0,1]" : "=v"(r) : "v"(a), "v"(b), "s"(1.0f));
+    return r;
+}
+template <bool HI> __device__ __forceinline__ float add_f16_f32(uint32_t h, float acc) {
+    float r;
+    if (HI) asm("v_fma_mix_f32 %0, %1, %3, %2 op_sel:[1,0,0] op_sel_hi:[1,0,0]" : "=v"(r) : "v"(h), "v"(acc), "s"(1.0f));
+    else asm("v_fma_mix_f32 %0, %1, %3, %2 op_sel:[0,0,0] op_sel_hi:[1,0,0]" : "=v"(r) : "v"(h), "v"(acc), "s"(1.0f));
+    return r;
+}
 
 __device__ __forceinline__ void ema_catch_up(half8_t& e, const half8_t& w, uint32_t t, uint32_t k, float log2_d) {
     const float dk = exp2f((float)k * log2_d), a = dk * (1.f - exp2f((float)t * log2_d)), b = 1.f - dk, inv = 1.f / (1.f - exp2f((float)(t + k) * log2_d));
@@ -28,7 +41,7 @@
 
 template <bool DENSE, bool LAZY, bool ONE = false ,
           bool LIVE = false>
-__global__ void __launch_bounds__(256) k_optimizer(ParamPtrs p, OptimConst oc, const DevState* __restrict__ st, DevState* __restrict__ st_next, OptimNext nx,
+__global__ void __launch_bounds__(256, 4) k_optimizer(ParamPtrs p, OptimConst oc, const DevState* __restrict__ st, DevState* __restrict__ st_next, OptimNext nx,
         uint32_t lazy_below) {
     const uint32_t n_extra = nx.cand_blocks + nx.pos_blocks, n_opt = gridDim.x - n_extra, vblock = blockIdx.x < n_opt ? blockIdx.x + n_extra
             : blockIdx.x - n_opt;
@@ -47,6 +60,15 @@
             s0 = u32x4{ v[0] & 0xffffu, v[0] >> 16, v[1] & 0xffffu, v[1] >> 16 }; s1 = u32x4{ v[2] & 0xffffu, v[2] >> 16, v[3] & 0xffffu, v[3] >> 16 }; }
         else { s0 = *reinterpret_cast<const u32x4*>(p.steps + i0); s1 = *reinterpret_cast<const u32x4*>(p.steps + i0 + 4); }
     };
+    const bool bias_table = p.bias != nullptr;
+    auto bias_lr = [&](const uint32_t (&sc)[8], float lr0, float (&lrv)[8]) __attribute__((always_inline)) {
+#pragma unroll
+        for (int j = 0; j < 8; ++j) lrv[j] = lr0;
+        if (bias_table) {
+#pragma unroll
+            for (int j = 0; j < 8; ++j) lrv[j] = adam_bias_lr(lr0, adam_bias_lookup(p.bias, p.bias_last, min(sc[j] + 1u, step_cap)));
+        }
+    };
     struct Pre { float4_t w0, w1, a0, a1, b0, b1; u32x4 s0, s1; half8_t e; float4_t gm0, gm1; };
     auto issue = [&](uint32_t c, Pre& L) __attribute__((always_inline)) {
         const uint32_t i0 = c << 3;
@@ -155,22 +177,28 @@
                 }
                 uint32_t n_part = 0;
                 if (p.gpart) {
-                    const uint32_t e0 = (i0 - oc.n_mlp) >> 1; int lvl = 0;
-#pragma unroll
-                    for (int l = 1; l < kMaxLevels; ++l) { const bool in = e0 >= p.sl.entry_offset[l]; lvl += in ? 1 : 0;
-                        lvl_off = in ? p.sl.entry_offset[l] : lvl_off; lvl_end = in ? p.sl.entry_offset[l + 1] : lvl_end; }
-                    n_part = p.sl.P[lvl];
+                    const uint32_t e0 = (i0 - oc.n_mlp) >> 1, e_first = (uint32_t)__builtin_amdgcn_readfirstlane((int)e0);
+                    uint32_t w_off = 0u, w_end = p.sl.entry_offset[1]; int w_lvl = 0;
+#pragma unroll
+                    for (int l = 1; l < kMaxLevels; ++l) { const bool in = e_first >= p.sl.entry_offset[l]; w_lvl += in ? 1 : 0;
+                        w_off = in ? p.sl.entry_offset[l] : w_off; w_end = in ? p.sl.entry_offset[l + 1] : w_end; }
+                    if (__ballot(e0 < w_off || e0 >= w_end) == 0ull) { lvl_off = w_off; lvl_end = w_end; n_part = p.sl.P[w_lvl]; }
+                    else {
+                        int lvl = 0;
+#pragma unroll
+                        for (int l = 1; l < kMaxLevels; ++l) { const bool in = e0 >= p.sl.entry_offset[l]; lvl += in ? 1 : 0;
+                            lvl_off = in ? p.sl.entry_offset[l] : lvl_off; lvl_end = in ? p.sl.entry_offset[l + 1] : lvl_end; }
+                        n_part = p.sl.P[lvl];
+                    }
                 }
                 const uint16_t* pp = p.gpart + ((i0 - oc.n_mlp) >> 2);
                 const size_t plane = p.part_stride >> 2;
-                auto quad = [&](uint32_t q, float (&v)[8]) {
+                auto quad = [&](uint32_t q, uint32_t (&h)[4]) {
 #pragma unroll
                     for (int f = 0; f < 2; ++f)
 #pragma unroll
-                        for (int b = 0; b < 2; ++b) {
-                            const half2_t h = *reinterpret_cast<const half2_t*>(pp + ((size_t)(q * 2u + (uint32_t)f) * 2u + (uint32_t)b) * plane);
-                            v[2 * b + f] = (float)h.x; v[2 * (2 + b) + f] = (float)h.y;
-                        }
+                        for (int b = 0; b < 2; ++b)
+                            h[2 * f + b] = *reinterpret_cast<const uint32_t*>(pp + ((size_t)(q * 2u + (uint32_t)f) * 2u + (uint32_t)b) * plane);
                 };
                 uint32_t q = 0;
 #if defined(MON_OPT_ABLATE) && (MON_OPT_ABLATE & 2)
@@ -178,14 +206,20 @@
                 n_part = 0;
 #endif
                 for (; q + 2 <= n_part; q += 2) {
-                    float va[8], vb[8]; quad(q, va); quad(q + 1u, vb);
-#pragma unroll
-                    for (int j = 0; j < 8; ++j) g[j] += va[j] + vb[j];
+                    uint32_t ha[4], hb[4]; quad(q, ha); quad(q + 1u, hb);
+#pragma unroll
+                    for (int f = 0; f < 2; ++f)
+#pragma unroll
+                        for (int b = 0; b < 2; ++b) { g[2 * b + f] += add_f16_f16<false>(ha[2 * f + b], hb[2 * f + b]);
+                            g[2 * (2 + b) + f] += add_f16_f16<true>(ha[2 * f + b], hb[2 * f + b]); }
                 }
                 for (; q < n_part; ++q) {
-                    float va[8]; quad(q, va);
-#pragma unroll
-                    for (int j = 0; j < 8; ++j) g[j] += va[j];
+                    uint32_t ha[4]; quad(q, ha);
+#pragma unroll
+                    for (int f = 0; f < 2; ++f)
+#pragma unroll
+                        for (int b = 0; b < 2; ++b) { g[2 * b + f] = add_f16_f32<false>(ha[2 * f + b], g[2 * b + f]);
+                            g[2 * (2 + b) + f] = add_f16_f32<true>(ha[2 * f + b], g[2 * (2 + b) + f]); }
                 }
 #pragma unroll
                 for (int j = 0; j < 8; ++j) { any |= g[j] != 0.f; g[j] = unscale(g[j]); }
@@ -214,6 +248,7 @@
                 float m1[8] = { a0[0], a0[1], a0[2], a0[3], a1[0], a1[1], a1[2], a1[3] };
                 float m2[8] = { b0[0], b0[1], b0[2], b0[3], b1[0], b1[1], b1[2], b1[3] };
                 uint32_t sc[8] = { s0.x, s0.y, s0.z, s0.w, s1.x, s1.y, s1.z, s1.w };
+                float lrv[8]; bias_lr(sc, lr0, lrv);
 #pragma unroll
                 for (int j = 0; j < 8; ++j) {
                     float gj = g[j];
@@ -222,7 +257,7 @@
 #if defined(MON_OPT_ABLATE) && (MON_OPT_ABLATE & 1)
                     m1[j] += gj; m2[j] += gj; sc[j] += 1u; w[j] -= 1e-6f * gj;
 #else
-                    w[j] = adam_update(gj, w[j], m1[j], m2[j], sc[j], lr0, oc, step_cap);
+                    w[j] = adam_update(gj, w[j], m1[j], m2[j], sc[j], lr0, oc, step_cap, bias_table, lrv[j]);
 #endif
                     wh[j] = (half_t)w[j];
                 }
@@ -353,10 +388,11 @@
                 float m1[8] = { a0[0], a0[1], a0[2], a0[3], a1[0], a1[1], a1[2], a1[3] };
                 float m2[8] = { b0[0], b0[1], b0[2], b0[3], b1[0], b1[1], b1[2], b1[3] };
                 uint32_t sc[8] = { t0[0], t0[1], t0[2], t0[3], t1[0], t1[1], t1[2], t1[3] };
+                float lrv[8]; bias_lr(sc, lr0, lrv);
 #pragma unroll
                 for (int j = 0; j < 8; ++j) {
                     if (g[j] == 0.f) continue;
-                    w[j] = adam_update(g[j], w[j], m1[j], m2[j], sc[j], lr0, oc, step_cap);
+                    w[j] = adam_update(g[j], w[j], m1[j], m2[j], sc[j], lr0, oc, step_cap, bias_table, lrv[j]);
                     wh[j] = (half_t)w[j];
                 }
                 state_store<false>(float4_t{ w[0], w[1], w[2], w[3] }, reinterpret_cast<float4_t*>(st_master(c)));
@@ -554,6 +590,14 @@
     hipLaunchKernelGGL(k_master_to_half, dim3(1024), dim3(256), 0, s, master, half, n);
 }
 
+__global__ void __launch_bounds__(256) k_adam_bias_table(float* __restrict__ table, uint32_t len, float log2_beta1, float log2_beta2) {
+    const uint32_t cs = blockIdx.x * blockDim.x + threadIdx.x;
+    if (cs < len) reinterpret_cast<adam_f2*>(table)[cs] = adam_bias_direct(cs, log2_beta1, log2_beta2);
+}
+void launch_adam_bias_table(hipStream_t s, float* table, uint32_t len, float log2_beta1, float log2_beta2) {
+    if (len) hipLaunchKernelGGL(k_adam_bias_table, dim3((len + 255u) / 256u), dim3(256), 0, s, table, len, log2_beta1, log2_beta2);
+}
+
 void launch_optimizer(hipStream_t s, const ParamPtrs& p, const OptimConst& oc, const DevState* st, DevState* st_next, const OptimNext& nx,
         uint32_t lazy_below) {
     const uint32_t chunks = oc.n_params >> 3;
diff --git a/ro-map_amd/csrc/model.cpp b/ro-map_amd/csrc/model.cpp
--- a/ro-map_amd/csrc/model.cpp
+++ b/ro-map_amd/csrc/model.cpp
@@ -466,6 +466,14 @@
     if ((rc = dev_alloc(m, m.P.half, n, false)) || (rc = dev_alloc(m, m.P.ema, n)) || (rc = records ? MON_OK : dev_alloc(m, m.d_ema_step, n / 8 + 1)) ||
         
         (rc = dev_alloc(m, m.P.gmlp, m.nd.n_mlp)) || (rc = dev_alloc(m, m.P.ggrid, m.n_grid))) return rc;
+#ifndef MON_OPT_BIAS_DIRECT
+    if (const uint32_t bias_len = adam_bias_table_len(m.opt.log2_beta1, m.opt.log2_beta2)) {
+        float* tab = nullptr; if ((rc = dev_alloc(m, tab, 2 * (size_t)bias_len, false))) return rc;
+        launch_adam_bias_table(m.train_stream, tab, bias_len, m.opt.log2_beta1, m.opt.log2_beta2);
+        HIPCHECK(hipStreamSynchronize(m.train_stream));
+        m.P.bias = tab; m.P.bias_last = bias_len - 1u;
+    }
+#endif
     if (init_params) {
         std::vector<float> master; init_params_host(cfg, m.nd, m.n_params, master);
         const int urc = upload_master(m, master.data()); if (urc) return urc;
diff --git a/ro-map_amd/csrc/model.h b/ro-map_amd/csrc/model.h
--- a/ro-map_amd/csrc/model.h
+++ b/ro-map_amd/csrc/model.h
@@ -8,6 +8,7 @@
 #include "../../include/mon_core.h"
 #include "device_common.h"
 #include "frag_layout.h"
+#include "adam_bias.h"
 
 namespace mon {
 
@@ -74,6 +75,7 @@
     uint8_t* touched; uint32_t first_flag_chunk;
     int all_levels_dense;
     uint16_t* half_tiles;
+    const float* bias; uint32_t bias_last;
 };
 
 constexpr uint32_t kEncWholeMax = 163840u / 4u;
@@ -194,6 +196,7 @@
 
 void launch_optimizer(hipStream_t s, const ParamPtrs& p, const OptimConst& oc, const DevState* st, DevState* st_next, const OptimNext& nx, uint32_t lazy_below);
 void launch_ema_finalize(hipStream_t s, const ParamPtrs& p, const OptimConst& oc, const DevState* st);
+void launch_adam_bias_table(hipStream_t s, float* table, uint32_t len, float log2_beta1, float log2_beta2);
 void launch_reduce_partials(hipStream_t s, const float* partials, uint32_t n_partials, const NetDims& nd, float* gmlp, DevState* st);
 uint32_t fused_partial_cols(const NetDims& nd);
 
```

Result: slower. 2.117 billion ray-samples/s (-1.0%).
